# emdgroup/tnmf

Hardware: AMD Instinct MI355X
Metric: MU-iterations/sec (higher is better)
Workload: dtype f32

## Files before the change

include/tnmf_hip.h:

```cpp
#ifndef TNMF_HIP_H
#define TNMF_HIP_H

#include <stddef.h>

#ifdef __cplusplus
extern "C" {
#endif

#define TNMF_HIP_ABI_VERSION 8

enum {
    TNMF_OK = 0,
    TNMF_E_NULL = -1,
    TNMF_E_GEOM = -2,
    TNMF_E_DTYPE = -3,
    TNMF_E_WORKSPACE = -4,
    TNMF_E_UNSUPPORTED = -5,
    TNMF_E_STRIDE = -6
};

typedef struct tnmf_hip_ctx tnmf_hip_ctx;

typedef struct {
    int ndim;
    int N;
    int M;
    int C;
    int D[3];
    int A[3];
    int dtype;
    int h_row_stride;
} tnmf_hip_geom;

enum { TNMF_PATH_AUTO = 0, TNMF_PATH_GENERIC = 1, TNMF_PATH_MFMA = 2, TNMF_PATH_FFT = 3, TNMF_PATH_HYBRID = 4,
       TNMF_PATH_SPLIT = 5 };

int tnmf_hip_ctx_set_split(tnmf_hip_ctx *ctx, int enable);

int tnmf_hip_ctx_set_persistent(tnmf_hip_ctx *ctx, int mode);
int tnmf_hip_ctx_last_schedule_persistent(const tnmf_hip_ctx *ctx);

int tnmf_hip_abi_version(void);
int tnmf_hip_ctx_h_row_stride(tnmf_hip_ctx *ctx, const tnmf_hip_geom *geom, int *stride_out);
const char *tnmf_hip_strerror(int code);

int tnmf_hip_ctx_create(int device_id, tnmf_hip_ctx **out);
int tnmf_hip_ctx_destroy(tnmf_hip_ctx *ctx);
int tnmf_hip_ctx_reserve(tnmf_hip_ctx *ctx, const tnmf_hip_geom *geom);
int tnmf_hip_ctx_set_path(tnmf_hip_ctx *ctx, int path);
const char *tnmf_hip_ctx_last_path(const tnmf_hip_ctx *ctx);
int tnmf_hip_ctx_set_cache(tnmf_hip_ctx *ctx, int enable);
int tnmf_hip_ctx_invalidate(tnmf_hip_ctx *ctx);
int tnmf_hip_ctx_bind(tnmf_hip_ctx *ctx, const tnmf_hip_geom *geom, const void *H, const void *V);
int tnmf_hip_ctx_cache_counters(const tnmf_hip_ctx *ctx, unsigned long long out[4]);


int tnmf_hip_reconstruct(tnmf_hip_ctx *ctx, const tnmf_hip_geom *geom, const void *W, const void *H, void *R,
                         void *stream);

int tnmf_hip_grad_H(tnmf_hip_ctx *ctx, const tnmf_hip_geom *geom, const void *V, const void *R_or_null,
                    const void *W, const void *H, void *neg, void *pos, void *stream);

int tnmf_hip_grad_W(tnmf_hip_ctx *ctx, const tnmf_hip_geom *geom, const void *V, const void *R_or_null,
                    const void *W, const void *H, void *neg, void *pos, void *stream);

int tnmf_hip_mu_update(tnmf_hip_ctx *ctx, int dtype, void *arr, const void *neg, void *pos, double reg,
                       size_t n_elems, void *stream);

int tnmf_hip_normalize_W(tnmf_hip_ctx *ctx, const tnmf_hip_geom *geom, void *W, void *stream);

int tnmf_hip_energy(tnmf_hip_ctx *ctx, const tnmf_hip_geom *geom, const void *V, const void *W, const void *H,
                    double *out_host, void *stream);

int tnmf_hip_convolve_multi_1d(tnmf_hip_ctx *ctx, int dtype, int ndim, size_t rows, const int *shape,
                               const void *in, void *out, void *tmp, const double *kernel0, int len0,
                               const double *kernel1, int len1, void *stream);

int tnmf_hip_convolve_axis(tnmf_hip_ctx *ctx, int dtype, size_t rows, int len, size_t inner, const void *in, void *out,
                           const double *kernel, int klen, void *stream);


enum { TNMF_MODE_VALID = 0, TNMF_MODE_FULL = 1, TNMF_MODE_CIRCULAR = 2, TNMF_MODE_REFLECT = 3 };

int tnmf_hip_pad_H(tnmf_hip_ctx *ctx, const tnmf_hip_geom *geom, int mode, const void *H, void *Hpad, void *stream);
int tnmf_hip_fold_H(tnmf_hip_ctx *ctx, const tnmf_hip_geom *geom, int mode, const void *Gpad, void *G, void *stream);


int tnmf_hip_update_H(tnmf_hip_ctx *ctx, const tnmf_hip_geom *geom, const void *V, const void *W, void *H_inout,
                      void *R_scratch, int r_is_valid, double eps, double sparsity, void *stream);

int tnmf_hip_update_H_ex(tnmf_hip_ctx *ctx, const tnmf_hip_geom *geom, int mode, const void *V, const void *W,
                         void *H_inout, void *R_scratch, double eps, double sparsity, double inhibition,
                         double cross_inhibition, const double *kernel0, int len0, const double *kernel1, int len1,
                         const double *kernel2, int len2, void *stream);

int tnmf_hip_grad_W_fused(tnmf_hip_ctx *ctx, const tnmf_hip_geom *geom, const void *V, const void *W, const void *H,
                          void *R_scratch, int r_is_valid, void *negpos, void *stream);

enum { TNMF_OP_UPDATE_H = 0, TNMF_OP_GRAD_W = 1, TNMF_OP_APPLY_W = 2 };
typedef struct {
    int kind;
    int n0, n1;
    double a, b;
} tnmf_hip_op;
int tnmf_hip_run_schedule(tnmf_hip_ctx *ctx, const tnmf_hip_geom *geom, const void *V, void *W_inout, void *H_inout,
                          void *R_scratch, void *acc, const tnmf_hip_op *ops, int n_ops, double eps, double sparsity,
                          void *stream);

int tnmf_hip_axpby(tnmf_hip_ctx *ctx, int dtype, void *acc, const void *g, double a, double b, size_t n_elems,
                   void *stream);

int tnmf_hip_sum_parts(tnmf_hip_ctx *ctx, int dtype, const void *parts, int n_parts, size_t n_elems, void *out,
                       void *stream);

int tnmf_hip_apply_W(tnmf_hip_ctx *ctx, const tnmf_hip_geom *geom, void *W_inout, void *negpos, double eps,
                     void *stream);


int tnmf_hip_beta_fields(tnmf_hip_ctx *ctx, int dtype, double beta, double eps, const void *V, const void *R, void *Q,
                         void *P, size_t n_elems, void *stream);

int tnmf_hip_update_H_beta(tnmf_hip_ctx *ctx, const tnmf_hip_geom *geom, int mode, const void *V, const void *W,
                           void *H_inout, void *R_scratch, double eps, double sparsity, double inhibition,
                           double cross_inhibition, const double *kernel0, int len0, const double *kernel1, int len1,
                           const double *kernel2, int len2, double beta, void *stream);

int tnmf_hip_grad_W_beta(tnmf_hip_ctx *ctx, const tnmf_hip_geom *geom, const void *V, const void *W, const void *H,
                         void *R_scratch, int r_is_valid, void *negpos, double beta, double eps, void *stream);

int tnmf_hip_energy_beta(tnmf_hip_ctx *ctx, const tnmf_hip_geom *geom, double beta, double eps, const void *V,
                         const void *W, const void *H, double *out_host, void *stream);


int tnmf_hip_weighted_fields(tnmf_hip_ctx *ctx, int dtype, double beta, double eps, const void *V, const void *G,
                             const void *R, void *Q, void *P, size_t n_elems, void *stream);

int tnmf_hip_update_H_weighted(tnmf_hip_ctx *ctx, const tnmf_hip_geom *geom, int mode, const void *V, const void *G,
                               const void *W, void *H_inout, void *R_scratch, double eps, double sparsity,
                               double inhibition, double cross_inhibition, const double *kernel0, int len0,
                               const double *kernel1, int len1, const double *kernel2, int len2, double beta,
                               void *stream);

int tnmf_hip_grad_W_weighted(tnmf_hip_ctx *ctx, const tnmf_hip_geom *geom, const void *V, const void *G, const void *W,
                             const void *H, void *R_scratch, int r_is_valid, void *negpos, double beta, double eps,
                             void *stream);

int tnmf_hip_energy_weighted(tnmf_hip_ctx *ctx, const tnmf_hip_geom *geom, double beta, double eps, const void *V,
                             const void *G, const void *W, const void *H, double *out_host, void *stream);


int tnmf_hip_ctx_set_objective_tap(tnmf_hip_ctx *ctx, double *per_sample_dev);

int tnmf_hip_sample_objective(tnmf_hip_ctx *ctx, const tnmf_hip_geom *geom, double beta, double eps, const void *V,
                              const void *G_or_null, const void *W, const void *H, double *per_sample_dev, void *stream);

enum { TNMF_GROUP_FLIP = 0, TNMF_GROUP_MIRRORS = 1, TNMF_GROUP_ROT90 = 2, TNMF_GROUP_DIHEDRAL = 3 };

int tnmf_hip_group_expand_W(tnmf_hip_ctx *ctx, const tnmf_hip_geom *geom, int group, const void *W, void *W_eff,
                            void *stream);

int tnmf_hip_group_fold_grad_W(tnmf_hip_ctx *ctx, const tnmf_hip_geom *geom, int group, const void *negpos_eff,
                               void *negpos, void *stream);

int tnmf_hip_group_apply_W(tnmf_hip_ctx *ctx, const tnmf_hip_geom *geom, int group, void *W_inout, void *W_eff_out,
                           const void *negpos_eff, double eps, void *stream);

typedef struct tnmf_hip_atom_ops tnmf_hip_atom_ops;

int tnmf_hip_atom_ops_create(tnmf_hip_ctx *ctx, int ndim, const int *A, int T, int nnz, const int *t,
                             const int *out_px, const int *in_px, const double *w, tnmf_hip_atom_ops **out);
int tnmf_hip_atom_ops_destroy(tnmf_hip_atom_ops *ops);

int tnmf_hip_ops_expand_W(tnmf_hip_ctx *ctx, const tnmf_hip_geom *geom, const tnmf_hip_atom_ops *ops, const void *W,
                          void *W_eff, void *stream);

int tnmf_hip_ops_fold_grad_W(tnmf_hip_ctx *ctx, const tnmf_hip_geom *geom, const tnmf_hip_atom_ops *ops,
                             const void *negpos_eff, void *negpos, void *stream);

int tnmf_hip_ops_apply_W(tnmf_hip_ctx *ctx, const tnmf_hip_geom *geom, const tnmf_hip_atom_ops *ops, void *W_inout,
                         void *W_eff_out, const void *negpos_eff, double eps, void *stream);

int tnmf_hip_find_peaks(tnmf_hip_ctx *ctx, const tnmf_hip_geom *geom, const void *H, double threshold, const int *radius,
                        int group, long long *idx_out, void *val_out, size_t capacity, unsigned long long *count_out,
                        void *stream);

#define TNMF_EVENTS_CELL_1D 256
#define TNMF_EVENTS_CELL_2D 16

int tnmf_hip_events_render(tnmf_hip_ctx *ctx, const tnmf_hip_geom *geom, const void *W_eff, const int *images,
                           long long n_images, const int *cell_start, const void *strength, long long n_events, void *R,
                           void *stream);

int tnmf_hip_events_update(tnmf_hip_ctx *ctx, const tnmf_hip_geom *geom, int mode, const void *W_eff, const int *events,
                           void *strength_inout, long long n_events, const void *V, const void *R, double eps,
                           double sparsity, void *stream);

int tnmf_hip_events_gain(tnmf_hip_ctx *ctx, const tnmf_hip_geom *geom, int mode, const void *W_eff, const int *events,
                         const void *strength, long long n_events, const void *V, const void *R, double *gain,
                         double *mag , void *stream);

#ifndef TNMF_EVENTS_SEGMENT
#define TNMF_EVENTS_SEGMENT 64
#endif

int tnmf_hip_events_grad_W(tnmf_hip_ctx *ctx, const tnmf_hip_geom *geom, int mode, const int *events, const int *by_plane,
                           const int *plane_start, const void *strength, long long n_events, const void *V, const void *R,
                           void *workspace, void *negpos_eff, void *stream);

int tnmf_hip_events_norms(tnmf_hip_ctx *ctx, const tnmf_hip_geom *geom, int mode, const void *W_eff,
                          double *b , void *stream);

int tnmf_hip_pursuit_score(tnmf_hip_ctx *ctx, const tnmf_hip_geom *geom, const void *a, const double *b, void *gain_out,
// ... 12 lines not shown
```

tnmf_amd/_lib.py:

```python
import ctypes
import os
from typing import Optional, Sequence

_HERE = os.path.dirname(os.path.abspath(__file__))
LIB_PATH = os.path.join(_HERE, 'lib', 'libtnmf_hip.so')

ABI_VERSION = 8

EXPORTS = (
    'tnmf_hip_abi_version', 'tnmf_hip_strerror', 'tnmf_hip_ctx_create', 'tnmf_hip_ctx_destroy',
    'tnmf_hip_ctx_reserve', 'tnmf_hip_ctx_set_path', 'tnmf_hip_ctx_last_path', 'tnmf_hip_reconstruct',
    'tnmf_hip_grad_H', 'tnmf_hip_grad_W', 'tnmf_hip_mu_update', 'tnmf_hip_normalize_W', 'tnmf_hip_energy',
    'tnmf_hip_convolve_multi_1d', 'tnmf_hip_update_H', 'tnmf_hip_grad_W_fused', 'tnmf_hip_apply_W',
    'tnmf_hip_pad_H', 'tnmf_hip_fold_H', 'tnmf_hip_ctx_set_cache', 'tnmf_hip_ctx_invalidate',
    'tnmf_hip_ctx_set_split', 'tnmf_hip_ctx_h_row_stride', 'tnmf_hip_ctx_bind', 'tnmf_hip_ctx_set_persistent',
    'tnmf_hip_ctx_last_schedule_persistent',
    'tnmf_hip_ctx_cache_counters', 'tnmf_hip_sum_parts',
    'tnmf_hip_update_H_ex', 'tnmf_hip_run_schedule', 'tnmf_hip_axpby', 'tnmf_hip_convolve_axis',
    'tnmf_hip_beta_fields', 'tnmf_hip_update_H_beta', 'tnmf_hip_grad_W_beta', 'tnmf_hip_energy_beta',
    'tnmf_hip_weighted_fields', 'tnmf_hip_update_H_weighted', 'tnmf_hip_grad_W_weighted', 'tnmf_hip_energy_weighted',
    'tnmf_hip_group_expand_W', 'tnmf_hip_group_fold_grad_W', 'tnmf_hip_group_apply_W',
    'tnmf_hip_atom_ops_create', 'tnmf_hip_atom_ops_destroy', 'tnmf_hip_ops_expand_W', 'tnmf_hip_ops_fold_grad_W',
    'tnmf_hip_ops_apply_W',
    'tnmf_hip_ctx_set_objective_tap', 'tnmf_hip_sample_objective',
    'tnmf_hip_find_peaks',
    'tnmf_hip_events_render', 'tnmf_hip_events_update', 'tnmf_hip_events_grad_W', 'tnmf_hip_events_gain',
    'tnmf_hip_events_norms', 'tnmf_hip_pursuit_score', 'tnmf_hip_pursuit_pick',
)

MODES = {'valid': 0, 'full': 1, 'circular': 2, 'reflect': 3}

GROUPS = {'flip': 0, 'mirrors': 1, 'rot90': 2, 'dihedral': 3}

EVENT_CELLS = {1: (256,), 2: (16, 16)}
EVENT_SEGMENT = 64

PATHS = {'auto': 0, 'generic': 1, 'mfma': 2, 'fft': 3, 'hybrid': 4, 'split': 5}


class Geom(ctypes.Structure):
    _fields_ = [('ndim', ctypes.c_int), ('N', ctypes.c_int), ('M', ctypes.c_int), ('C', ctypes.c_int),
                ('D', ctypes.c_int * 3), ('A', ctypes.c_int * 3), ('dtype', ctypes.c_int),
                ('h_row_stride', ctypes.c_int)]


class Op(ctypes.Structure):
    _fields_ = [('kind', ctypes.c_int), ('n0', ctypes.c_int), ('n1', ctypes.c_int), ('a', ctypes.c_double),
                ('b', ctypes.c_double)]


OP_UPDATE_H, OP_GRAD_W, OP_APPLY_W = 0, 1, 2

E_GEOM = -2
E_UNSUPPORTED = -5
E_STRIDE = -6


class TnmfHipError(RuntimeError):
    def __init__(self, code: int, where: str, text: str):
        super().__init__(f'{where} failed with code {code}: {text}')
        self.code = code


_lib: Optional[ctypes.CDLL] = None


def load() -> ctypes.CDLL:
    global _lib
    if _lib is not None:
        return _lib
    if not os.path.exists(LIB_PATH):
        raise RuntimeError(
            f'{LIB_PATH} not found: the HIP extension is not built. The hip backend has no CPU fallback. '
            'Run `make -C tnmf_amd/csrc` (needs hipcc) first.')
    lib = ctypes.CDLL(LIB_PATH)
    missing = [name for name in EXPORTS if not hasattr(lib, name)]
    if missing:
        raise RuntimeError(f'{LIB_PATH} does not export {missing}')
    vp, ci, cd, sz = ctypes.c_void_p, ctypes.c_int, ctypes.c_double, ctypes.c_size_t
    gp = ctypes.POINTER(Geom)
    lib.tnmf_hip_abi_version.restype = ci
    lib.tnmf_hip_strerror.restype = ctypes.c_char_p
    lib.tnmf_hip_strerror.argtypes = [ci]
    lib.tnmf_hip_ctx_create.argtypes = [ci, ctypes.POINTER(vp)]
    lib.tnmf_hip_ctx_destroy.argtypes = [vp]
    lib.tnmf_hip_ctx_reserve.argtypes = [vp, gp]
    lib.tnmf_hip_ctx_set_path.argtypes = [vp, ci]
    lib.tnmf_hip_ctx_set_cache.argtypes = [vp, ci]
    lib.tnmf_hip_ctx_set_split.argtypes = [vp, ci]
    lib.tnmf_hip_ctx_set_persistent.argtypes = [vp, ci]
    lib.tnmf_hip_ctx_last_schedule_persistent.argtypes = [vp]
    lib.tnmf_hip_ctx_last_schedule_persistent.restype = ci
    lib.tnmf_hip_ctx_h_row_stride.argtypes = [vp, gp, ctypes.POINTER(ci)]
    lib.tnmf_hip_ctx_invalidate.argtypes = [vp]
    lib.tnmf_hip_ctx_bind.argtypes = [vp, gp, vp, vp]
    lib.tnmf_hip_ctx_cache_counters.argtypes = [vp, ctypes.POINTER(ctypes.c_ulonglong * 4)]
    lib.tnmf_hip_ctx_last_path.restype = ctypes.c_char_p
    lib.tnmf_hip_ctx_last_path.argtypes = [vp]
    lib.tnmf_hip_reconstruct.argtypes = [vp, gp, vp, vp, vp, vp]
    lib.tnmf_hip_grad_H.argtypes = [vp, gp, vp, vp, vp, vp, vp, vp, vp]
    lib.tnmf_hip_grad_W.argtypes = [vp, gp, vp, vp, vp, vp, vp, vp, vp]
    lib.tnmf_hip_mu_update.argtypes = [vp, ci, vp, vp, vp, cd, sz, vp]
    lib.tnmf_hip_normalize_W.argtypes = [vp, gp, vp, vp]
    lib.tnmf_hip_energy.argtypes = [vp, gp, vp, vp, vp, ctypes.POINTER(cd), vp]
    lib.tnmf_hip_convolve_multi_1d.argtypes = [vp, ci, ci, sz, ctypes.POINTER(ci), vp, vp, vp,
                                               ctypes.POINTER(cd), ci, ctypes.POINTER(cd), ci, vp]
    lib.tnmf_hip_convolve_axis.argtypes = [vp, ci, sz, ci, sz, vp, vp, ctypes.POINTER(cd), ci, vp]
    lib.tnmf_hip_update_H.argtypes = [vp, gp, vp, vp, vp, vp, ci, cd, cd, vp]
    lib.tnmf_hip_update_H_ex.argtypes = [vp, gp, ci, vp, vp, vp, vp, cd, cd, cd, cd, ctypes.POINTER(cd), ci,
                                         ctypes.POINTER(cd), ci, ctypes.POINTER(cd), ci, vp]
    lib.tnmf_hip_run_schedule.argtypes = [vp, gp, vp, vp, vp, vp, vp, ctypes.POINTER(Op), ci, cd, cd, vp]
    lib.tnmf_hip_grad_W_fused.argtypes = [vp, gp, vp, vp, vp, vp, ci, vp, vp]
    lib.tnmf_hip_apply_W.argtypes = [vp, gp, vp, vp, cd, vp]
    lib.tnmf_hip_sum_parts.argtypes = [vp, ci, vp, ci, sz, vp, vp]
    lib.tnmf_hip_axpby.argtypes = [vp, ci, vp, vp, cd, cd, sz, vp]
    lib.tnmf_hip_beta_fields.argtypes = [vp, ci, cd, cd, vp, vp, vp, vp, sz, vp]
    lib.tnmf_hip_update_H_beta.argtypes = [vp, gp, ci, vp, vp, vp, vp, cd, cd, cd, cd, ctypes.POINTER(cd), ci,
                                           ctypes.POINTER(cd), ci, ctypes.POINTER(cd), ci, cd, vp]
    lib.tnmf_hip_grad_W_beta.argtypes = [vp, gp, vp, vp, vp, vp, ci, vp, cd, cd, vp]
    lib.tnmf_hip_energy_beta.argtypes = [vp, gp, cd, cd, vp, vp, vp, ctypes.POINTER(cd), vp]
    lib.tnmf_hip_weighted_fields.argtypes = [vp, ci, cd, cd, vp, vp, vp, vp, vp, sz, vp]
    lib.tnmf_hip_update_H_weighted.argtypes = [vp, gp, ci, vp, vp, vp, vp, vp, cd, cd, cd, cd, ctypes.POINTER(cd), ci,
                                               ctypes.POINTER(cd), ci, ctypes.POINTER(cd), ci, cd, vp]
    lib.tnmf_hip_grad_W_weighted.argtypes = [vp, gp, vp, vp, vp, vp, vp, ci, vp, cd, cd, vp]
    lib.tnmf_hip_energy_weighted.argtypes = [vp, gp, cd, cd, vp, vp, vp, vp, ctypes.POINTER(cd), vp]
    lib.tnmf_hip_group_expand_W.argtypes = [vp, gp, ci, vp, vp, vp]
    lib.tnmf_hip_group_fold_grad_W.argtypes = [vp, gp, ci, vp, vp, vp]
    lib.tnmf_hip_group_apply_W.argtypes = [vp, gp, ci, vp, vp, vp, cd, vp]
    pi = ctypes.POINTER(ci)
    lib.tnmf_hip_atom_ops_create.argtypes = [vp, ci, pi, ci, ci, pi, pi, pi, ctypes.POINTER(cd), ctypes.POINTER(vp)]
    lib.tnmf_hip_atom_ops_destroy.argtypes = [vp]
    lib.tnmf_hip_ops_expand_W.argtypes = [vp, gp, vp, vp, vp, vp]
    lib.tnmf_hip_ops_fold_grad_W.argtypes = [vp, gp, vp, vp, vp, vp]
    lib.tnmf_hip_ops_apply_W.argtypes = [vp, gp, vp, vp, vp, vp, cd, vp]
    lib.tnmf_hip_ctx_set_objective_tap.argtypes = [vp, vp]
    lib.tnmf_hip_sample_objective.argtypes = [vp, gp, cd, cd, vp, vp, vp, vp, vp, vp]
    lib.tnmf_hip_find_peaks.argtypes = [vp, gp, vp, cd, pi, ci, vp, vp, sz, vp, vp]
    ll = ctypes.c_longlong
    lib.tnmf_hip_events_render.argtypes = [vp, gp, vp, vp, ll, vp, vp, ll, vp, vp]
    lib.tnmf_hip_events_update.argtypes = [vp, gp, ci, vp, vp, vp, ll, vp, vp, cd, cd, vp]
    lib.tnmf_hip_events_grad_W.argtypes = [vp, gp, ci, vp, vp, vp, vp, ll, vp, vp, vp, vp, vp]
    lib.tnmf_hip_events_gain.argtypes = [vp, gp, ci, vp, vp, vp, ll, vp, vp, vp, vp, vp]
    lib.tnmf_hip_events_norms.argtypes = [vp, gp, ci, vp, vp, vp]
    lib.tnmf_hip_pursuit_score.argtypes = [vp, gp, vp, vp, vp, vp, ll, vp]
    lib.tnmf_hip_pursuit_pick.argtypes = [vp, gp, ci, vp, vp, ll, vp, vp, vp, vp, vp, vp, vp]
    lib.tnmf_hip_pad_H.argtypes = [vp, gp, ci, vp, vp, vp]
    lib.tnmf_hip_fold_H.argtypes = [vp, gp, ci, vp, vp, vp]
    for name in EXPORTS:
        fn = getattr(lib, name)
        if fn.restype is ctypes.c_int or name not in ('tnmf_hip_strerror', 'tnmf_hip_ctx_last_path'):
            fn.restype = ci
    if lib.tnmf_hip_abi_version() != ABI_VERSION:
        raise RuntimeError(f'{LIB_PATH}: ABI version {lib.tnmf_hip_abi_version()} != expected {ABI_VERSION}')
    _lib = lib
    return lib


def check(code: int, where: str) -> None:
    if code != 0:
        text = load().tnmf_hip_strerror(code)
        raise TnmfHipError(code, where, text.decode() if text else '?')


def make_geom(n: int, m: int, c: int, sample_shape: Sequence[int], atom_shape: Sequence[int], dtype_code: int,
              h_row_stride: int = 0) -> Geom:
    k = len(atom_shape)
    if k not in (1, 2, 3) or len(sample_shape) != k:
        raise NotImplementedError('the hip backend supports 1, 2 or 3 shift dimensions')
    g = Geom()
    g.ndim, g.N, g.M, g.C, g.dtype = k, int(n), int(m), int(c), int(dtype_code)
    for i in range(k):
        g.D[i] = int(sample_shape[i])
        g.A[i] = int(atom_shape[i])
    g.h_row_stride = int(h_row_stride)
    return g
```

tnmf_amd/backends/HIP.py:

```python
from typing import Optional, Sequence, Tuple

import ctypes
import itertools
import weakref

import numpy as np
import torch

from .. import _lib, sharding, transforms as _transforms
from ._Backend import Backend, sliceNone

_DTYPES = {np.dtype('float32'): (torch.float32, 0), np.dtype('float64'): (torch.float64, 1)}


def _ptr(t: Optional[torch.Tensor]):
    return None if t is None else ctypes.c_void_p(t.data_ptr())


class _EventSpan:

    def __init__(self, backend, name):
        self.backend, self.name = backend, name

    def __enter__(self):
# ... 849 lines not shown
            _lib.check(self._lib.tnmf_hip_axpby(self._ctx, self._dtype_code, _ptr(d), _ptr(self._V_dev), -1., 1., d.numel(),
                                                self._stream()), 'tnmf_hip_axpby')
            taken = s * P + p
            for i in range(k):
                taken = taken * self._transform_shape[i] + u[:, i]
            return self.pursuit_round(W, b, d, taken.contiguous(), min_gain, buffers)

        def score(sample, plane, shift, strength, idx):
            at = torch.as_tensor(np.ascontiguousarray(idx, dtype=np.int64)).to(self._device)
            _, h, gain = self.pick_events(W, at, R)
            return h.cpu().numpy(), gain.cpu().numpy()

        def refit(sample, plane, shift, strength, n):
            return self.refit_events(V, W, sample, plane, shift, strength, n, 0., eps).cpu().numpy()
        return pursuit_loop(shape, self.atom_shape, self._sample_shape, self._reconstruction_mode, min_gain, max_events,
                            max_rounds, refit_iterations, sample.cpu().numpy(), plane.cpu().numpy(),
                            shift.cpu().numpy().reshape(-1, k), strength.cpu().numpy(), candidates, score, refit)

    def event_plane_list(self, plane: torch.Tensor, n_planes: int):
        with self._timed('event_plane_list'):
            K = plane.numel()
            sorted_plane, by_plane = torch.sort(plane, stable=True)
            plane_start = torch.searchsorted(sorted_plane, torch.arange(n_planes + 1, dtype=torch.int64,
                                                                        device=self._device)).to(torch.int32).contiguous()
            taps = self.n_channels * int(np.prod(self.atom_shape))
            workspace = torch.empty((K // _lib.EVENT_SEGMENT + n_planes) * 2 * taps, dtype=torch.float64,
                                    device=self._device)
        return by_plane.to(torch.int32).contiguous(), plane_start, workspace

    def gradient_W_event_list(self, W: torch.Tensor, events: torch.Tensor, lists, strength: torch.Tensor,
                              R: torch.Tensor) -> torch.Tensor:
        self._check_W(W)
        by_plane, plane_start, workspace = lists
        assert strength.is_contiguous() and strength.dtype == self._torch_dtype and events.shape[0] == strength.numel()
        assert by_plane.numel() == strength.numel() and plane_start.numel() == W.shape[0] + 1
        assert R.is_contiguous() and R.dtype == self._torch_dtype and tuple(R.shape) == tuple(self._V_dev.shape)
        negpos = torch.empty((2,) + tuple(W.shape), dtype=W.dtype, device=W.device)
        with self._timed('events_grad_W'):
            _lib.check(self._lib.tnmf_hip_events_grad_W(
                self._ctx, ctypes.byref(self._geom(self.n_local_samples, W.shape[0])), self._mode, _ptr(events),
                _ptr(by_plane), _ptr(plane_start), _ptr(strength), strength.numel(), _ptr(self._V_dev), _ptr(R),
                _ptr(workspace), _ptr(negpos), self._stream()), 'tnmf_hip_events_grad_W')
        return negpos

    def update_W_event_list(self, W: torch.Tensor, W_eff: Optional[torch.Tensor], transforms, negpos_eff: torch.Tensor,
                            eps: float = 1e-9) -> None:
        negpos = negpos_eff if transforms is None else self.fold_gradient_W(negpos_eff, transforms)
        self._all_reduce(negpos)
        keep = ~negpos[0].reshape(W.shape[0], -1).any(dim=1)
        kept = W.clone()
        if transforms is None:
            self.apply_W(W, negpos, eps)
        elif self._world == 1:
            self.apply_W_transformed(W, W_eff, negpos_eff, transforms, eps)
        else:
            self.apply_W(W, negpos, eps)
        W.copy_(torch.where(keep.reshape((-1,) + (1,) * (W.dim() - 1)), kept, W))
        if transforms is not None:
            self.expand_W(W, transforms, W_eff)

    def fit_events(self, V, W: torch.Tensor, W_eff: Optional[torch.Tensor], transforms, sample, plane, shift, strength,
                   n_iterations: int, update_H: bool = True, update_W: bool = True, sparsity: float = 0.,
                   eps: float = 1e-9) -> torch.Tensor:
        if self._G_dev is not None:
            raise NotImplementedError('fit_events is unweighted')
        D = W if transforms is None else W_eff
        sample, plane, shift, strength = self._check_events(D.shape[0], sample, plane, shift, strength)
        images, cell_start, events = self.event_list(sample, plane, shift)
        lists = self.event_plane_list(plane, D.shape[0]) if update_W else None
        strength = strength.clone()
        R = torch.empty_like(self._V_dev)
        for _ in range(int(n_iterations)):
            if update_H:
                self.render_event_list(D, images, cell_start, strength, R)
                self.update_event_list(D, events, strength, R, sparsity, eps)
            if update_W:
                self.render_event_list(D, images, cell_start, strength, R)
                negpos_eff = self.gradient_W_event_list(D, events, lists, strength, R)
                self.update_W_event_list(W, W_eff, transforms, negpos_eff, eps)
        return strength

    @property
    def supports_schedules(self) -> bool:
        return self._mode == 0 and self._world == 1

    def prefers_schedule(self, H: torch.Tensor) -> bool:
        return self.supports_schedules and H.shape[0] > 0 and H.numel() <= (1 << 18)

    def blend_gradient_W(self, acc: torch.Tensor, g: torch.Tensor, a: float, b: float) -> torch.Tensor:
        assert acc.is_contiguous() and g.is_contiguous() and acc.shape == g.shape and acc.dtype == g.dtype
        _lib.check(self._lib.tnmf_hip_axpby(self._ctx, self._dtype_code, _ptr(acc), _ptr(g), float(a), float(b),
                                            acc.numel(), self._stream()), 'tnmf_hip_axpby')
        return acc

    def new_gradient_accumulator(self, W: torch.Tensor) -> torch.Tensor:
        return torch.empty((2,) + tuple(W.shape), dtype=W.dtype, device=W.device)

    def run_schedule(self, V, W: torch.Tensor, H: torch.Tensor, ops, acc: torch.Tensor, sparsity: float = 0.,
                     eps: float = 1e-9) -> None:
        assert self.supports_schedules
        if self._G_dev is not None:
            raise NotImplementedError('run_schedule is unweighted; a weighted fit runs its epochs step by step')
        self._check_W(W)
        self._check_H(H, W.shape[0])
        ld = self._row_stride(H)
        assert ld is not None and H.shape[0] == self.n_local_samples
        assert acc.is_contiguous() and tuple(acc.shape) == (2,) + tuple(W.shape)
        assert acc.dtype == W.dtype and acc.device == W.device
        arr = (_lib.Op * max(1, len(ops)))()
        for i, op in enumerate(ops):
            if op[0] == 'W':
                arr[i].kind, arr[i].n0, arr[i].n1 = _lib.OP_APPLY_W, 0, 0
                continue
            sl = self._local(op[1])
            arr[i].n0, arr[i].n1 = sl.start, sl.stop
            if op[0] == 'H':
                arr[i].kind = _lib.OP_UPDATE_H
            else:
                arr[i].kind, arr[i].a, arr[i].b = _lib.OP_GRAD_W, float(op[2]), float(op[3])

        def run(Hc, ld):
            with self._timed('schedule'):
                return self._lib.tnmf_hip_run_schedule(
                    self._ctx, ctypes.byref(self._geom(Hc.shape[0], W.shape[0], ld)), _ptr(self._V_dev), _ptr(W),
                    _ptr(Hc), _ptr(self._R_scratch), _ptr(acc), arr, len(ops), float(eps), float(sparsity),
                    self._stream()), 'tnmf_hip_run_schedule'
        self._call_resident_H(H, W, True, run)

    def apply_W(self, W: torch.Tensor, negpos: torch.Tensor, eps: float = 1e-9) -> None:
        self._check_W(W)
        assert negpos.is_contiguous() and tuple(negpos.shape) == (2,) + tuple(W.shape)
        assert negpos.dtype == W.dtype and negpos.device == W.device
        g = self._geom(0, W.shape[0])
        with self._timed('apply_W'):
            _lib.check(self._lib.tnmf_hip_apply_W(self._ctx, ctypes.byref(g), _ptr(W), _ptr(negpos), float(eps),
                                                  self._stream()), 'tnmf_hip_apply_W')

    def local_gradient_W(self, V, W: torch.Tensor, H: torch.Tensor, s: slice = sliceNone, beta: float = 2.,
                         eps: float = 1e-9) -> torch.Tensor:
        self._check_beta(beta)
        ls = self._local(s)
        Hs, Vs = H[ls], self._V_dev[ls]
        self._check_W(W)
        self._check_H(Hs, W.shape[0])
        Hs = self._pad(Hs)
        negpos = torch.empty_like(self._negpos)
        Rs = self._R_scratch[ls] if Hs.shape[0] else None
        Gs = self._G(ls)

        def run(Hc, ld):
            g = self._geom(Hc.shape[0], W.shape[0], ld)
            r_valid = 0
            if self._timeline is not None and Hc.shape[0]:
                with self._timed('reconstruct'):
                    rc = self._lib.tnmf_hip_reconstruct(self._ctx, ctypes.byref(g), _ptr(W), _ptr(Hc), _ptr(Rs),
                                                        self._stream())
                if rc != 0:
                    return rc, 'tnmf_hip_reconstruct'
                r_valid = 1
            with self._timed('grad_W'):
                if Gs is not None:
                    return self._lib.tnmf_hip_grad_W_weighted(
                        self._ctx, ctypes.byref(g), _ptr(Vs), Gs, _ptr(W), _ptr(Hc), _ptr(Rs), r_valid, _ptr(negpos),
                        float(beta), float(eps), self._stream()), 'tnmf_hip_grad_W_weighted'
                rc = self._lib.tnmf_hip_grad_W_beta(self._ctx, ctypes.byref(g), _ptr(Vs), _ptr(W), _ptr(Hc), _ptr(Rs),
                                                    r_valid, _ptr(negpos), float(beta), float(eps), self._stream())
            return rc, 'tnmf_hip_grad_W_beta'
        self._call_resident_H(Hs, W, False, run)
        return negpos

    def all_reduce_gradient_W(self, negpos: torch.Tensor) -> torch.Tensor:
        self._all_reduce(negpos)
        return negpos

    def fused_update_W(self, V, W: torch.Tensor, H: torch.Tensor, s: slice = sliceNone, eps: float = 1e-9,
                       beta: float = 2.) -> None:
        negpos = self.local_gradient_W(V, W, H, s, beta=beta, eps=eps)
        self._all_reduce(negpos)
        self.apply_W(W, negpos, eps)

    def expand_W(self, W: torch.Tensor, transforms, W_eff: Optional[torch.Tensor] = None) -> torch.Tensor:
        kind, arg = self._transform_arg(transforms)
        self._check_W(W)
        shape = (W.shape[0] * _transforms.size(transforms),) + tuple(W.shape[1:])
        if W_eff is None:
            W_eff = torch.empty(shape, dtype=W.dtype, device=W.device)
        self._check_W(W_eff)
        assert tuple(W_eff.shape) == shape
        g = self._geom(0, W.shape[0])
        name = f'tnmf_hip_{kind}_expand_W'
        with self._timed(f'{kind}_expand_W'):
            _lib.check(getattr(self._lib, name)(self._ctx, ctypes.byref(g), arg, _ptr(W), _ptr(W_eff), self._stream()),
                       name)
        return W_eff

    def fold_gradient_W(self, negpos_eff: torch.Tensor, transforms) -> torch.Tensor:
        kind, arg = self._transform_arg(transforms)
        T = _transforms.size(transforms)
        assert negpos_eff.is_contiguous() and negpos_eff.dtype == self._torch_dtype and negpos_eff.shape[1] % T == 0
        assert tuple(negpos_eff.shape[2:]) == (self.n_channels,) + self.atom_shape and negpos_eff.shape[0] == 2
        M = negpos_eff.shape[1] // T
        negpos = torch.empty((2, M) + tuple(negpos_eff.shape[2:]), dtype=negpos_eff.dtype, device=negpos_eff.device)
        g = self._geom(0, M)
        name = f'tnmf_hip_{kind}_fold_grad_W'
        with self._timed(f'{kind}_fold_grad_W'):
            _lib.check(getattr(self._lib, name)(self._ctx, ctypes.byref(g), arg, _ptr(negpos_eff), _ptr(negpos),
                                                self._stream()), name)
        return negpos

    def apply_W_transformed(self, W: torch.Tensor, W_eff: torch.Tensor, negpos_eff: torch.Tensor, transforms,
                            eps: float = 1e-9) -> None:
        kind, arg = self._transform_arg(transforms)
        self._check_W(W)
        self._check_W(W_eff)
        T = _transforms.size(transforms)
        assert W_eff.shape[0] == W.shape[0] * T
        assert negpos_eff.is_contiguous() and tuple(negpos_eff.shape) == (2,) + tuple(W_eff.shape)
        assert negpos_eff.dtype == W.dtype and negpos_eff.device == W.device
        g = self._geom(0, W.shape[0])
        name = f'tnmf_hip_{kind}_apply_W'
        with self._timed(f'{kind}_apply_W'):
            _lib.check(getattr(self._lib, name)(self._ctx, ctypes.byref(g), arg, _ptr(W), _ptr(W_eff), _ptr(negpos_eff),
                                                float(eps), self._stream()), name)

    def fused_update_W_transformed(self, V, W: torch.Tensor, W_eff: torch.Tensor, H: torch.Tensor, s: slice = sliceNone,
                                   transforms=None, eps: float = 1e-9, beta: float = 2.) -> None:
        negpos_eff = self.local_gradient_W(V, W_eff, H, s, beta=beta, eps=eps)
        if self._world == 1:
            self.apply_W_transformed(W, W_eff, negpos_eff, transforms, eps)
            return
        negpos = self.fold_gradient_W(negpos_eff, transforms)
        self._all_reduce(negpos)
        self.apply_W(W, negpos, eps)
        self.expand_W(W, transforms, W_eff)
```

tnmf_amd/csrc/api.hip:

```cpp
#include <cstdlib>
#include <cstring>
#include <new>
#include <algorithm>
#include <vector>

#include "beta.h"
#include "events.h"
#include "fft.h"
#include "generic.h"
#include "mfma.h"
#include "peaks.h"
#include "split.h"
#include "volume.h"

namespace {

int to_geo(const tnmf_hip_geom *in, Geo *g) {
    if (!in) return TNMF_E_NULL;
    if (in->dtype != 0 && in->dtype != 1) return TNMF_E_DTYPE;
    if (in->ndim != 1 && in->ndim != 2) return TNMF_E_GEOM;
    g->N = in->N;
    g->M = in->M;
    g->C = in->C;
    if (in->ndim == 1) {
// ... 22 lines not shown

int to_vol(const tnmf_hip_geom *in, Vol *v) {
    if (!in) return TNMF_E_NULL;
    if (in->dtype != 0 && in->dtype != 1) return TNMF_E_DTYPE;
    v->N = in->N;
    v->M = in->M;
    v->C = in->C;
    if (v->N < 0 || v->M <= 0 || v->C <= 0) return TNMF_E_GEOM;
    for (int i = 0; i < 3; ++i) {
        v->D[i] = in->D[i];
        v->A[i] = in->A[i];
        if (v->D[i] <= 0 || v->A[i] <= 0) return TNMF_E_GEOM;
        v->H[i] = v->D[i] + v->A[i] - 1;
    }
    if (in->h_row_stride > 0 && in->h_row_stride != v->H[2]) return TNMF_E_STRIDE;
    return TNMF_OK;
}
inline size_t vol_vox(const Vol &v) { return (size_t)v.D[0] * v.D[1] * v.D[2]; }
inline size_t vol_hvox(const Vol &v) { return (size_t)v.H[0] * v.H[1] * v.H[2]; }
inline size_t vol_avox(const Vol &v) { return (size_t)v.A[0] * v.A[1] * v.A[2]; }
inline Geo vol_dict_geo(const Vol &v) {
    Geo g = {};
    g.N = v.N;
    g.M = v.M;
    g.C = v.C;
    g.Ay = v.A[0] * v.A[1];
    g.Ax = v.A[2];
    return g;
}

struct Scratch {
    size_t r_off, r_bytes;
    size_t part_off, part_bytes;
    size_t red_off, red_bytes;
    size_t total;
    int P;
};

Scratch plan_scratch(const tnmf_hip_ctx *ctx, const Geo &g, int dtype) {
    Scratch s;
    s.r_off = 0;
    s.r_bytes = align_up((size_t)g.N * g.C * g.Dy * g.Dx * esize(dtype), 256);
    int P = generic_corr_H_chunks(ctx, g);
    const int Pm = mfma_corr_H_chunks(ctx, g);
    if (Pm > P) P = Pm;
    s.P = P;
    s.part_off = s.r_off + s.r_bytes;
    s.part_bytes = align_up((size_t)P * g.M * g.C * g.Ay * g.Ax * 2 * sizeof(double), 256);
    s.red_off = s.part_off + s.part_bytes;
    s.red_bytes = align_up((size_t)(kEnergyPartials + 8) * sizeof(double), 256);
    s.total = s.red_off + s.red_bytes;
    return s;
}

int ensure_buffer(void **buf, size_t *have, size_t bytes, bool slack);

int ensure_scratch(tnmf_hip_ctx *ctx, size_t bytes) { return ensure_buffer(&ctx->ws, &ctx->ws_bytes, bytes, true); }
int ensure_hwork(tnmf_hip_ctx *ctx, size_t bytes) { return ensure_buffer(&ctx->hw, &ctx->hw_bytes, bytes, false); }

int ensure_buffer(void **buf, size_t *have, size_t bytes, bool slack) {
    if (bytes <= *have) return TNMF_OK;
    const size_t want = align_up(bytes + (slack ? bytes / 8 : 0), 1 << 20);
    void *bigger = nullptr;
    if (hipMalloc(&bigger, want) != hipSuccess) {
        (void)hipGetLastError();
        bigger = nullptr;
        if (!*buf) return TNMF_E_WORKSPACE;
    }
    if (*buf) {
        TNMF_HIP_TRY(hipDeviceSynchronize());
        TNMF_HIP_TRY(hipFree(*buf));
        *buf = nullptr;
        *have = 0;
    }
    if (!bigger && hipMalloc(&bigger, want) != hipSuccess) {
        (void)hipGetLastError();
        return TNMF_E_WORKSPACE;
    }
    *buf = bigger;
    *have = want;
    return TNMF_OK;
}

inline char *ws_at(tnmf_hip_ctx *ctx, size_t off) { return static_cast<char *>(ctx->ws) + off; }

enum Prim { kReconstruct, kCorrW, kCorrH };

bool use_fft_hybrid(const tnmf_hip_ctx *ctx, const Geo &g, int dtype) {
    if (ctx->path == TNMF_PATH_HYBRID) return fft_has(g, dtype);
    if (ctx->path != TNMF_PATH_AUTO || dtype != 0 || !fft_has(g, dtype)) return false;
    return (size_t)g.N * g.M * g.Hy * g.Hx >= ((size_t)1 << 19);
}

bool use_split(const tnmf_hip_ctx *ctx, const Geo &g, int dtype) {
    if (ctx->path == TNMF_PATH_SPLIT) return split_has_corr_W(g, dtype);
    if (ctx->path != TNMF_PATH_AUTO && ctx->path != TNMF_PATH_HYBRID) return false;
    if (ctx->path == TNMF_PATH_AUTO && (size_t)g.N * g.M * g.Hy * g.Hx < ((size_t)1 << 16)) return false;
    return ctx->split && split_has_corr_W(g, dtype, true);
}

bool use_mfma(const tnmf_hip_ctx *ctx, const Geo &g, int dtype, Prim prim) {
    if (ctx->path == TNMF_PATH_GENERIC || ctx->path == TNMF_PATH_FFT) return false;
    switch (prim) {
        case kReconstruct: return mfma_has_reconstruct(g, dtype);
        case kCorrW: return mfma_has_corr_W(g, dtype);
        default: return mfma_has_corr_H(g, dtype);
    }
}

#define ENTER(ctx, geom)                                   \
    if (!(ctx)) return TNMF_E_NULL;                        \
    Geo g;                                                 \
    {                                                      \
        const int _rc = to_geo((geom), &g);                \
        if (_rc != TNMF_OK) return _rc;                    \
    }                                                      \
    const int dtype = (geom)->dtype;                       \
    hipStream_t s = static_cast<hipStream_t>(stream);      \
    TNMF_HIP_TRY(hipSetDevice((ctx)->device));

#define CHECK(rc_expr)                  \
    do {                                \
        const int _rc = (rc_expr);      \
        if (_rc != TNMF_OK) return _rc; \
    } while (0)

#define VOL_ENTER(ctx, geom)                               \
    if (!(ctx)) return TNMF_E_NULL;                        \
    Vol v;                                                 \
    {                                                      \
        const int _rc = to_vol((geom), &v);                \
        if (_rc != TNMF_OK) return _rc;                    \
    }                                                      \
    const int dtype = (geom)->dtype;                       \
    hipStream_t s = static_cast<hipStream_t>(stream);      \
    TNMF_HIP_TRY(hipSetDevice((ctx)->device));             \
    (ctx)->last_path = "volume";

int vol_scratch(tnmf_hip_ctx *ctx, const Vol &v, int dtype, void **R, double **red, double **part = nullptr,
                int *P = nullptr, size_t extra = 0) {
    const size_t r_bytes = align_up((size_t)v.N * v.C * vol_vox(v) * esize(dtype), 256);
    const size_t e_bytes = align_up((size_t)(kEnergyPartials + 8) * sizeof(double), 256);
    const int chunks = vol_corr_H_chunks(ctx, v);
    const size_t p_bytes = align_up((size_t)chunks * v.M * v.C * vol_avox(v) * 2 * sizeof(double), 256);
    const int rc = ensure_scratch(ctx, r_bytes + e_bytes + p_bytes + extra);
    if (rc != TNMF_OK) return rc;
    if (R) *R = ws_at(ctx, 0);
    if (red) *red = reinterpret_cast<double *>(ws_at(ctx, r_bytes));
    if (part) *part = reinterpret_cast<double *>(ws_at(ctx, r_bytes + e_bytes));
    if (P) *P = chunks;
    return TNMF_OK;
}

int do_reconstruct(tnmf_hip_ctx *ctx, const Geo &g, int dtype, const void *W, const void *H, void *R, hipStream_t s) {
    if (g.N == 0) return TNMF_OK;
    if (ctx->path == TNMF_PATH_FFT || use_fft_hybrid(ctx, g, dtype)) {
        const int rc = fft_reconstruct(ctx, g, dtype, W, H, R, true, s);
        if (!(rc == TNMF_E_WORKSPACE && ctx->path == TNMF_PATH_AUTO)) return rc;
    }
    if (g.Hs == g.Hx && use_mfma(ctx, g, dtype, kReconstruct)) {
        ctx->last_path = "mfma";
        return mfma_reconstruct(ctx, g, (const float *)W, (const float *)H, (float *)R, s);
    }
    if (ctx->path == TNMF_PATH_MFMA) return g.Hs != g.Hx ? TNMF_E_STRIDE : TNMF_E_UNSUPPORTED;
    ctx->last_path = "generic";
    return generic_reconstruct(ctx, g, dtype, W, H, R, s);
}

int do_corr_W(tnmf_hip_ctx *ctx, const Geo &g, int dtype, const void *V, const void *R, const void *W, void *Hio,
              void *neg, void *pos, bool fused, double reg, hipStream_t s, const void *extra = nullptr) {
    if (g.N == 0) return TNMF_OK;
    if (extra && (!fused || ctx->path == TNMF_PATH_FFT)) return TNMF_E_UNSUPPORTED;
    if (ctx->path == TNMF_PATH_FFT)
        return fused ? fft_update_H(ctx, g, dtype, V, R, W, Hio, reg, s) : fft_grad_H(ctx, g, dtype, V, R, W, neg, pos, s);
    if (fused) fft_invalidate_H(ctx, g, dtype, Hio);
    if (use_split(ctx, g, dtype)) {
        const int rc = split_corr_W(ctx, g, (const float *)V, (const float *)R, (const float *)W, (float *)Hio,
                                    (float *)neg, (float *)pos, fused, (float)reg, s, (const float *)extra);
        if (rc == TNMF_OK) ctx->last_path = "split";
        if (rc != TNMF_E_UNSUPPORTED) return rc;
    }
    if ((!fused || g.Hs == g.Hx) && use_mfma(ctx, g, dtype, kCorrW)) {
        if (extra) return TNMF_E_UNSUPPORTED;
        ctx->last_path = "mfma";
        return mfma_corr_W(ctx, g, (const float *)V, (const float *)R, (const float *)W, (float *)Hio, (float *)neg,
                           (float *)pos, fused, (float)reg, s);
    }
    if (ctx->path == TNMF_PATH_MFMA || ctx->path == TNMF_PATH_SPLIT)
        return fused && g.Hs != g.Hx ? TNMF_E_STRIDE : TNMF_E_UNSUPPORTED;
    ctx->last_path = "generic";
    return generic_corr_W(ctx, g, dtype, V, R, W, Hio, neg, pos, fused, reg, s, extra);
}

int do_corr_H_partials(tnmf_hip_ctx *ctx, const Geo &g, int dtype, const void *V, const void *R, const void *H,
                       double *partials, int *P_out, hipStream_t s) {
    if (g.Hs == g.Hx && use_mfma(ctx, g, dtype, kCorrH)) {
        ctx->last_path = "mfma";
        *P_out = mfma_corr_H_chunks(ctx, g);
        return mfma_corr_H(ctx, g, (const float *)V, (const float *)R, (const float *)H, partials, *P_out, s);
    }
    if (ctx->path == TNMF_PATH_MFMA) return g.Hs != g.Hx ? TNMF_E_STRIDE : TNMF_E_UNSUPPORTED;
    ctx->last_path = "generic";
    *P_out = generic_corr_H_chunks(ctx, g);
    return generic_corr_H(ctx, g, dtype, V, R, H, partials, *P_out, s);
}

bool corr_H_on_fft(const tnmf_hip_ctx *ctx, const Geo &g, int dtype) {
    return ctx->path == TNMF_PATH_FFT || use_fft_hybrid(ctx, g, dtype);
}

int do_corr_H(tnmf_hip_ctx *ctx, const Geo &g, int dtype, const Scratch &sc, const void *V, const void *R,
              const void *H, void *neg, void *pos, hipStream_t s) {
    double *partials = reinterpret_cast<double *>(ws_at(ctx, sc.part_off));
    int P;
    if (g.N == 0) {
        TNMF_HIP_TRY(hipMemsetAsync(neg, 0, (size_t)g.M * g.C * g.Ay * g.Ax * esize(dtype), s));
        TNMF_HIP_TRY(hipMemsetAsync(pos, 0, (size_t)g.M * g.C * g.Ay * g.Ax * esize(dtype), s));
        return TNMF_OK;
    }
    if (corr_H_on_fft(ctx, g, dtype)) {
        const int rc = fft_grad_W(ctx, g, dtype, V, R, H, neg, pos, true, s);
        if (!(rc == TNMF_E_WORKSPACE && ctx->path == TNMF_PATH_AUTO)) return rc;
    }
    CHECK(do_corr_H_partials(ctx, g, dtype, V, R, H, partials, &P, s));
    return finalize_corr_H(g, dtype, partials, P, neg, pos, s);
}


int beta_fields_of(tnmf_hip_ctx *ctx, const Geo &g, int dtype, const double *beta, double eps, const void *V,
                   const void *G, void *R, const void **Q_out, hipStream_t s) {
    const size_t n = (size_t)g.N * g.C * g.Dy * g.Dx;
    CHECK(ensure_buffer(&ctx->qb, &ctx->qb_bytes, align_up(n * esize(dtype), 256), false));
    ctx->fft.V_volatile = ctx->qb;
    CHECK(launch_beta_fields(ctx, dtype, beta ? *beta : 2.0, eps, V, G, R, ctx->qb, R, n, s));
    *Q_out = ctx->qb;
    return TNMF_OK;
}

int sample_objective_of(tnmf_hip_ctx *ctx, int dtype, const double *beta, double eps, const void *V, const void *G,
                        const void *R, size_t N, size_t L, double *out, hipStream_t s) {
    const size_t B = objective_blocks(L);
    if (B > 1) CHECK(ensure_buffer(&ctx->ob, &ctx->ob_bytes, align_up(N * B * sizeof(double), 256), false));
    return launch_sample_objective(dtype, beta ? *beta : 2.0, eps, V, G, R, N, L, static_cast<double *>(ctx->ob), out, s);
}

inline int tap_objective(tnmf_hip_ctx *ctx, int dtype, const double *beta, double eps, const void *V, const void *G,
                         const void *R, size_t N, size_t L, hipStream_t s) {
    if (!ctx->obj_tap) return TNMF_OK;
    return sample_objective_of(ctx, dtype, beta, eps, V, G, R, N, L, ctx->obj_tap, s);
}

static_assert(kBetaPartials <= kEnergyPartials, "the energy words of the scratch hold the beta partials");

inline bool beta_ok(double beta) { return beta == beta && beta - beta == 0.0; }

int vol_api_reconstruct(tnmf_hip_ctx *ctx, const tnmf_hip_geom *geom, const void *W, const void *H, void *R, void *stream) {
    VOL_ENTER(ctx, geom);
    if (!W || (v.N > 0 && (!H || !R))) return TNMF_E_NULL;
    return vol_reconstruct(v, dtype, W, H, R, s);
}

int vol_api_grad_H(tnmf_hip_ctx *ctx, const tnmf_hip_geom *geom, const void *V, const void *R_or_null, const void *W,
                   const void *H, void *neg, void *pos, void *stream) {
    VOL_ENTER(ctx, geom);
    if (!W || (v.N > 0 && (!V || !neg || !pos))) return TNMF_E_NULL;
    const void *R = R_or_null;
    if (!R && v.N > 0) {
        if (!H) return TNMF_E_NULL;
        void *Rs;
        CHECK(vol_scratch(ctx, v, dtype, &Rs, nullptr));
        CHECK(vol_reconstruct(v, dtype, W, H, Rs, s));
        R = Rs;
    }
    return vol_corr_W(v, dtype, V, R, W, nullptr, neg, pos, false, 0.0, s);
}

int vol_api_grad_W(tnmf_hip_ctx *ctx, const tnmf_hip_geom *geom, const void *V, const void *R_scratch, int r_is_valid,
                   const void *W, const void *H, void *neg, void *pos, void *stream) {
    VOL_ENTER(ctx, geom);
    if (!neg || !pos || (v.N > 0 && (!V || !H))) return TNMF_E_NULL;
    const void *R = R_scratch;
    void *Rws;
    double *part;
    int P;
    CHECK(vol_scratch(ctx, v, dtype, &Rws, nullptr, &part, &P));
    if (v.N > 0 && !r_is_valid) {
        if (!W) return TNMF_E_NULL;
        void *Rs = R_scratch ? const_cast<void *>(R_scratch) : Rws;
        CHECK(vol_reconstruct(v, dtype, W, H, Rs, s));
        R = Rs;
    }
    return vol_corr_H(v, dtype, V, R, H, neg, pos, part, P, s);
}

int vol_api_energy(tnmf_hip_ctx *ctx, const tnmf_hip_geom *geom, const void *V, const void *W, const void *H,
                   double *out_host, void *stream) {
    VOL_ENTER(ctx, geom);
    if (!out_host) return TNMF_E_NULL;
    *out_host = 0.0;
    if (v.N == 0) return TNMF_OK;
    if (!V || !W || !H) return TNMF_E_NULL;
    void *Rs;
    double *red;
    CHECK(vol_scratch(ctx, v, dtype, &Rs, &red));
    CHECK(vol_reconstruct(v, dtype, W, H, Rs, s));
    CHECK(launch_half_sqdiff(ctx, dtype, V, Rs, (size_t)v.N * v.C * vol_vox(v), red, red + kEnergyPartials, s));
    TNMF_HIP_TRY(hipMemcpyAsync(out_host, red + kEnergyPartials, sizeof(double), hipMemcpyDeviceToHost, s));
    TNMF_HIP_TRY(hipStreamSynchronize(s));
    return TNMF_OK;
}
// ... 179 lines not shown

int tnmf_hip_ctx_create(int device_id, tnmf_hip_ctx **out) {
    if (!out) return TNMF_E_NULL;
    *out = nullptr;
    TNMF_HIP_TRY(hipSetDevice(device_id));
    hipDeviceProp_t prop;
    TNMF_HIP_TRY(hipGetDeviceProperties(&prop, device_id));
    {
        int rc = mfma_prepare_device();
        if (rc == TNMF_OK) rc = split_prepare_device();
        if (rc != TNMF_OK) return rc;
    }
    tnmf_hip_ctx *ctx = new (std::nothrow) tnmf_hip_ctx();
    if (!ctx) return TNMF_E_WORKSPACE;
    ctx->device = device_id;
    ctx->num_cu = prop.multiProcessorCount > 0 ? prop.multiProcessorCount : 256;
    ctx->path = TNMF_PATH_AUTO;
    ctx->last_path = "none";
    {
        const char *ab = tnmf_diag_env("TNMF_HIP_ABLATE");
        ctx->ablate = ab ? atoi(ab) : 0;
    }
    ctx->ws = nullptr;
    ctx->ws_bytes = 0;
    ctx->split = 1;
    ctx->wimg = nullptr;
    ctx->wimg_bytes = 0;
    ctx->fft = FftState();
    *out = ctx;
    return TNMF_OK;
}

int tnmf_hip_ctx_destroy(tnmf_hip_ctx *ctx) {
    if (!ctx) return TNMF_OK;
    int rc = TNMF_OK;
    if (ctx->ws || ctx->fft.ws || ctx->wimg || ctx->hw || ctx->qb || ctx->ob) {
        (void)hipSetDevice(ctx->device);
        (void)hipDeviceSynchronize();
    }
    fft_release(ctx);
    split_release(ctx);
    if (ctx->hw) (void)hipFree(ctx->hw);
    if (ctx->qb) (void)hipFree(ctx->qb);
    if (ctx->ob) (void)hipFree(ctx->ob);
    for (int i = 0; i < tnmf_hip_ctx::kOpSlots; ++i) {
        if (ctx->ops_done[i]) (void)hipEventDestroy(ctx->ops_done[i]);
        if (ctx->ops_pinned[i]) (void)hipHostFree(ctx->ops_pinned[i]);
    }
    if (ctx->ws) {
        const hipError_t e = hipFree(ctx->ws);
        if (e != hipSuccess) rc = (int)e;
    }
    delete ctx;
    return rc;
}

int tnmf_hip_ctx_reserve(tnmf_hip_ctx *ctx, const tnmf_hip_geom *geom) {
    void *stream = nullptr;
    if (is_vol(geom)) {
        VOL_ENTER(ctx, geom);
        (void)s;
        return vol_scratch(ctx, v, dtype, nullptr, nullptr);
    }
    ENTER(ctx, geom);
    (void)s;
    if (g.N > 0 && ctx->path == TNMF_PATH_FFT) CHECK(fft_reserve(ctx, g, dtype, true));
    if (g.N > 0 && use_fft_hybrid(ctx, g, dtype)) {
        const int rc = fft_reserve(ctx, g, dtype, false);
        if (rc != TNMF_OK && !(rc == TNMF_E_WORKSPACE && ctx->path == TNMF_PATH_AUTO)) return rc;
    }
    return ensure_scratch(ctx, plan_scratch(ctx, g, dtype).total);
}

int tnmf_hip_ctx_set_path(tnmf_hip_ctx *ctx, int path) {
    if (!ctx) return TNMF_E_NULL;
    if (path < TNMF_PATH_AUTO || path > TNMF_PATH_SPLIT) return TNMF_E_UNSUPPORTED;
    if (path != ctx->path) fft_invalidate(ctx);
    ctx->path = path;
    return TNMF_OK;
}

int tnmf_hip_ctx_set_split(tnmf_hip_ctx *ctx, int enable) {
    if (!ctx) return TNMF_E_NULL;
    ctx->split = enable != 0;
    return TNMF_OK;
}

int tnmf_hip_ctx_set_persistent(tnmf_hip_ctx *ctx, int mode) {
    if (!ctx) return TNMF_E_NULL;
    if (mode < 0 || mode > 2) return TNMF_E_UNSUPPORTED;
    ctx->persistent = mode;
    return TNMF_OK;
}

int tnmf_hip_ctx_last_schedule_persistent(const tnmf_hip_ctx *ctx) { return ctx && ctx->last_schedule_persistent ? 1 : 0; }

int tnmf_hip_ctx_set_cache(tnmf_hip_ctx *ctx, int enable) {
    if (!ctx) return TNMF_E_NULL;
    ctx->fft.cache_enabled = enable != 0;
    fft_invalidate(ctx);
    return TNMF_OK;
}

int tnmf_hip_ctx_bind(tnmf_hip_ctx *ctx, const tnmf_hip_geom *geom, const void *H, const void *V) {
    if (!ctx) return TNMF_E_NULL;
    if (!geom || !H) {
        fft_unbind(ctx);
        return TNMF_OK;
    }
    if (is_vol(geom)) {
        fft_unbind(ctx);
        return TNMF_OK;
    }
    Geo g;
    const int rc = to_geo(geom, &g);
    if (rc != TNMF_OK) return rc;
    fft_bind(ctx, g, geom->dtype, H, V);
    return TNMF_OK;
}

int tnmf_hip_ctx_cache_counters(const tnmf_hip_ctx *ctx, unsigned long long out[4]) {
    if (!ctx || !out) return TNMF_E_NULL;
    out[0] = ctx->fft.h_runs;
    out[1] = ctx->fft.h_hits;
    out[2] = ctx->fft.v_runs;
    out[3] = ctx->fft.v_hits;
    return TNMF_OK;
}

int tnmf_hip_ctx_invalidate(tnmf_hip_ctx *ctx) {
    if (!ctx) return TNMF_E_NULL;
    fft_invalidate(ctx);
    return TNMF_OK;
}

const char *tnmf_hip_ctx_last_path(const tnmf_hip_ctx *ctx) { return ctx ? ctx->last_path : "none"; }

#ifdef TNMF_DIAG
int tnmf_hip_diag_set_ablate(tnmf_hip_ctx *ctx, int mask) {
    if (!ctx) return TNMF_E_NULL;
    ctx->ablate = mask;
    return TNMF_OK;
}
#endif

int tnmf_hip_reconstruct(tnmf_hip_ctx *ctx, const tnmf_hip_geom *geom, const void *W, const void *H, void *R,
                         void *stream) {
    if (is_vol(geom)) return vol_api_reconstruct(ctx, geom, W, H, R, stream);
    ENTER(ctx, geom);
    if (!W || (g.N > 0 && (!H || !R))) return TNMF_E_NULL;
    return do_reconstruct(ctx, g, dtype, W, H, R, s);
}

int tnmf_hip_grad_H(tnmf_hip_ctx *ctx, const tnmf_hip_geom *geom, const void *V, const void *R_or_null,
                    const void *W, const void *H, void *neg, void *pos, void *stream) {
    if (is_vol(geom)) return vol_api_grad_H(ctx, geom, V, R_or_null, W, H, neg, pos, stream);
    ENTER(ctx, geom);
    if (!W || (g.N > 0 && (!V || !neg || !pos))) return TNMF_E_NULL;
    const void *R = R_or_null;
    if (!R && g.N > 0) {
        if (!H) return TNMF_E_NULL;
        const Scratch sc = plan_scratch(ctx, g, dtype);
        CHECK(ensure_scratch(ctx, sc.total));
        void *Rs = ws_at(ctx, sc.r_off);
        CHECK(do_reconstruct(ctx, g, dtype, W, H, Rs, s));
        R = Rs;
    }
    return do_corr_W(ctx, g, dtype, V, R, W, nullptr, neg, pos, false, 0.0, s);
}

int tnmf_hip_grad_W(tnmf_hip_ctx *ctx, const tnmf_hip_geom *geom, const void *V, const void *R_or_null,
                    const void *W, const void *H, void *neg, void *pos, void *stream) {
    if (is_vol(geom)) return vol_api_grad_W(ctx, geom, V, R_or_null, R_or_null != nullptr, W, H, neg, pos, stream);
    ENTER(ctx, geom);
    if (!neg || !pos || (g.N > 0 && (!V || !H))) return TNMF_E_NULL;
    const Scratch sc = plan_scratch(ctx, g, dtype);
    CHECK(ensure_scratch(ctx, sc.total));
    const void *R = R_or_null;
    if (!R && g.N > 0) {
        if (!W) return TNMF_E_NULL;
        void *Rs = ws_at(ctx, sc.r_off);
        CHECK(do_reconstruct(ctx, g, dtype, W, H, Rs, s));
        R = Rs;
    }
    return do_corr_H(ctx, g, dtype, sc, V, R, H, neg, pos, s);
}

int tnmf_hip_mu_update(tnmf_hip_ctx *ctx, int dtype, void *arr, const void *neg, void *pos, double reg,
                       size_t n_elems, void *stream) {
    if (!ctx) return TNMF_E_NULL;
    if (dtype != 0 && dtype != 1) return TNMF_E_DTYPE;
    if (n_elems > 0 && (!arr || !neg || !pos)) return TNMF_E_NULL;
    TNMF_HIP_TRY(hipSetDevice(ctx->device));
    fft_invalidate(ctx);
    return launch_mu_update(ctx, dtype, arr, neg, pos, reg, n_elems, static_cast<hipStream_t>(stream));
}

int tnmf_hip_normalize_W(tnmf_hip_ctx *ctx, const tnmf_hip_geom *geom, void *W, void *stream) {
    if (is_vol(geom)) {
        VOL_ENTER(ctx, geom);
        if (!W) return TNMF_E_NULL;
        return launch_apply_normalize_W(vol_dict_geo(v), dtype, W, nullptr, nullptr, 0.0, false, s);
    }
    ENTER(ctx, geom);
    if (!W) return TNMF_E_NULL;
    fft_invalidate_W(ctx);
    return launch_apply_normalize_W(g, dtype, W, nullptr, nullptr, 0.0, false, s);
}

static int energy_2d(tnmf_hip_ctx *ctx, const tnmf_hip_geom *geom, const void *V, const void *G, const void *W,
                     const void *H, double *out_host, const double *beta, double eps, void *stream) {
    ENTER(ctx, geom);
    if (!out_host) return TNMF_E_NULL;
    if (g.N == 0) {
        *out_host = 0.0;
        return TNMF_OK;
    }
    if (!V || !W || !H) return TNMF_E_NULL;
    const Scratch sc = plan_scratch(ctx, g, dtype);
    CHECK(ensure_scratch(ctx, sc.total));
    void *Rs = ws_at(ctx, sc.r_off);
    CHECK(do_reconstruct(ctx, g, dtype, W, H, Rs, s));
    double *red = reinterpret_cast<double *>(ws_at(ctx, sc.red_off));
    const size_t n = (size_t)g.N * g.C * g.Dy * g.Dx;
    CHECK(beta || G ? launch_beta_energy(ctx, dtype, beta ? *beta : 2.0, eps, V, G, Rs, n, red, red + kEnergyPartials, s)
                    : launch_half_sqdiff(ctx, dtype, V, Rs, n, red, red + kEnergyPartials, s));
    TNMF_HIP_TRY(hipMemcpyAsync(out_host, red + kEnergyPartials, sizeof(double), hipMemcpyDeviceToHost, s));
    TNMF_HIP_TRY(hipStreamSynchronize(s));
    return TNMF_OK;
}

int tnmf_hip_energy(tnmf_hip_ctx *ctx, const tnmf_hip_geom *geom, const void *V, const void *W, const void *H,
                    double *out_host, void *stream) {
    if (is_vol(geom)) return vol_api_energy(ctx, geom, V, W, H, out_host, stream);
    return energy_2d(ctx, geom, V, nullptr, W, H, out_host, nullptr, 0.0, stream);
}

int tnmf_hip_energy_beta(tnmf_hip_ctx *ctx, const tnmf_hip_geom *geom, double beta, double eps, const void *V,
                         const void *W, const void *H, double *out_host, void *stream) {
    if (beta == 2.0) return tnmf_hip_energy(ctx, geom, V, W, H, out_host, stream);
    if (!ctx || !geom) return TNMF_E_NULL;
    if (is_vol(geom) || !beta_ok(beta)) return TNMF_E_UNSUPPORTED;
    return energy_2d(ctx, geom, V, nullptr, W, H, out_host, &beta, eps, stream);
}

int tnmf_hip_energy_weighted(tnmf_hip_ctx *ctx, const tnmf_hip_geom *geom, double beta, double eps, const void *V,
                             const void *G, const void *W, const void *H, double *out_host, void *stream) {
    if (!G) return tnmf_hip_energy_beta(ctx, geom, beta, eps, V, W, H, out_host, stream);
    if (!ctx || !geom) return TNMF_E_NULL;
    if (is_vol(geom) || !beta_ok(beta)) return TNMF_E_UNSUPPORTED;
    return energy_2d(ctx, geom, V, G, W, H, out_host, beta == 2.0 ? nullptr : &beta, eps, stream);
}

int tnmf_hip_ctx_set_objective_tap(tnmf_hip_ctx *ctx, double *per_sample_dev) {
    if (!ctx) return TNMF_E_NULL;
    ctx->obj_tap = per_sample_dev;
    return TNMF_OK;
}

int tnmf_hip_sample_objective(tnmf_hip_ctx *ctx, const tnmf_hip_geom *geom, double beta, double eps, const void *V,
                              const void *G_or_null, const void *W, const void *H, double *per_sample_dev, void *stream) {
    if (!ctx || !geom) return TNMF_E_NULL;
    if (!beta_ok(beta)) return TNMF_E_UNSUPPORTED;
    const double *bp = beta == 2.0 ? nullptr : &beta;
    if (is_vol(geom)) {
        if (bp || G_or_null) return TNMF_E_UNSUPPORTED;
        VOL_ENTER(ctx, geom);
        if (v.N == 0) return TNMF_OK;
        if (!V || !W || !H || !per_sample_dev) return TNMF_E_NULL;
        void *Rs;
        CHECK(vol_scratch(ctx, v, dtype, &Rs, nullptr));
        CHECK(vol_reconstruct(v, dtype, W, H, Rs, s));
        return sample_objective_of(ctx, dtype, nullptr, eps, V, nullptr, Rs, (size_t)v.N, (size_t)v.C * vol_vox(v),
                                   per_sample_dev, s);
    }
    ENTER(ctx, geom);
    if (g.N == 0) return TNMF_OK;
    if (!V || !W || !H || !per_sample_dev) return TNMF_E_NULL;
    const Scratch sc = plan_scratch(ctx, g, dtype);
    CHECK(ensure_scratch(ctx, sc.total));
    void *Rs = ws_at(ctx, sc.r_off);
    CHECK(do_reconstruct(ctx, g, dtype, W, H, Rs, s));
    return sample_objective_of(ctx, dtype, bp, eps, V, G_or_null, Rs, (size_t)g.N, (size_t)g.C * g.Dy * g.Dx,
                               per_sample_dev, s);
}

int tnmf_hip_beta_fields(tnmf_hip_ctx *ctx, int dtype, double beta, double eps, const void *V, const void *R, void *Q,
                         void *P, size_t n_elems, void *stream) {
    if (!ctx) return TNMF_E_NULL;
    if (dtype != 0 && dtype != 1) return TNMF_E_DTYPE;
    if (!beta_ok(beta)) return TNMF_E_UNSUPPORTED;
    if (n_elems > 0 && (!V || !R || !Q || !P)) return TNMF_E_NULL;
    if (n_elems > 0 && (Q == V || Q == R || P == V)) return TNMF_E_NULL;
    TNMF_HIP_TRY(hipSetDevice(ctx->device));
    return launch_beta_fields(ctx, dtype, beta, eps, V, nullptr, R, Q, P, n_elems, static_cast<hipStream_t>(stream));
}

int tnmf_hip_weighted_fields(tnmf_hip_ctx *ctx, int dtype, double beta, double eps, const void *V, const void *G,
                             const void *R, void *Q, void *P, size_t n_elems, void *stream) {
    if (!ctx || !G) return TNMF_E_NULL;
    if (dtype != 0 && dtype != 1) return TNMF_E_DTYPE;
    if (!beta_ok(beta)) return TNMF_E_UNSUPPORTED;
    if (n_elems > 0 && (!V || !R || !Q || !P)) return TNMF_E_NULL;
    if (n_elems > 0 && (Q == V || Q == G || Q == R || P == V || P == G)) return TNMF_E_NULL;
    TNMF_HIP_TRY(hipSetDevice(ctx->device));
    return launch_beta_fields(ctx, dtype, beta, eps, V, G, R, Q, P, n_elems, static_cast<hipStream_t>(stream));
// ... 21 lines not shown
    if (dtype != 0 && dtype != 1) return TNMF_E_DTYPE;
    if (len < 0 || inner > 0x7fffffffu) return TNMF_E_GEOM;
    TNMF_HIP_TRY(hipSetDevice(ctx->device));
    if (rows == 0 || len == 0 || inner == 0) return TNMF_OK;
    if (!in || !out || in == out) return TNMF_E_NULL;
    return launch_convolve_axis(ctx, dtype, in, out, rows, len, (int)inner, kernel, klen, static_cast<hipStream_t>(stream));
}

int tnmf_hip_pad_H(tnmf_hip_ctx *ctx, const tnmf_hip_geom *geom, int mode, const void *H, void *Hpad, void *stream) {
    if (is_vol(geom)) return vol_api_pad_fold(ctx, geom, mode, false, H, Hpad, stream);
    ENTER(ctx, geom);
    if (mode < TNMF_MODE_VALID || mode > TNMF_MODE_REFLECT) return TNMF_E_UNSUPPORTED;
    if (g.N > 0 && (!H || !Hpad)) return TNMF_E_NULL;
    if (g.Hs != g.Hx) return TNMF_E_STRIDE;
    return launch_pad_fold(ctx, g, dtype, mode, false, H, Hpad, s);
}

int tnmf_hip_fold_H(tnmf_hip_ctx *ctx, const tnmf_hip_geom *geom, int mode, const void *Gpad, void *G, void *stream) {
    if (is_vol(geom)) return vol_api_pad_fold(ctx, geom, mode, true, Gpad, G, stream);
    ENTER(ctx, geom);
    if (mode < TNMF_MODE_VALID || mode > TNMF_MODE_REFLECT) return TNMF_E_UNSUPPORTED;
    if (g.N > 0 && (!Gpad || !G)) return TNMF_E_NULL;
    return launch_pad_fold(ctx, g, dtype, mode, true, Gpad, G, s);
}

static int update_H_2d(tnmf_hip_ctx *ctx, const tnmf_hip_geom *geom, int mode, const void *V, const void *G,
                       const void *W, void *H_inout, void *R_scratch, int r_is_valid, double eps, double sparsity,
                       double inhibition, double cross_inhibition, const double *kernel0, int len0,
                       const double *kernel1, int len1, const double *beta, void *stream) {
    ENTER(ctx, geom);
    if (mode < TNMF_MODE_VALID || mode > TNMF_MODE_REFLECT) return TNMF_E_UNSUPPORTED;
    if (g.N == 0) return TNMF_OK;
    if (!V || !W || !H_inout) return TNMF_E_NULL;
    const bool lateral = inhibition > 0 || cross_inhibition > 0;
    if (lateral && (!kernel0 || (geom->ndim == 2 && !kernel1))) return TNMF_E_NULL;
    if (inhibition < 0 || cross_inhibition < 0) return TNMF_E_GEOM;
    double reg = eps;
    if (sparsity > 0) reg += sparsity;
    const size_t es = esize(dtype);
    void *Rs = R_scratch;
    if (!Rs) {
        if (r_is_valid) return TNMF_E_NULL;
        const Scratch sc = plan_scratch(ctx, g, dtype);
        CHECK(ensure_scratch(ctx, sc.total));
        Rs = ws_at(ctx, sc.r_off);
    }
    const double one = 1.0;
    const double *ky = geom->ndim == 2 ? kernel0 : &one, *kx = geom->ndim == 2 ? kernel1 : kernel0;
    const int ly = geom->ndim == 2 ? len0 : 1, lx = geom->ndim == 2 ? len1 : len0;
    const double xc = cross_inhibition > 0 && g.M > 1 ? cross_inhibition / (g.M - 1) : 0.0;

    if (mode == TNMF_MODE_VALID) {
        const size_t nE = align_up((size_t)g.N * g.M * g.Hy * g.Hs * es, 256);
        const size_t nG = align_up((size_t)g.N * g.M * g.Hy * g.Hx * es, 256);
        void *E = nullptr;
        if (lateral) {
            CHECK(ensure_hwork(ctx, nE));
            E = ctx->hw;
            CHECK(launch_inhibition(ctx, dtype, g.N, g.M, g.Hy, g.Hs, H_inout, E, ky, ly, kx, lx, inhibition, xc, s));
        }
        if (!r_is_valid) CHECK(do_reconstruct(ctx, g, dtype, W, H_inout, Rs, s));
        CHECK(tap_objective(ctx, dtype, beta, eps, V, G, Rs, (size_t)g.N, (size_t)g.C * g.Dy * g.Dx, s));
        if (beta || G) CHECK(beta_fields_of(ctx, g, dtype, beta, eps, V, G, Rs, &V, s));
        int rc = do_corr_W(ctx, g, dtype, V, Rs, W, H_inout, nullptr, nullptr, true, reg, s, E);
        if (!E || (rc != TNMF_E_UNSUPPORTED && rc != TNMF_E_STRIDE)) return rc;
        if (ctx->hw_bytes < nE + 2 * nG) {
            CHECK(ensure_hwork(ctx, nE + 2 * nG));
            E = ctx->hw;
            CHECK(launch_inhibition(ctx, dtype, g.N, g.M, g.Hy, g.Hs, H_inout, E, ky, ly, kx, lx, inhibition, xc, s));
        }
        char *neg = static_cast<char *>(ctx->hw) + nE, *pos = neg + nG;
        CHECK(do_corr_W(ctx, g, dtype, V, Rs, W, nullptr, neg, pos, false, 0.0, s));
        fft_invalidate_H(ctx, g, dtype, H_inout);
        return launch_mu_update_extra(ctx, dtype, H_inout, neg, pos, E, (size_t)g.N * g.M * g.Hy, g.Hx, g.Hs, reg, s);
    }

    if (g.Hs != g.Hx) return TNMF_E_STRIDE;
    const int Sy = geom->ndim == 1 ? 1 : (mode == TNMF_MODE_FULL ? g.Dy - g.Ay + 1 : g.Dy);
    const int Sx = mode == TNMF_MODE_FULL ? g.Dx - g.Ax + 1 : g.Dx;
    if (Sy < 1 || Sx < 1) return TNMF_E_GEOM;
    const size_t nP = align_up((size_t)g.N * g.M * g.Hy * g.Hx * es, 256);
    const size_t nE = lateral ? align_up((size_t)g.N * g.M * Sy * Sx * es, 256) : 0;
    CHECK(ensure_hwork(ctx, 3 * nP + nE));
    char *Hp = static_cast<char *>(ctx->hw), *negp = Hp + nP, *posp = negp + nP;
    void *E = lateral ? posp + nP : nullptr;
    fft_invalidate(ctx);
    CHECK(launch_pad_fold(ctx, g, dtype, mode, false, H_inout, Hp, s));
    CHECK(do_reconstruct(ctx, g, dtype, W, Hp, Rs, s));
    CHECK(tap_objective(ctx, dtype, beta, eps, V, G, Rs, (size_t)g.N, (size_t)g.C * g.Dy * g.Dx, s));
    if (beta || G) CHECK(beta_fields_of(ctx, g, dtype, beta, eps, V, G, Rs, &V, s));
    CHECK(do_corr_W(ctx, g, dtype, V, Rs, W, nullptr, negp, posp, false, 0.0, s));
    if (lateral) CHECK(launch_inhibition(ctx, dtype, g.N, g.M, Sy, Sx, H_inout, E, ky, ly, kx, lx, inhibition, xc, s));
    fft_invalidate(ctx);
    return launch_fold_update(ctx, g, dtype, mode, Sy, Sx, H_inout, negp, posp, E, reg, s);
}

int tnmf_hip_update_H(tnmf_hip_ctx *ctx, const tnmf_hip_geom *geom, const void *V, const void *W, void *H_inout,
                      void *R_scratch, int r_is_valid, double eps, double sparsity, void *stream) {
    if (is_vol(geom)) return vol_api_update_H(ctx, geom, V, W, H_inout, R_scratch, r_is_valid, eps, sparsity, stream);
    return update_H_2d(ctx, geom, TNMF_MODE_VALID, V, nullptr, W, H_inout, R_scratch, r_is_valid, eps, sparsity, 0.0, 0.0,
                       nullptr, 0, nullptr, 0, nullptr, stream);
}

int tnmf_hip_update_H_ex(tnmf_hip_ctx *ctx, const tnmf_hip_geom *geom, int mode, const void *V, const void *W,
                         void *H_inout, void *R_scratch, double eps, double sparsity, double inhibition,
                         double cross_inhibition, const double *kernel0, int len0, const double *kernel1, int len1,
                         const double *kernel2, int len2, void *stream) {
    if (is_vol(geom)) {
        const double *const kern[3] = {kernel0, kernel1, kernel2};
        const int klen[3] = {len0, len1, len2};
        return vol_api_update_H_ex(ctx, geom, mode, V, W, H_inout, R_scratch, eps, sparsity, inhibition, cross_inhibition,
                                   kern, klen, stream);
    }
    return update_H_2d(ctx, geom, mode, V, nullptr, W, H_inout, R_scratch, 0, eps, sparsity, inhibition,
                       cross_inhibition, kernel0, len0, kernel1, len1, nullptr, stream);
}

int tnmf_hip_update_H_beta(tnmf_hip_ctx *ctx, const tnmf_hip_geom *geom, int mode, const void *V, const void *W,
                           void *H_inout, void *R_scratch, double eps, double sparsity, double inhibition,
                           double cross_inhibition, const double *kernel0, int len0, const double *kernel1, int len1,
                           const double *kernel2, int len2, double beta, void *stream) {
    if (beta == 2.0)
        return tnmf_hip_update_H_ex(ctx, geom, mode, V, W, H_inout, R_scratch, eps, sparsity, inhibition,
                                    cross_inhibition, kernel0, len0, kernel1, len1, kernel2, len2, stream);
    if (!ctx || !geom) return TNMF_E_NULL;
    if (is_vol(geom) || !beta_ok(beta)) return TNMF_E_UNSUPPORTED;
    return update_H_2d(ctx, geom, mode, V, nullptr, W, H_inout, R_scratch, 0, eps, sparsity, inhibition,
                       cross_inhibition, kernel0, len0, kernel1, len1, &beta, stream);
}

int tnmf_hip_update_H_weighted(tnmf_hip_ctx *ctx, const tnmf_hip_geom *geom, int mode, const void *V, const void *G,
                               const void *W, void *H_inout, void *R_scratch, double eps, double sparsity,
                               double inhibition, double cross_inhibition, const double *kernel0, int len0,
                               const double *kernel1, int len1, const double *kernel2, int len2, double beta,
                               void *stream) {
    if (!G)
        return tnmf_hip_update_H_beta(ctx, geom, mode, V, W, H_inout, R_scratch, eps, sparsity, inhibition,
                                      cross_inhibition, kernel0, len0, kernel1, len1, kernel2, len2, beta, stream);
    if (!ctx || !geom) return TNMF_E_NULL;
    if (is_vol(geom) || !beta_ok(beta)) return TNMF_E_UNSUPPORTED;
    return update_H_2d(ctx, geom, mode, V, G, W, H_inout, R_scratch, 0, eps, sparsity, inhibition, cross_inhibition,
                       kernel0, len0, kernel1, len1, beta == 2.0 ? nullptr : &beta, stream);
}

static int grad_W_2d(tnmf_hip_ctx *ctx, const tnmf_hip_geom *geom, const void *V, const void *G, const void *W,
                     const void *H, void *R_scratch, int r_is_valid, void *negpos, const double *beta, double eps,
                     void *stream) {
    ENTER(ctx, geom);
    if (!negpos || !W || (g.N > 0 && (!V || !H))) return TNMF_E_NULL;
    const Scratch sc = plan_scratch(ctx, g, dtype);
    CHECK(ensure_scratch(ctx, sc.total));
    if (r_is_valid && !R_scratch) return TNMF_E_NULL;
    void *Rs = R_scratch ? R_scratch : ws_at(ctx, sc.r_off);
    if (!r_is_valid) CHECK(do_reconstruct(ctx, g, dtype, W, H, Rs, s));
    if ((beta || G) && g.N > 0) CHECK(beta_fields_of(ctx, g, dtype, beta, eps, V, G, Rs, &V, s));
    char *np = static_cast<char *>(negpos);
    const size_t wbytes = (size_t)g.M * g.C * g.Ay * g.Ax * esize(dtype);
    return do_corr_H(ctx, g, dtype, sc, V, Rs, H, np, np + wbytes, s);
}

int tnmf_hip_grad_W_fused(tnmf_hip_ctx *ctx, const tnmf_hip_geom *geom, const void *V, const void *W, const void *H,
                          void *R_scratch, int r_is_valid, void *negpos, void *stream) {
    if (is_vol(geom)) {
        if (!negpos || (r_is_valid && !R_scratch)) return TNMF_E_NULL;
        Vol vv;
        CHECK(to_vol(geom, &vv));
        char *np3 = static_cast<char *>(negpos);
        return vol_api_grad_W(ctx, geom, V, R_scratch, r_is_valid, W, H, np3,
                              np3 + (size_t)vv.M * vv.C * vol_avox(vv) * esize(geom->dtype), stream);
    }
    return grad_W_2d(ctx, geom, V, nullptr, W, H, R_scratch, r_is_valid, negpos, nullptr, 0.0, stream);
}

int tnmf_hip_grad_W_beta(tnmf_hip_ctx *ctx, const tnmf_hip_geom *geom, const void *V, const void *W, const void *H,
                         void *R_scratch, int r_is_valid, void *negpos, double beta, double eps, void *stream) {
    if (beta == 2.0) return tnmf_hip_grad_W_fused(ctx, geom, V, W, H, R_scratch, r_is_valid, negpos, stream);
    if (!ctx || !geom) return TNMF_E_NULL;
    if (is_vol(geom) || !beta_ok(beta)) return TNMF_E_UNSUPPORTED;
    return grad_W_2d(ctx, geom, V, nullptr, W, H, R_scratch, r_is_valid, negpos, &beta, eps, stream);
}

int tnmf_hip_grad_W_weighted(tnmf_hip_ctx *ctx, const tnmf_hip_geom *geom, const void *V, const void *G, const void *W,
                             const void *H, void *R_scratch, int r_is_valid, void *negpos, double beta, double eps,
                             void *stream) {
    if (!G) return tnmf_hip_grad_W_beta(ctx, geom, V, W, H, R_scratch, r_is_valid, negpos, beta, eps, stream);
    if (!ctx || !geom) return TNMF_E_NULL;
    if (is_vol(geom) || !beta_ok(beta)) return TNMF_E_UNSUPPORTED;
    return grad_W_2d(ctx, geom, V, G, W, H, R_scratch, r_is_valid, negpos, beta == 2.0 ? nullptr : &beta, eps, stream);
}

int tnmf_hip_run_schedule(tnmf_hip_ctx *ctx, const tnmf_hip_geom *geom, const void *V, void *W_inout, void *H_inout,
                          void *R_scratch, void *acc, const tnmf_hip_op *ops, int n_ops, double eps, double sparsity,
                          void *stream) {
    if (is_vol(geom))
        return vol_api_run_schedule(ctx, geom, V, W_inout, H_inout, R_scratch, acc, ops, n_ops, eps, sparsity, stream);
    ENTER(ctx, geom);
    if (n_ops < 0 || (n_ops > 0 && !ops)) return TNMF_E_NULL;
    if (!V || !W_inout || !H_inout || !acc) return TNMF_E_NULL;
    const size_t es = esize(dtype);
    const size_t vs = (size_t)g.C * g.Dy * g.Dx * es, hs = (size_t)g.M * g.Hy * g.Hs * es;
    const size_t wn = (size_t)g.M * g.C * g.Ay * g.Ax;
    for (int i = 0; i < n_ops; ++i) {
        if (ops[i].kind != TNMF_OP_UPDATE_H && ops[i].kind != TNMF_OP_GRAD_W && ops[i].kind != TNMF_OP_APPLY_W)
            return TNMF_E_UNSUPPORTED;
        if (ops[i].kind == TNMF_OP_APPLY_W) continue;
        if (ops[i].n0 < 0 || ops[i].n1 < ops[i].n0 || ops[i].n1 > g.N) return TNMF_E_GEOM;
    }
    std::vector<tnmf_hip_op> joined;
    joined.reserve(n_ops);
    for (int i = 0; i < n_ops;) {
        if (ops[i].kind != TNMF_OP_UPDATE_H) {
            joined.push_back(ops[i++]);
            continue;
        }
        int j = i;
        while (j < n_ops && ops[j].kind == TNMF_OP_UPDATE_H) ++j;
        std::vector<tnmf_hip_op> run(ops + i, ops + j);
        run.erase(std::remove_if(run.begin(), run.end(), [](const tnmf_hip_op &o) { return o.n1 <= o.n0; }), run.end());
        std::vector<tnmf_hip_op> sorted_run = run;
        std::sort(sorted_run.begin(), sorted_run.end(), [](const tnmf_hip_op &a, const tnmf_hip_op &b) { return a.n0 < b.n0; });
        bool disjoint = true;
        for (size_t k = 1; k < sorted_run.size(); ++k) disjoint = disjoint && sorted_run[k].n0 >= sorted_run[k - 1].n1;
        if (!disjoint) {
            joined.insert(joined.end(), run.begin(), run.end());
        } else {
            for (size_t k = 0; k < sorted_run.size(); ++k) {
                if (!joined.empty() && joined.back().kind == TNMF_OP_UPDATE_H && k > 0 && joined.back().n1 == sorted_run[k].n0)
                    joined.back().n1 = sorted_run[k].n1;
                else
                    joined.push_back(sorted_run[k]);
            }
        }
        i = j;
    }
    ops = joined.data();
    n_ops = (int)joined.size();
    int nmax = 1;
    for (int i = 0; i < n_ops; ++i)
        if (ops[i].kind != TNMF_OP_APPLY_W && ops[i].n1 - ops[i].n0 > nmax) nmax = ops[i].n1 - ops[i].n0;
    double reg = eps;
    if (sparsity > 0) reg += sparsity;
    (void)nmax;
    const bool tiny = (size_t)g.N * g.M * g.Hy * g.Hx <= ((size_t)1 << 18);
    if (n_ops > 0 && tiny && ctx->persistent != 0 && (ctx->path == TNMF_PATH_AUTO || ctx->path == TNMF_PATH_GENERIC) &&
        generic_schedule_fits(ctx, g, dtype)) {
        const int P = generic_schedule_chunks(ctx, g);
        const size_t r_bytes = R_scratch ? 0 : align_up((size_t)g.N * vs, 256);
        const size_t p_bytes = align_up((size_t)P * wn * 2 * sizeof(double), 256);
        const size_t o_bytes = align_up((size_t)n_ops * sizeof(tnmf_hip_op), 256);
        CHECK(ensure_scratch(ctx, r_bytes + p_bytes + o_bytes + 1024));
        void *Rs = R_scratch ? R_scratch : static_cast<void *>(ws_at(ctx, 0));
        double *partials = reinterpret_cast<double *>(ws_at(ctx, r_bytes));
        tnmf_hip_op *ops_dev = reinterpret_cast<tnmf_hip_op *>(ws_at(ctx, r_bytes + p_bytes));
        unsigned *counter = reinterpret_cast<unsigned *>(ws_at(ctx, r_bytes + p_bytes + o_bytes));
        {
            const int slot = ctx->ops_next;
            ctx->ops_next = (slot + 1) % tnmf_hip_ctx::kOpSlots;
            const size_t need = (size_t)n_ops * sizeof(tnmf_hip_op);
            if (ctx->ops_done[slot]) TNMF_HIP_TRY(hipEventSynchronize(ctx->ops_done[slot]));
            else TNMF_HIP_TRY(hipEventCreateWithFlags(&ctx->ops_done[slot], hipEventDisableTiming));
            if (ctx->ops_cap[slot] < need) {
                if (ctx->ops_pinned[slot]) TNMF_HIP_TRY(hipHostFree(ctx->ops_pinned[slot]));
                ctx->ops_pinned[slot] = nullptr;
                ctx->ops_cap[slot] = 0;
                if (hipHostMalloc(&ctx->ops_pinned[slot], align_up(need, 4096), hipHostMallocDefault) != hipSuccess) {
                    (void)hipGetLastError();
                    return TNMF_E_WORKSPACE;
                }
                ctx->ops_cap[slot] = align_up(need, 4096);
            }
            memcpy(ctx->ops_pinned[slot], ops, need);
            TNMF_HIP_TRY(hipMemcpyAsync(ops_dev, ctx->ops_pinned[slot], need, hipMemcpyHostToDevice, s));
            TNMF_HIP_TRY(hipEventRecord(ctx->ops_done[slot], s));
        }
        fft_invalidate(ctx);
        ctx->last_path = "generic";
        const int rc = generic_run_schedule(ctx, g, dtype, V, W_inout, H_inout, Rs, acc, partials, P, ops_dev, n_ops, reg,
                                            eps, counter, s);
        if (rc != TNMF_E_UNSUPPORTED) {
            ctx->last_schedule_persistent = rc == TNMF_OK;
            return rc;
        }
    }
    ctx->last_schedule_persistent = false;
    Geo gmax = g;
    gmax.N = nmax;
    const Scratch scm = plan_scratch(ctx, gmax, dtype);
    const size_t grad_off = scm.total;
    CHECK(ensure_scratch(ctx, scm.total + align_up(2 * wn * es, 256)));
    char *grad = ws_at(ctx, grad_off);
    for (int i = 0; i < n_ops; ++i) {
        const tnmf_hip_op &op = ops[i];
        Geo gs = g;
        gs.N = op.n1 - op.n0;
        const char *Vb = static_cast<const char *>(V) + (size_t)op.n0 * vs;
        char *Hb = static_cast<char *>(H_inout) + (size_t)op.n0 * hs;
        void *Rb = R_scratch ? static_cast<void *>(static_cast<char *>(R_scratch) + (size_t)op.n0 * vs)
                             : static_cast<void *>(ws_at(ctx, scm.r_off));
        switch (op.kind) {
            case TNMF_OP_UPDATE_H:
                if (gs.N == 0) break;
                CHECK(do_reconstruct(ctx, gs, dtype, W_inout, Hb, Rb, s));
                CHECK(do_corr_W(ctx, gs, dtype, Vb, Rb, W_inout, Hb, nullptr, nullptr, true, reg, s));
                break;
            case TNMF_OP_GRAD_W: {
                Scratch sc = plan_scratch(ctx, gs, dtype);
                sc.part_off = scm.part_off;
// ... 246 lines not shown
```

tnmf_amd/csrc/common.h:

```cpp
#pragma once

#include <hip/hip_runtime.h>
#include <stddef.h>
#include <stdint.h>

#include "tnmf_hip.h"

struct Geo {
    int N, M, C;
    int Dy, Dx;
    int Ay, Ax;
    int Hy, Hx;
    int Hs;
};

#include <vector>
struct FftState {
    void *ws = nullptr;
    size_t ws_bytes = 0;
    size_t failed_bytes = 0;
    bool cache_enabled = false;
    bool bound = false;
    bool explicit_bind = false;
    const void *H_base = nullptr;
    const void *V_base = nullptr;
    const void *V_volatile = nullptr;
    Geo geo = {};
    int dtype = 0;
    std::vector<unsigned char> T_ok;
    std::vector<unsigned char> SH_ok;
    std::vector<unsigned char> V_ok;
    std::vector<unsigned char> SV_ok;
    const void *W_owner = nullptr;
    bool W_ok = false;
    Geo W_geo = {};
    int W_dtype = 0;
    unsigned long long h_runs = 0, h_hits = 0, v_runs = 0, v_hits = 0;
};

struct tnmf_hip_ctx {
    int device;
    int num_cu;
    int path;
    const char *last_path;
    int ablate;
    void *ws;
    size_t ws_bytes;
    int split;
    void *wimg;
    size_t wimg_bytes;
    void *hw = nullptr;
    size_t hw_bytes = 0;
    void *qb = nullptr;
    size_t qb_bytes = 0;
    double *obj_tap = nullptr;
    void *ob = nullptr;
    size_t ob_bytes = 0;
    static constexpr int kOpSlots = 4;
    void *ops_pinned[kOpSlots] = {nullptr, nullptr, nullptr, nullptr};
    size_t ops_cap[kOpSlots] = {0, 0, 0, 0};
    hipEvent_t ops_done[kOpSlots] = {nullptr, nullptr, nullptr, nullptr};
    int ops_next = 0;
    int persistent = 1;
    bool last_schedule_persistent = false;
    FftState fft;
};

#ifdef TNMF_DIAG
#include <stdlib.h>
#define TNMF_ABL(x) (x)
static inline const char *tnmf_diag_env(const char *name) { return getenv(name); }
#else
#define TNMF_ABL(x) 0
static inline const char *tnmf_diag_env(const char *) { return nullptr; }
#endif

#define TNMF_HIP_TRY(expr)                          \
    do {                                            \
        hipError_t _e = (expr);                     \
        if (_e != hipSuccess) return (int)_e;       \
    } while (0)

#define TNMF_LAUNCH_CHECK()                         \
    do {                                            \
        hipError_t _e = hipGetLastError();          \
        if (_e != hipSuccess) return (int)_e;       \
    } while (0)

static inline size_t align_up(size_t x, size_t a) { return (x + a - 1) / a * a; }
static inline int cdiv(int a, int b) { return (a + b - 1) / b; }
```

tnmf_amd/csrc/fft.h:

```cpp
#pragma once
#include "common.h"

struct FftArgs {
    const void *src0, *src1, *src2;
    void *dst0, *dst1;
    long ps_src, ps_dst;
    int planes, rows, cols;
    int ld_src, ld_dst;
    int KX, KXP;
    int yoff, xoff;
    int N, M, C, Hy;
    int n0, ngroups, nper;
    int mgroups, mper;
    int clamp0;
    double reg;
};

enum FftOp {
    kFftRowsFwd = 0,
    kFftRowsInv,
    kFftRowsInv2,
    kFftRowsMu,
    kFftColsFwd,
    kFftColsInv,
    kFftContractR,
    kFftGradH,
    kFftGradW,
};

typedef int (*fft_run_fn)(int op, int dtype, const FftArgs *a, hipStream_t s);
#define TNMF_FFT_DECL(L) int fft_run_##L(int op, int dtype, const FftArgs *a, hipStream_t s)
TNMF_FFT_DECL(32);
TNMF_FFT_DECL(48);
TNMF_FFT_DECL(64);
TNMF_FFT_DECL(96);
TNMF_FFT_DECL(144);
TNMF_FFT_DECL(192);
TNMF_FFT_DECL(270);
TNMF_FFT_DECL(288);
TNMF_FFT_DECL(384);
TNMF_FFT_DECL(540);
TNMF_FFT_DECL(576);
#undef TNMF_FFT_DECL

bool mixed_has_reconstruct(const Geo &g, int dtype);
bool mixed_has_grad_W(const Geo &g, int dtype);
int mixed_reconstruct(const Geo &g, const void *Tsp, const void *WT, void *OT, int KX, int KXP, hipStream_t s);
int mixed_grad_W(const Geo &g, const void *Tsp, const void *VT, const void *RT, void *Gn, void *Gp, int KX, int KXP,
                 int ngroups, int nper, hipStream_t s);

#ifndef TNMF_MIX_W3_WAVES
#define TNMF_MIX_W3_WAVES 3
#endif
constexpr int kMixW3Atoms = 16, kMixW3Waves = TNMF_MIX_W3_WAVES, kMixW3MaxAy = 12;
constexpr long kMixW3MinBytes = 24L << 20;
constexpr int mix_w3_waves(int Ay) {
    const int w = Ay >= 8 ? 3 : (Ay >= 4 ? 4 : (Ay >= 2 ? 5 : 7));
    return kMixW3Waves < 3 ? kMixW3Waves : w;
}
bool mixed_grad_W3_takes(const Geo &g, int KXP);

int spectral_contract_R(const Geo &g, int dtype, const void *SH, const void *SW, void *SR, int Ly, int KX, int KXP,
                        hipStream_t s);
int spectral_grad_W(const Geo &g, int dtype, const void *SH, const void *SV, const void *SR, void *Gn, void *Gp, int Ly,
                    int KX, int KXP, int ngroups, int nper, hipStream_t s);

bool fft_has(const Geo &g, int dtype);
void fft_invalidate(tnmf_hip_ctx *ctx);
void fft_invalidate_H(tnmf_hip_ctx *ctx, const Geo &g, int dtype, const void *H);
void fft_bind(tnmf_hip_ctx *ctx, const Geo &g, int dtype, const void *H, const void *V);
void fft_unbind(tnmf_hip_ctx *ctx);
void fft_invalidate_W(tnmf_hip_ctx *ctx);
void fft_release(tnmf_hip_ctx *ctx);
int fft_reserve(tnmf_hip_ctx *ctx, const Geo &g, int dtype, bool with_window);

int fft_reconstruct(tnmf_hip_ctx *ctx, const Geo &g, int dtype, const void *W, const void *H, void *R, bool nonneg,
                    hipStream_t s);
int fft_grad_H(tnmf_hip_ctx *ctx, const Geo &g, int dtype, const void *V, const void *R, const void *W, void *neg,
               void *pos, hipStream_t s);
int fft_update_H(tnmf_hip_ctx *ctx, const Geo &g, int dtype, const void *V, const void *R, const void *W, void *H,
                 double reg, hipStream_t s);
int fft_grad_W(tnmf_hip_ctx *ctx, const Geo &g, int dtype, const void *V, const void *R, const void *H, void *neg,
               void *pos, bool nonneg, hipStream_t s);
```

tnmf_amd/csrc/fft.hip:

```cpp
#include <algorithm>
#include <cstdlib>

#include "fft.h"
#include "fft_engine.h"

namespace {

const int kLensY[] = {32, 48, 64, 96, 144, 192, 270, 288, 384, 576};
const int kLensX[] = {32, 48, 64, 96, 144, 192, 270, 288, 384, 540, 576};
constexpr int kMixMaxGroups = 128;

int pick_len(int h, int dtype, bool along_x, bool tall = false) {
    if (along_x || tall) {
        for (int L : kLensX)
            if (L >= h && (dtype == 0 || L <= 288)) return L;
        return 0;
    }
    for (int L : kLensY)
        if (L >= h && (dtype == 0 || L <= 288)) return L;
    return 0;
}

bool tall_columns(const tnmf_hip_ctx *ctx) { return ctx->path != TNMF_PATH_FFT; }

fft_run_fn lookup(int L) {
    switch (L) {
        case 32: return fft_run_32;
        case 48: return fft_run_48;
        case 64: return fft_run_64;
        case 96: return fft_run_96;
        case 144: return fft_run_144;
        case 192: return fft_run_192;
        case 270: return fft_run_270;
        case 288: return fft_run_288;
        case 384: return fft_run_384;
        case 540: return fft_run_540;
        case 576: return fft_run_576;
        default: return nullptr;
    }
}

bool use_mixed(const Geo &g, int dtype, bool grad_W);

struct Lay {
    int Ly, Lx, KX, KXP, ngroups, nper, chunk, mgroups, mper;
    fft_run_fn rowf, colf;
    size_t csz;
    size_t T, SH, Tn, Tp, SV, SR, Ts, VT, RT, SW, SWf, TW, TWr, Wt, Gn, Gp, Gs, Wo, total, total_no_window;
    size_t sT, sSH, sS, sD;
    bool resident;
};

void sample_groups(const Geo &g, int tiles, int *ngroups, int *nper) {
    int ng = cdiv(2048, g.M * tiles);
    if (ng > 16) ng = 16;
    if (ng > g.N) ng = g.N;
    if (ng < 1) ng = 1;
    *nper = cdiv(g.N > 0 ? g.N : 1, ng);
    *ngroups = cdiv(g.N > 0 ? g.N : 1, *nper);
}

bool make_layout(const tnmf_hip_ctx *ctx, const Geo &gfull, const Geo &g, int dtype, Lay *l) {
    l->Ly = pick_len(g.Hy, dtype, false, tall_columns(ctx));
    l->Lx = pick_len(g.Hx, dtype, true);
    if (!l->Ly || !l->Lx) return false;
    l->rowf = lookup(l->Lx);
    l->colf = lookup(l->Ly);
    l->KX = l->Lx / 2 + 1;
    l->KXP = (int)align_up((size_t)l->KX, 16);
    l->csz = dtype == 0 ? 8 : 16;
    const int tiles = cdiv(l->KX, l->Ly > 384 ? 8 : 16);
    int ngroups_full, nper_full;
    sample_groups(gfull, tiles, &ngroups_full, &nper_full);
    sample_groups(g, tiles, &l->ngroups, &l->nper);
    const size_t c = l->csz, kxp = (size_t)l->KXP;
    const size_t Nf = gfull.N > 0 ? gfull.N : 1;
    l->sT = (size_t)g.M * g.Hy * kxp * c;
    l->sSH = (size_t)g.M * l->Ly * kxp * c;
    l->sS = (size_t)g.C * l->Ly * kxp * c;
    l->sD = (size_t)g.C * g.Dy * kxp * c;
    size_t budget = (size_t)8 << 30;
    if (const char *e = tnmf_diag_env("TNMF_FFT_WINDOW_MB")) budget = (size_t)atol(e) << 20;
    long chunk_full = (long)(budget / (2 * l->sT));
    if (chunk_full < 1) chunk_full = 1;
    if (chunk_full > (long)Nf) chunk_full = (long)Nf;
    l->chunk = (int)(chunk_full > g.N && g.N > 0 ? g.N : chunk_full);
    int mg = cdiv(1024, l->chunk * cdiv(l->KX, 16) * 2);
    if (mg > g.M) mg = g.M;
    if (mg < 1) mg = 1;
    l->mper = cdiv(g.M, mg);
    l->mgroups = cdiv(g.M, l->mper);
    const size_t nSW = (size_t)g.M * g.C * l->Ly * kxp * c;
    size_t o = 0;
    auto take = [&o](size_t bytes) {
        const size_t at = o;
        o += align_up(bytes, 256);
        return at;
    };
    l->T = take(Nf * l->sT + (size_t)64 * kxp * c);
    l->resident = !(use_mixed(g, dtype, false) && use_mixed(g, dtype, true));
    l->SH = take(l->resident ? Nf * l->sSH : 0);
    l->SV = take(Nf * l->sS);
    l->SR = take(Nf * l->sS);
    l->Ts = take(Nf * l->sD);
    l->VT = take(Nf * l->sD);
    l->RT = take(Nf * l->sD);
    l->SW = take(nSW);
    l->SWf = take(nSW);
    l->TW = take((size_t)2 * g.M * g.C * g.Ay * kxp * c);
    l->TWr = take((size_t)g.M * g.C * g.Ay * kxp * c);
    l->Wt = take((size_t)2 * g.M * g.C * g.Ay * g.Ax * (c / 2));
    const size_t nG = std::max(nSW * ngroups_full, (size_t)kMixMaxGroups * g.M * g.C * g.Ay * kxp * c);
    l->Gn = take(nG);
    l->Gp = take(nG);
    l->Gs = take(nSW * 2);
    l->Wo = take((size_t)2 * g.M * g.C * g.Ay * g.Ax * (c / 2));
    l->total_no_window = o;
    const size_t nTc = (size_t)chunk_full * l->sT;
    l->Tn = take(nTc);
    l->Tp = take(nTc);
    l->total = o;
    return true;
}

void clear_flags(FftState &f) {
    f.W_ok = false;
    std::fill(f.T_ok.begin(), f.T_ok.end(), 0);
    std::fill(f.SH_ok.begin(), f.SH_ok.end(), 0);
    std::fill(f.V_ok.begin(), f.V_ok.end(), 0);
    std::fill(f.SV_ok.begin(), f.SV_ok.end(), 0);
}

int ensure_ws(tnmf_hip_ctx *ctx, size_t bytes) {
    FftState &f = ctx->fft;
    if (bytes <= f.ws_bytes) return TNMF_OK;
    if (f.failed_bytes && bytes >= f.failed_bytes) return TNMF_E_WORKSPACE;
    const size_t want = align_up(bytes, 1 << 20);
    void *bigger = nullptr;
    if (hipMalloc(&bigger, want) != hipSuccess) {
        (void)hipGetLastError();
        bigger = nullptr;
        if (!f.ws) {
            f.failed_bytes = bytes;
            return TNMF_E_WORKSPACE;
        }
    }
    if (f.ws) {
        TNMF_HIP_TRY(hipDeviceSynchronize());
        TNMF_HIP_TRY(hipFree(f.ws));
        f.ws = nullptr;
        f.ws_bytes = 0;
        clear_flags(f);
    }
    if (!bigger && hipMalloc(&bigger, want) != hipSuccess) {
        (void)hipGetLastError();
        f.failed_bytes = bytes;
        return TNMF_E_WORKSPACE;
    }
    f.ws = bigger;
    f.ws_bytes = want;
    clear_flags(f);
    return TNMF_OK;
}

inline char *at(tnmf_hip_ctx *ctx, size_t off) { return static_cast<char *>(ctx->fft.ws) + off; }

#define CHECK(rc_expr)                  \
    do {                                \
        const int _rc = (rc_expr);      \
        if (_rc != TNMF_OK) return _rc; \
    } while (0)

template <typename T>
__global__ void k_fft_prep_W(const T *W, T *out0, T *out1, int planes, int Ay, int Ax, double scale) {
    const int i = blockIdx.x * blockDim.x + threadIdx.x, per = Ay * Ax;
    if (i >= planes * per) return;
    const int p = i / per, r = i - p * per, ay = r / Ax, ax = r - ay * Ax;
    const T v = (T)(scale * (double)W[i]);
    out0[i] = v;
    out1[(long)p * per + (Ay - 1 - ay) * Ax + (Ax - 1 - ax)] = v;
}

template <typename T>
__global__ __launch_bounds__(64) void k_fft_sum_groups(const cplx<T> *parts0, const cplx<T> *parts1, cplx<T> *out0,
                                                      cplx<T> *out1, long count, int ngroups, double scale) {
    const long i = (long)blockIdx.x * blockDim.x + threadIdx.x;
    if (i >= count) return;
    const cplx<T> *parts = blockIdx.y ? parts1 : parts0;
    double re = 0, im = 0;
    int gidx = 0;
    for (; gidx + 4 <= ngroups; gidx += 4) {
        cplx<T> v[4];
#pragma unroll
        for (int k = 0; k < 4; ++k) v[k] = parts[(gidx + k) * count + i];
#pragma unroll
        for (int k = 0; k < 4; ++k) {
            re += (double)v[k].x;
            im += (double)v[k].y;
        }
    }
    for (; gidx < ngroups; ++gidx) {
        const cplx<T> v = parts[gidx * count + i];
        re += (double)v.x;
        im += (double)v.y;
    }
    (blockIdx.y ? out1 : out0)[i] = {(T)(re * scale), (T)(im * scale)};
}

template <typename T>
__global__ void k_fft_flip_out(const T *in, T *out, int planes, int Ay, int Ax, int clamp0) {
    const int i = blockIdx.x * blockDim.x + threadIdx.x, per = Ay * Ax;
    if (i >= planes * per) return;
    const int p = i / per, r = i - p * per, ay = r / Ax, ax = r - ay * Ax;
    T v = in[(long)p * per + (Ay - 1 - ay) * Ax + (Ax - 1 - ax)];
    if (clamp0) v = v < (T)0 ? (T)0 : v;
    out[i] = v;
}

FftArgs base_args(const Geo &g, const Lay &l) {
    FftArgs a = {};
    a.KX = l.KX;
    a.KXP = l.KXP;
    a.N = g.N;
    a.M = g.M;
    a.C = g.C;
    a.Hy = g.Hy;
    return a;
}

int forward_planes(const Geo &g, const Lay &l, int dtype, const void *src, int planes, int rows, int cols, void *Ttmp,
                   void *S, hipStream_t s) {
    FftArgs a = base_args(g, l);
    a.src0 = src;
    a.dst0 = Ttmp;
    a.planes = planes;
    a.rows = rows;
    a.cols = cols;
    a.ld_src = cols;
    a.ps_src = (long)rows * cols;
    a.ps_dst = (long)rows * l.KXP;
    CHECK(l.rowf(kFftRowsFwd, dtype, &a, s));
    FftArgs b = base_args(g, l);
    b.src0 = Ttmp;
    b.dst0 = S;
    b.planes = planes;
    b.rows = rows;
    return l.colf(kFftColsFwd, dtype, &b, s);
}

bool use_mixed(const Geo &g, int dtype, bool grad_W) {
    static const bool off = tnmf_diag_env("TNMF_FFT_NO_MIXED") != nullptr;
    return !off && (grad_W ? mixed_has_grad_W(g, dtype) : mixed_has_reconstruct(g, dtype));
}

bool use_resident(const Lay &l) {
    static const bool off = tnmf_diag_env("TNMF_FFT_NO_RESIDENT") != nullptr;
    return l.resident && !off;
}

int scaled_W(tnmf_hip_ctx *ctx, const Geo &g, const Lay &l, int dtype, const void *W, double scale, hipStream_t s) {
    const int planes = g.M * g.C, n = planes * g.Ay * g.Ax;
    char *wt = at(ctx, l.Wt);
    const size_t half = (size_t)n * (l.csz / 2);
    if (dtype == 0)
        hipLaunchKernelGGL(k_fft_prep_W<float>, dim3(cdiv(n, 256)), dim3(256), 0, s, (const float *)W, (float *)wt,
                           (float *)(wt + half), planes, g.Ay, g.Ax, scale);
    else
        hipLaunchKernelGGL(k_fft_prep_W<double>, dim3(cdiv(n, 256)), dim3(256), 0, s, (const double *)W, (double *)wt,
                           (double *)(wt + half), planes, g.Ay, g.Ax, scale);
    TNMF_LAUNCH_CHECK();
    return TNMF_OK;
}

int spectra_W(tnmf_hip_ctx *ctx, const Geo &g, const Lay &l, int dtype, const void *W, bool plain, bool flipped,
              hipStream_t s) {
    const int planes = g.M * g.C, per = g.Ay * g.Ax, n = planes * per;
    const double scale = 1.0 / ((double)l.Ly * l.Lx);
    char *wt = at(ctx, l.Wt);
    const size_t half = (size_t)n * (l.csz / 2);
    if (dtype == 0)
        hipLaunchKernelGGL(k_fft_prep_W<float>, dim3(cdiv(n, 256)), dim3(256), 0, s, (const float *)W, (float *)wt,
                           (float *)(wt + half), planes, g.Ay, g.Ax, scale);
    else
        hipLaunchKernelGGL(k_fft_prep_W<double>, dim3(cdiv(n, 256)), dim3(256), 0, s, (const double *)W, (double *)wt,
                           (double *)(wt + half), planes, g.Ay, g.Ax, scale);
    TNMF_LAUNCH_CHECK();
    if (plain) CHECK(forward_planes(g, l, dtype, wt, planes, g.Ay, g.Ax, at(ctx, l.TW), at(ctx, l.SW), s));
    if (flipped) CHECK(forward_planes(g, l, dtype, wt + half, planes, g.Ay, g.Ax, at(ctx, l.TW), at(ctx, l.SWf), s));
    return TNMF_OK;
}


inline size_t esz_of(int dtype) { return dtype == 0 ? 4 : 8; }

bool same_shape(const Geo &a, const Geo &b) {
    return a.M == b.M && a.C == b.C && a.Dy == b.Dy && a.Dx == b.Dx && a.Ay == b.Ay && a.Ax == b.Ax && a.Hs == b.Hs;
}

void bind(FftState &f, const Geo &g, int dtype, const void *H, const void *V, bool explicit_bind) {
    f.bound = true;
    f.explicit_bind = explicit_bind;
    f.H_base = H;
    f.V_base = V;
    f.geo = g;
    f.dtype = dtype;
    const size_t n = g.N > 0 ? (size_t)g.N : 0;
    f.T_ok.assign(n, 0);
    f.SH_ok.assign(n, 0);
    f.V_ok.assign(n, 0);
    f.SV_ok.assign(n, 0);
}

struct Slot {
    int n0;
    bool cached;
    bool v_cached;
};

Slot locate(FftState &f, const Geo &g, int dtype, const void *H, const void *V) {
    Slot sl = {0, false, false};
    if (!f.cache_enabled || !f.bound || dtype != f.dtype || !same_shape(f.geo, g) || g.N <= 0) return sl;
    const size_t es = esz_of(dtype);
    const size_t hb = (size_t)g.M * g.Hy * g.Hs * es, vb = (size_t)g.C * g.Dy * g.Dx * es;
    long n0 = -1;
    if (H) {
        const ptrdiff_t d = static_cast<const char *>(H) - static_cast<const char *>(f.H_base);
        if (!f.H_base || d < 0 || (size_t)d % hb) return sl;
        n0 = (long)((size_t)d / hb);
    } else if (V && f.V_base) {
        const ptrdiff_t d = static_cast<const char *>(V) - static_cast<const char *>(f.V_base);
        if (d < 0 || (size_t)d % vb) return sl;
        n0 = (long)((size_t)d / vb);
    }
    if (n0 < 0 || n0 + g.N > f.geo.N) return sl;
    sl.n0 = (int)n0;
    sl.cached = true;
    if (V) {
        if (!f.V_base) {
            f.V_base = static_cast<const char *>(V) - (size_t)n0 * vb;
            std::fill(f.V_ok.begin(), f.V_ok.end(), 0);
            std::fill(f.SV_ok.begin(), f.SV_ok.end(), 0);
        }
        sl.v_cached = static_cast<const char *>(V) == static_cast<const char *>(f.V_base) + (size_t)n0 * vb;
    }
    return sl;
}

bool all_ok(const std::vector<unsigned char> &v, int n0, int n) {
    for (int i = n0; i < n0 + n; ++i)
        if (!v[i]) return false;
    return true;
}
void set_ok(std::vector<unsigned char> &v, int n0, int n, unsigned char val) {
    for (int i = n0; i < n0 + n && i < (int)v.size(); ++i) v[i] = val;
}

struct Call {
    Lay l;
    Slot sl;
    char *T, *SH, *SV, *SR, *Ts, *VT, *RT;
};

int prepare(tnmf_hip_ctx *ctx, const Geo &g, int dtype, const void *H, const void *V, Call *c, bool window = false) {
    if (!fft_has(g, dtype)) return TNMF_E_UNSUPPORTED;
    FftState &f = ctx->fft;
    if (V && V == f.V_volatile) V = nullptr;
    c->sl = locate(f, g, dtype, H, V);
    if (!c->sl.cached) {
        if (f.cache_enabled && !f.explicit_bind && (H || V)) {
            bind(f, g, dtype, H, V, false);
            c->sl = {0, H != nullptr, V != nullptr};
        } else {
            clear_flags(f);
        }
    }
    const bool in_binding = c->sl.cached || c->sl.v_cached;
    if (!make_layout(ctx, in_binding ? f.geo : g, g, dtype, &c->l)) return TNMF_E_UNSUPPORTED;
    CHECK(ensure_ws(ctx, window ? c->l.total : c->l.total_no_window));
    const Lay &l = c->l;
    const size_t n0 = (size_t)c->sl.n0;
    c->T = at(ctx, l.T) + n0 * l.sT;
    c->SH = at(ctx, l.SH) + n0 * l.sSH;
    c->SV = at(ctx, l.SV) + n0 * l.sS;
    c->SR = at(ctx, l.SR) + n0 * l.sS;
    c->Ts = at(ctx, l.Ts) + n0 * l.sD;
    c->VT = at(ctx, l.VT) + n0 * l.sD;
    c->RT = at(ctx, l.RT) + n0 * l.sD;
    ctx->last_path = "fft";
    return TNMF_OK;
}

int forward_rows(const Geo &g, const Lay &l, int dtype, const void *src, int planes, int rows, int cols, void *Tdst,
                 hipStream_t s) {
    FftArgs a = base_args(g, l);
    a.src0 = src;
    a.dst0 = Tdst;
    a.planes = planes;
    a.rows = rows;
    a.cols = cols;
    a.ld_src = cols;
    a.ps_src = (long)rows * cols;
    a.ps_dst = (long)rows * l.KXP;
    return l.rowf(kFftRowsFwd, dtype, &a, s);
}

int columns_of(const Geo &g, const Lay &l, int dtype, const void *Tsrc, int planes, int rows, void *S, hipStream_t s) {
    FftArgs b = base_args(g, l);
    b.src0 = Tsrc;
    b.dst0 = S;
    b.planes = planes;
    b.rows = rows;
    return l.colf(kFftColsFwd, dtype, &b, s);
}

int spectra_V(tnmf_hip_ctx *ctx, const Geo &g, const Call &c, int dtype, const void *V, bool full, hipStream_t s) {
    FftState &f = ctx->fft;
    const Lay &l = c.l;
    const bool track = c.sl.v_cached && f.cache_enabled;
    const bool hit = track && all_ok(f.V_ok, c.sl.n0, g.N);
    ++(hit ? f.v_hits : f.v_runs);
    if (!track && c.sl.cached) {
        set_ok(f.V_ok, c.sl.n0, g.N, 0);
        set_ok(f.SV_ok, c.sl.n0, g.N, 0);
    }
    if (!hit) {
        if (track) {
            set_ok(f.V_ok, c.sl.n0, g.N, 0);
            set_ok(f.SV_ok, c.sl.n0, g.N, 0);
        }
        CHECK(forward_rows(g, l, dtype, V, g.N * g.C, g.Dy, g.Dx, c.VT, s));
        if (track) set_ok(f.V_ok, c.sl.n0, g.N, 1);
    }
    if (full && !(hit && all_ok(f.SV_ok, c.sl.n0, g.N))) {
        CHECK(columns_of(g, l, dtype, c.VT, g.N * g.C, g.Dy, c.SV, s));
        if (track) set_ok(f.SV_ok, c.sl.n0, g.N, 1);
    }
    return TNMF_OK;
}

int rows_of_H(tnmf_hip_ctx *ctx, const Geo &g, const Call &c, int dtype, const void *H, hipStream_t s) {
    FftState &f = ctx->fft;
    const bool track = c.sl.cached && f.cache_enabled;
    if (track && all_ok(f.T_ok, c.sl.n0, g.N)) {
        ++f.h_hits;
        return TNMF_OK;
    }
    ++f.h_runs;
    if (track) {
        set_ok(f.T_ok, c.sl.n0, g.N, 0);
        set_ok(f.SH_ok, c.sl.n0, g.N, 0);
    }
    FftArgs a = base_args(g, c.l);
    a.src0 = H;
    a.dst0 = c.T;
    a.planes = g.N * g.M;
    a.rows = g.Hy;
    a.cols = g.Hx;
    a.ld_src = g.Hs;
    a.ps_src = (long)g.Hy * g.Hs;
    a.ps_dst = (long)g.Hy * c.l.KXP;
    CHECK(c.l.rowf(kFftRowsFwd, dtype, &a, s));
    if (track) set_ok(f.T_ok, c.sl.n0, g.N, 1);
    return TNMF_OK;
}

int spectra_of_H(tnmf_hip_ctx *ctx, const Geo &g, const Call &c, int dtype, const void *H, hipStream_t s) {
    FftState &f = ctx->fft;
    CHECK(rows_of_H(ctx, g, c, dtype, H, s));
    const bool track = c.sl.cached && f.cache_enabled;
    if (track && all_ok(f.SH_ok, c.sl.n0, g.N)) return TNMF_OK;
    CHECK(columns_of(g, c.l, dtype, c.T, g.N * g.M, g.Hy, c.SH, s));
    if (track) set_ok(f.SH_ok, c.sl.n0, g.N, 1);
    return TNMF_OK;
}

}

bool fft_has(const Geo &g, int dtype) {
    if (g.Dy == 1 && g.Ay == 1) {
        return pick_len(g.Hx, dtype, true) != 0 && mixed_has_reconstruct(g, dtype) && mixed_has_grad_W(g, dtype);
    }
    return pick_len(g.Hy, dtype, false) != 0 && pick_len(g.Hx, dtype, true) != 0;
}

void fft_bind(tnmf_hip_ctx *ctx, const Geo &g, int dtype, const void *H, const void *V) {
    bind(ctx->fft, g, dtype, H, V, true);
}

void fft_unbind(tnmf_hip_ctx *ctx) {
    FftState &f = ctx->fft;
    f.bound = f.explicit_bind = false;
    f.H_base = f.V_base = nullptr;
    f.T_ok.clear();
    f.SH_ok.clear();
    f.V_ok.clear();
    f.SV_ok.clear();
}

void fft_invalidate_H(tnmf_hip_ctx *ctx, const Geo &g, int dtype, const void *H) {
    FftState &f = ctx->fft;
    const Slot sl = locate(f, g, dtype, H, nullptr);
    if (sl.cached) {
        set_ok(f.T_ok, sl.n0, g.N, 0);
        set_ok(f.SH_ok, sl.n0, g.N, 0);
    } else {
        std::fill(f.T_ok.begin(), f.T_ok.end(), 0);
        std::fill(f.SH_ok.begin(), f.SH_ok.end(), 0);
    }
}

void fft_invalidate(tnmf_hip_ctx *ctx) { clear_flags(ctx->fft); }

void fft_invalidate_W(tnmf_hip_ctx *ctx) { ctx->fft.W_ok = false; }

int fft_reserve(tnmf_hip_ctx *ctx, const Geo &g, int dtype, bool with_window) {
    Lay l;
    ctx->fft.failed_bytes = 0;
    const FftState &f = ctx->fft;
    const bool in_binding = f.bound && f.dtype == dtype && same_shape(f.geo, g) && f.geo.N >= g.N;
    if (!fft_has(g, dtype) || !make_layout(ctx, in_binding ? f.geo : g, g, dtype, &l)) return TNMF_E_UNSUPPORTED;
    return ensure_ws(ctx, with_window ? l.total : l.total_no_window);
}

void fft_release(tnmf_hip_ctx *ctx) {
    if (ctx->fft.ws) (void)hipFree(ctx->fft.ws);
    ctx->fft.ws = nullptr;
    ctx->fft.ws_bytes = 0;
    ctx->fft.failed_bytes = 0;
    clear_flags(ctx->fft);
}

int fft_reconstruct(tnmf_hip_ctx *ctx, const Geo &g, int dtype, const void *W, const void *H, void *R, bool nonneg,
                    hipStream_t s) {
    Call c;
    CHECK(prepare(ctx, g, dtype, H, nullptr, &c));
    const Lay &l = c.l;
    CHECK(rows_of_H(ctx, g, c, dtype, H, s));
    FftState &f = ctx->fft;
    const bool w_hit = f.cache_enabled && f.W_ok && f.W_owner == W && f.W_dtype == dtype && same_shape(f.W_geo, g) &&
                       (c.sl.cached || f.W_geo.N == g.N);
    auto w_mark = [&]() {
        f.W_ok = f.cache_enabled;
        f.W_owner = W;
        f.W_geo = g;
        f.W_dtype = dtype;
    };
    if (use_mixed(g, dtype, false)) {
        if (!w_hit) {
            f.W_ok = false;
            CHECK(scaled_W(ctx, g, l, dtype, W, 1.0 / l.Lx, s));
            CHECK(forward_rows(g, l, dtype, at(ctx, l.Wt), g.M * g.C, g.Ay, g.Ax, at(ctx, l.TWr), s));
            w_mark();
        }
        CHECK(mixed_reconstruct(g, c.T, at(ctx, l.TWr), c.Ts, l.KX, l.KXP, s));
    } else {
        if (!w_hit) {
            f.W_ok = false;
            CHECK(spectra_W(ctx, g, l, dtype, W, true, false, s));
            w_mark();
        }
        if (use_resident(l)) {
            CHECK(spectra_of_H(ctx, g, c, dtype, H, s));
            CHECK(spectral_contract_R(g, dtype, c.SH, at(ctx, l.SW), c.SR, l.Ly, l.KX, l.KXP, s));
        } else {
            FftArgs a = base_args(g, l);
            a.src0 = c.T;
            a.src1 = at(ctx, l.SW);
            a.dst0 = c.SR;
            CHECK(l.colf(kFftContractR, dtype, &a, s));
        }
        FftArgs b = base_args(g, l);
        b.src0 = c.SR;
        b.dst0 = c.Ts;
        b.planes = g.N * g.C;
        b.rows = g.Dy;
        b.yoff = g.Ay - 1;
        CHECK(l.colf(kFftColsInv, dtype, &b, s));
    }
    FftArgs d = base_args(g, l);
    d.src0 = c.Ts;
    d.dst0 = R;
    d.planes = g.N * g.C;
    d.rows = g.Dy;
    d.cols = g.Dx;
    d.xoff = g.Ax - 1;
    d.ld_dst = g.Dx;
    d.ps_dst = (long)g.Dy * g.Dx;
    d.clamp0 = nonneg ? 1 : 0;
    return l.rowf(kFftRowsInv, dtype, &d, s);
}

namespace {

int grad_H_spectra(tnmf_hip_ctx *ctx, const Geo &g, const Call &c, int dtype, const void *V, const void *R,
                   const void *W, hipStream_t s) {
    CHECK(spectra_W(ctx, g, c.l, dtype, W, false, true, s));
    CHECK(spectra_V(ctx, g, c, dtype, V, true, s));
    return forward_planes(g, c.l, dtype, R, g.N * g.C, g.Dy, g.Dx, c.Ts, c.SR, s);
}

int grad_H_window(tnmf_hip_ctx *ctx, const Geo &g, const Call &c, int dtype, int n0, int cnt, hipStream_t s) {
    const Lay &l = c.l;
    FftArgs a = base_args(g, l);
    a.src0 = c.SV;
    a.src1 = c.SR;
    a.src2 = at(ctx, l.SWf);
    a.dst0 = at(ctx, l.Tn);
    a.dst1 = at(ctx, l.Tp);
    a.n0 = n0;
    a.planes = cnt;
    a.mgroups = l.mgroups;
    a.mper = l.mper;
    return l.colf(kFftGradH, dtype, &a, s);
}

}

int fft_grad_H(tnmf_hip_ctx *ctx, const Geo &g, int dtype, const void *V, const void *R, const void *W, void *neg,
               void *pos, hipStream_t s) {
    if (g.Dy == 1 && g.Ay == 1) return TNMF_E_UNSUPPORTED;
    Call c;
    CHECK(prepare(ctx, g, dtype, nullptr, V, &c, true));
    const Lay &l = c.l;
    CHECK(grad_H_spectra(ctx, g, c, dtype, V, R, W, s));
    const size_t esz = l.csz / 2, hplane = (size_t)g.M * g.Hy * g.Hx;
    for (int n0 = 0; n0 < g.N; n0 += l.chunk) {
        const int cnt = g.N - n0 < l.chunk ? g.N - n0 : l.chunk;
        CHECK(grad_H_window(ctx, g, c, dtype, n0, cnt, s));
        FftArgs a = base_args(g, l);
        a.src0 = at(ctx, l.Tn);
        a.src1 = at(ctx, l.Tp);
        a.dst0 = static_cast<char *>(neg) + (size_t)n0 * hplane * esz;
        a.dst1 = static_cast<char *>(pos) + (size_t)n0 * hplane * esz;
        a.planes = cnt * g.M;
        a.rows = g.Hy;
        a.cols = g.Hx;
        a.xoff = 0;
        a.ld_dst = g.Hx;
        a.ps_dst = (long)g.Hy * g.Hx;
        CHECK(l.rowf(kFftRowsInv2, dtype, &a, s));
    }
    return TNMF_OK;
}

int fft_update_H(tnmf_hip_ctx *ctx, const Geo &g, int dtype, const void *V, const void *R, const void *W, void *H,
                 double reg, hipStream_t s) {
    if (g.Dy == 1 && g.Ay == 1) return TNMF_E_UNSUPPORTED;
    Call c;
    CHECK(prepare(ctx, g, dtype, H, V, &c, true));
    const Lay &l = c.l;
    FftState &f = ctx->fft;
    const bool track = c.sl.cached && f.cache_enabled;
    CHECK(grad_H_spectra(ctx, g, c, dtype, V, R, W, s));
    if (track) {
        set_ok(f.T_ok, c.sl.n0, g.N, 0);
        set_ok(f.SH_ok, c.sl.n0, g.N, 0);
    }
    const size_t esz = l.csz / 2, hplane = (size_t)g.M * g.Hy * g.Hs;
    for (int n0 = 0; n0 < g.N; n0 += l.chunk) {
        const int cnt = g.N - n0 < l.chunk ? g.N - n0 : l.chunk;
        CHECK(grad_H_window(ctx, g, c, dtype, n0, cnt, s));
        FftArgs a = base_args(g, l);
        a.src0 = at(ctx, l.Tn);
        a.src1 = at(ctx, l.Tp);
        a.dst0 = static_cast<char *>(H) + (size_t)n0 * hplane * esz;
        a.dst1 = c.T + (size_t)n0 * l.sT;
        a.planes = cnt * g.M;
        a.rows = g.Hy;
        a.cols = g.Hx;
        a.ld_dst = g.Hs;
        a.ps_src = (long)g.Hy * g.Hs;
        a.ps_dst = (long)g.Hy * l.KXP;
        a.reg = reg;
        CHECK(l.rowf(kFftRowsMu, dtype, &a, s));
    }
    if (track) set_ok(f.T_ok, c.sl.n0, g.N, 1);
    return TNMF_OK;
}

int mix_groups(const tnmf_hip_ctx *ctx, const Geo &g, const Lay &l) {
    const long slots = 2L * 4 * (ctx->num_cu > 0 ? ctx->num_cu : 256);
    const long per_group_block = (long)(g.C == 1 && g.Ay <= 12 ? cdiv(g.M, 2) : g.M) * cdiv(l.KX, 16);
    int best = 32;
    double best_cost = 1e30;
    for (int cand = 32; cand <= kMixMaxGroups; cand *= 2) {
        int ng = g.N < cand ? g.N : cand;
        const int nper = cdiv(g.N, ng);
        ng = cdiv(g.N, nper);
        const double rounds = (double)(per_group_block * cdiv(ng, 4)) / (double)slots;
        const double whole = rounds <= 1.0 ? 1.0 : (double)(long)(rounds + 0.999999);
        const double cost = whole / rounds + 0.03 * (cand / 32);
        if (cost < best_cost - 1e-9) {
            best_cost = cost;
            best = cand;
        }
    }
    return best;
}

int mix_groups_w3(const tnmf_hip_ctx *ctx, const Geo &g, const Lay &l) {
    const long slots3 = (long)mix_w3_waves(g.Ay) * (ctx->num_cu > 0 ? ctx->num_cu : 256);
    const long per_group = (long)cdiv(g.M, kMixW3Atoms) * cdiv(l.KX, 16);
    int best = 1;
    double best_cost = 1e30;
    for (int cand = g.N < kMixMaxGroups ? g.N : kMixMaxGroups; cand >= 1; --cand) {
        const int ng = cdiv(g.N, cdiv(g.N, cand));
        const double rounds = (double)(per_group * ng) / (double)slots3;
        const double whole = rounds <= 1.0 ? 1.0 : (double)(long)(rounds + 0.999999);
        const double cost3 = whole / rounds + 0.03 * ng / 32.0;
        if (cost3 < best_cost - 1e-9) {
            best_cost = cost3;
            best = ng;
        }
    }
    return best;
}

int fft_grad_W(tnmf_hip_ctx *ctx, const Geo &g, int dtype, const void *V, const void *R, const void *H, void *neg,
               void *pos, bool nonneg, hipStream_t s) {
    Call c;
    CHECK(prepare(ctx, g, dtype, H, V, &c));
    const Lay &l = c.l;
    CHECK(rows_of_H(ctx, g, c, dtype, H, s));
    const bool mixed = use_mixed(g, dtype, true);
    CHECK(spectra_V(ctx, g, c, dtype, V, !mixed, s));
    const int planes = 2 * g.M * g.C;
    if (mixed) {
        CHECK(forward_rows(g, l, dtype, R, g.N * g.C, g.Dy, g.Dx, c.RT, s));
        int ng_want = mix_groups(ctx, g, l);
        if (const char *e = tnmf_diag_env("TNMF_MIX_GROUPS")) ng_want = atoi(e);
        ng_want = ng_want < 1 ? 1 : (ng_want > kMixMaxGroups ? kMixMaxGroups : ng_want);
        int ng = g.N < ng_want ? g.N : ng_want;
        const int nper = cdiv(g.N, ng);
        ng = cdiv(g.N, nper);
        const int ngpad = (int)align_up((size_t)ng, 4);
        int nparts = ngpad, nper_call = nper;
        if (mixed_grad_W3_takes(g, l.KXP)) {
            nper_call = cdiv(g.N, mix_groups_w3(ctx, g, l));
            nparts = cdiv(g.N, nper_call);
        }
        CHECK(mixed_grad_W(g, c.T, c.VT, c.RT, at(ctx, l.Gn), at(ctx, l.Gp), l.KX, l.KXP, nparts, nper_call, s));
        const long count = (long)g.M * g.C * g.Ay * l.KXP;
        char *out = at(ctx, l.TW);
        hipLaunchKernelGGL(k_fft_sum_groups<float>, dim3((unsigned)((count + 63) / 64), 2), dim3(64), 0, s,
                           (const cplx<float> *)at(ctx, l.Gn), (const cplx<float> *)at(ctx, l.Gp), (cplx<float> *)out,
                           (cplx<float> *)(out + (size_t)count * l.csz), count, nparts, 1.0 / l.Lx);
        TNMF_LAUNCH_CHECK();
    } else {
        CHECK(forward_planes(g, l, dtype, R, g.N * g.C, g.Dy, g.Dx, c.Ts, c.SR, s));
        int ngroups = l.ngroups;
        if (use_resident(l)) {
            CHECK(spectra_of_H(ctx, g, c, dtype, H, s));
            const long blocks = (long)cdiv(g.M, 4) * (((long)l.Ly * l.KXP + 255) / 256) * cdiv(g.C, 4);
            int ng = (int)((8L * ctx->num_cu + blocks - 1) / blocks);
            ng = ng < 1 ? 1 : (ng > l.ngroups ? l.ngroups : ng);
            const int nper = cdiv(g.N, ng);
            ngroups = cdiv(g.N, nper);
            CHECK(spectral_grad_W(g, dtype, c.SH, c.SV, c.SR, at(ctx, l.Gn), at(ctx, l.Gp), l.Ly, l.KX, l.KXP, ngroups,
                                  nper, s));
        } else {
            FftArgs a = base_args(g, l);
            a.src0 = c.T;
            a.src1 = c.SV;
            a.src2 = c.SR;
            a.dst0 = at(ctx, l.Gn);
            a.dst1 = at(ctx, l.Gp);
            a.ngroups = l.ngroups;
            a.nper = l.nper;
            CHECK(l.colf(kFftGradW, dtype, &a, s));
        }
        const long count = (long)g.M * g.C * l.Ly * l.KXP;
        const size_t sbytes = (size_t)count * l.csz;
        const double scale = 1.0 / ((double)l.Ly * l.Lx);
        {
            char *out = at(ctx, l.Gs);
            const dim3 grid((unsigned)((count + 63) / 64), 2);
            if (dtype == 0)
                hipLaunchKernelGGL(k_fft_sum_groups<float>, grid, dim3(64), 0, s, (const cplx<float> *)at(ctx, l.Gn),
                                   (const cplx<float> *)at(ctx, l.Gp), (cplx<float> *)out, (cplx<float> *)(out + sbytes),
                                   count, ngroups, scale);
            else
                hipLaunchKernelGGL(k_fft_sum_groups<double>, grid, dim3(64), 0, s, (const cplx<double> *)at(ctx, l.Gn),
                                   (const cplx<double> *)at(ctx, l.Gp), (cplx<double> *)out,
                                   (cplx<double> *)(out + sbytes), count, ngroups, scale);
            TNMF_LAUNCH_CHECK();
        }
        FftArgs b = base_args(g, l);
        b.src0 = at(ctx, l.Gs);
        b.dst0 = at(ctx, l.TW);
        b.planes = planes;
        b.rows = g.Ay;
        b.yoff = 0;
        CHECK(l.colf(kFftColsInv, dtype, &b, s));
    }
    FftArgs d = base_args(g, l);
    d.src0 = at(ctx, l.TW);
    d.dst0 = at(ctx, l.Wo);
    d.planes = planes;
    d.rows = g.Ay;
    d.cols = g.Ax;
    d.xoff = 0;
    d.ld_dst = g.Ax;
    d.ps_dst = (long)g.Ay * g.Ax;
    CHECK(l.rowf(kFftRowsInv, dtype, &d, s));
    const int per = g.M * g.C * g.Ay * g.Ax;
    const char *wo = at(ctx, l.Wo);
    if (dtype == 0) {
        hipLaunchKernelGGL(k_fft_flip_out<float>, dim3(cdiv(per, 256)), dim3(256), 0, s, (const float *)wo,
                           (float *)neg, g.M * g.C, g.Ay, g.Ax, nonneg ? 1 : 0);
        hipLaunchKernelGGL(k_fft_flip_out<float>, dim3(cdiv(per, 256)), dim3(256), 0, s, (const float *)wo + per,
                           (float *)pos, g.M * g.C, g.Ay, g.Ax, nonneg ? 1 : 0);
    } else {
        hipLaunchKernelGGL(k_fft_flip_out<double>, dim3(cdiv(per, 256)), dim3(256), 0, s, (const double *)wo,
                           (double *)neg, g.M * g.C, g.Ay, g.Ax, nonneg ? 1 : 0);
        hipLaunchKernelGGL(k_fft_flip_out<double>, dim3(cdiv(per, 256)), dim3(256), 0, s, (const double *)wo + per,
                           (double *)pos, g.M * g.C, g.Ay, g.Ax, nonneg ? 1 : 0);
    }
    TNMF_LAUNCH_CHECK();
    return TNMF_OK;
}
```

tnmf_amd/csrc/fft_kernels.h:

```cpp
#pragma once
#include <atomic>
#include "fft.h"
#include "fft_engine.h"
#include "fft_len_twiddles.h"

namespace {


template <int L>
struct LenCfg {
    static constexpr int col_tile = L > 384 ? 8 : 16;
    static constexpr int col_threads = (L == 270 || L == 540) ? 480 : (L > 192 ? 512 : 256);
    static_assert((L * col_tile) % col_threads == 0 && (L * 16) % col_threads == 0, "whole tile elements per thread");
    static constexpr int col_elems = L * col_tile / col_threads;
    static constexpr int row_pairs = L > 288 ? 8 : 16;
    static constexpr int row_threads = 256;
    static constexpr int mu_pairs = L > 288 ? 4 : 8;
    static constexpr int mu_threads = L / 2 + 1 > 256 ? 512 : 256;
};

template <int L, bool WIDE>
struct ColTile {
    static constexpr int v = WIDE ? 16 : LenCfg<L>::col_tile;
};

template <typename T, int L>
__device__ __forceinline__ void make_twiddles(cplx<T> *tw, int tid, int nt) {
    static_assert(sizeof(tnmf_len_twiddles) == sizeof(double) * 2 * L, "the table of this translation unit's length");
    for (int t = tid; t < L; t += nt) tw[t] = {(T)tnmf_len_twiddles[t][0], (T)tnmf_len_twiddles[t][1]};
}

template <typename T, typename P, int NB, int BS, int NT>
__device__ __forceinline__ void tile_fwd(cplx<T> *x, const cplx<T> *tw, int tid) {
#pragma unroll 1
    for (int t = tid; t < NB * P::tasks1; t += NT) P::template fwd1<BS>(x + (t % NB), tw, t / NB);
    __syncthreads();
#pragma unroll 1
    for (int t = tid; t < NB * P::tasks2; t += NT) P::template fwd2<BS>(x + (t % NB), tw, t / NB);
    __syncthreads();
#pragma unroll 1
    for (int t = tid; t < NB * P::tasks3; t += NT) P::template fwd3<BS>(x + (t % NB), t / NB);
    __syncthreads();
}

template <typename T, typename P, int NB, int BS, int NT>
__device__ __forceinline__ void tile_inv(cplx<T> *x, const cplx<T> *tw, int tid) {
#pragma unroll 1
    for (int t = tid; t < NB * P::tasks3; t += NT) P::template inv3<BS>(x + (t % NB), t / NB);
    __syncthreads();
#pragma unroll 1
    for (int t = tid; t < NB * P::tasks2; t += NT) P::template inv2<BS>(x + (t % NB), tw, t / NB);
    __syncthreads();
#pragma unroll 1
    for (int t = tid; t < NB * P::tasks1; t += NT) P::template inv1<BS>(x + (t % NB), tw, t / NB);
    __syncthreads();
}


template <typename T, typename P, int NB, int BS, int NT>
__device__ __forceinline__ void store_rows_split(const cplx<T> *x, cplx<T> *dst, int y0, int rows, int KXP, int tid) {
    constexpr int L = P::L, KX = L / 2 + 1;
    for (int idx = tid; idx < 2 * NB * KX; idx += NT) {
        const int r = idx / KX, k = idx - r * KX, y = y0 + r;
        if (y >= rows) continue;
        const int pr = r >> 1;
        const cplx<T> z1 = x[P::pos_of_k(k) * BS + pr];
        const cplx<T> z2 = x[P::pos_of_k(k == 0 ? 0 : L - k) * BS + pr];
        cplx<T> A, B;
        split_pair(z1, z2, A, B);
        dst[(long)y * KXP + k] = (r & 1) ? B : A;
    }
}

template <typename T, typename P, int NB, int BS, int NT>
__device__ __forceinline__ void load_rows_merge(cplx<T> *x, const cplx<T> *src, int y0, int rows, int KXP, int tid) {
    constexpr int L = P::L, KX = L / 2 + 1;
    for (int idx = tid; idx < NB * KX; idx += NT) {
        const int pr = idx / KX, k = idx - pr * KX, ya = y0 + 2 * pr;
        cplx<T> A = {0, 0}, B = {0, 0};
        if (ya < rows) A = src[(long)ya * KXP + k];
        if (ya + 1 < rows) B = src[(long)(ya + 1) * KXP + k];
        if (k == 0 || 2 * k == L) {
            x[P::pos_of_k(k) * BS + pr] = {A.x, B.x};
        } else {
            cplx<T> zk, zlk;
            merge_pair(A, B, zk, zlk);
            x[P::pos_of_k(k) * BS + pr] = zk;
            x[P::pos_of_k(L - k) * BS + pr] = zlk;
        }
    }
}

template <typename T, int L, int NB, int NT>
__global__ __launch_bounds__(NT) void k_fft_rows_fwd(FftArgs a) {
    using P = FftPlanFor<T, L>;
    constexpr int BS = NB + 1, KX = L / 2 + 1, R2 = 2 * NB;
    constexpr int XS = (L + NT - 1) / NT, KS = (KX + NT - 1) / NT;
    extern __shared__ __align__(16) unsigned char smem[];
    cplx<T> *x = reinterpret_cast<cplx<T> *>(smem);
    cplx<T> *tw = x + L * BS;
    const int tid = threadIdx.x, y0 = blockIdx.x * R2;
    const long plane = blockIdx.y;
    make_twiddles<T, L>(tw, tid, NT);
    const T *src = static_cast<const T *>(a.src0) + plane * a.ps_src;
    T *xr = reinterpret_cast<T *>(x);
    if (tid < L) {
        const int xc = min(tid, a.cols - 1);
        T v[R2];
#pragma unroll
        for (int r = 0; r < R2; ++r) v[r] = src[(long)min(y0 + r, a.rows - 1) * a.ld_src + xc];
#pragma unroll
        for (int r = 0; r < R2; ++r) xr[tid * (2 * BS) + r] = (y0 + r < a.rows && tid < a.cols) ? v[r] : (T)0;
    }
    if constexpr (XS > 2) {
#pragma unroll
        for (int sl = 1; sl < XS; ++sl) {
            const int xx = tid + sl * NT;
            if (xx < L) {
                const int xc = min(xx, a.cols - 1);
                T v[R2];
#pragma unroll
                for (int r = 0; r < R2; ++r) v[r] = src[(long)min(y0 + r, a.rows - 1) * a.ld_src + xc];
#pragma unroll
                for (int r = 0; r < R2; ++r) xr[xx * (2 * BS) + r] = (y0 + r < a.rows && xx < a.cols) ? v[r] : (T)0;
            }
        }
    } else if constexpr (XS == 2) {
        const int rem = a.cols > NT ? a.cols - NT : 0, c0 = NT + rem;
        for (int idx = tid; idx < rem * R2; idx += NT) {
            const int r = idx / rem, c = idx - r * rem;
            xr[(NT + c) * (2 * BS) + r] = y0 + r < a.rows ? src[(long)(y0 + r) * a.ld_src + NT + c] : (T)0;
        }
        for (int idx = tid; idx < (L - c0) * R2; idx += NT) {
            const int c = idx / R2, r = idx - c * R2;
            xr[(c0 + c) * (2 * BS) + r] = (T)0;
        }
    }
    __syncthreads();
    tile_fwd<T, P, NB, BS, NT>(x, tw, tid);
    cplx<T> *dst = static_cast<cplx<T> *>(a.dst0) + plane * a.ps_dst;
#pragma unroll
    for (int ks = 0; ks < KS; ++ks) {
        const int k = tid + ks * NT;
        if (k < KX) {
            const int pk = P::pos_of_k(k) * BS, plk = P::pos_of_k(k == 0 ? 0 : L - k) * BS;
#pragma unroll
            for (int p = 0; p < NB; ++p) {
                const int ya = y0 + 2 * p;
                cplx<T> A, B;
                split_pair(x[pk + p], x[plk + p], A, B);
                if (ya < a.rows) dst[(long)ya * a.KXP + k] = A;
                if (ya + 1 < a.rows) dst[(long)(ya + 1) * a.KXP + k] = B;
            }
        }
    }
}

template <typename T, int L, int NB, int NT, int MODE>
__global__ __launch_bounds__(NT) void k_fft_rows_inv(FftArgs a) {
    using P = FftPlanFor<T, L>;
    constexpr int BS = NB + 1;
    extern __shared__ __align__(16) unsigned char smem[];
    cplx<T> *x = reinterpret_cast<cplx<T> *>(smem);
    cplx<T> *xb = x + L * BS;
    cplx<T> *tw = MODE == 0 ? xb : xb + L * BS;
    const int tid = threadIdx.x, y0 = blockIdx.x * 2 * NB;
    const long plane = blockIdx.y;
    make_twiddles<T, L>(tw, tid, NT);
    const long tin = plane * ((long)a.rows * a.KXP);
    load_rows_merge<T, P, NB, BS, NT>(x, static_cast<const cplx<T> *>(a.src0) + tin, y0, a.rows, a.KXP, tid);
    if (MODE != 0)
        load_rows_merge<T, P, NB, BS, NT>(xb, static_cast<const cplx<T> *>(a.src1) + tin, y0, a.rows, a.KXP, tid);
    __syncthreads();
    tile_inv<T, P, NB, BS, NT>(x, tw, tid);
    if (MODE != 0) tile_inv<T, P, NB, BS, NT>(xb, tw, tid);
    const T *xr = reinterpret_cast<const T *>(x);
    const T *xbr = reinterpret_cast<const T *>(xb);
    T *d0 = static_cast<T *>(a.dst0) + plane * a.ps_dst;
    T *d1 = MODE == 1 ? static_cast<T *>(a.dst1) + plane * a.ps_dst : nullptr;
    for (int idx = tid; idx < 2 * NB * a.cols; idx += NT) {
        const int r = idx / a.cols, xc = idx - r * a.cols, y = y0 + r;
        if (y >= a.rows) continue;
        const int off = ((xc + a.xoff) * BS + (r >> 1)) * 2 + (r & 1);
        T v = xr[off];
        if (MODE == 0 && a.clamp0) v = v < (T)0 ? (T)0 : v;
        d0[(long)y * a.ld_dst + xc] = v;
        if (MODE == 1) d1[(long)y * a.ld_dst + xc] = xbr[off];
    }
}

template <typename T, int L, int NB, int NT>
__global__ __launch_bounds__(NT) void k_fft_rows_mu(FftArgs a) {
    using P = FftPlanFor<T, L>;
    constexpr int BS = NB + 1, KX = L / 2 + 1, R2 = 2 * NB;
    constexpr int XS = (L + NT - 1) / NT;
    constexpr int KS = (KX + NT - 1) / NT;
    static_assert(KS == 1, "block size must cover Lx/2+1 frequencies");
    extern __shared__ __align__(16) unsigned char smem[];
    cplx<T> *x = reinterpret_cast<cplx<T> *>(smem);
    cplx<T> *tw = x + L * BS;
    T *stash = reinterpret_cast<T *>(tw + L);
    T *xr = reinterpret_cast<T *>(x);
    const int tid = threadIdx.x, y0 = blockIdx.x * R2;
    const long plane = blockIdx.y;
    make_twiddles<T, L>(tw, tid, NT);
    const long tin = plane * ((long)a.rows * a.KXP);
    const cplx<T> *sn = static_cast<const cplx<T> *>(a.src0) + tin;
    const cplx<T> *sp = static_cast<const cplx<T> *>(a.src1) + tin;
    T *Hp = static_cast<T *>(a.dst0) + plane * a.ps_src;
    const int k = tid < KX ? tid : KX - 1;
    const bool kact = tid < KX;
    const int pk = P::pos_of_k(k) * BS, plk = P::pos_of_k(k == 0 ? 0 : L - k) * BS;
    const bool kself = (k == 0 || 2 * k == L);
    cplx<T> na[NB], nb[NB], pa[NB], pb[NB];
#pragma unroll
    for (int p = 0; p < NB; ++p) {
        na[p] = sn[(long)min(y0 + 2 * p, a.rows - 1) * a.KXP + k];
        nb[p] = sn[(long)min(y0 + 2 * p + 1, a.rows - 1) * a.KXP + k];
    }
#pragma unroll
    for (int p = 0; p < NB; ++p) {
        pa[p] = sp[(long)min(y0 + 2 * p, a.rows - 1) * a.KXP + k];
        pb[p] = sp[(long)min(y0 + 2 * p + 1, a.rows - 1) * a.KXP + k];
    }
    const int xc = min(tid, a.cols - 1);
    T hv[R2];
#pragma unroll
    for (int r = 0; r < R2; ++r) hv[r] = Hp[(long)min(y0 + r, a.rows - 1) * a.ld_dst + xc];
    if (kact) {
#pragma unroll
        for (int p = 0; p < NB; ++p) {
            const int ya = y0 + 2 * p;
            cplx<T> A = na[p], B = nb[p];
            if (ya >= a.rows) A = {0, 0};
            if (ya + 1 >= a.rows) B = {0, 0};
            if (kself) {
                x[pk + p] = {A.x, B.x};
            } else {
                cplx<T> zk, zlk;
                merge_pair(A, B, zk, zlk);
                x[pk + p] = zk;
                x[plk + p] = zlk;
            }
        }
    }
    __syncthreads();
    tile_inv<T, P, NB, BS, NT>(x, tw, tid);
    T ng[R2];
    if (tid < L) {
#pragma unroll
        for (int r = 0; r < R2; ++r) ng[r] = xr[tid * (2 * BS) + r];
    }
#pragma unroll
    for (int sl = 1; sl < XS; ++sl) {
        const int xx = tid + sl * NT;
        if (xx < L) {
#pragma unroll
            for (int r = 0; r < R2; ++r) stash[(xx - NT) * R2 + r] = xr[xx * (2 * BS) + r];
        }
    }
    __syncthreads();
    if (kact) {
#pragma unroll
        for (int p = 0; p < NB; ++p) {
            const int ya = y0 + 2 * p;
            cplx<T> A = pa[p], B = pb[p];
            if (ya >= a.rows) A = {0, 0};
            if (ya + 1 >= a.rows) B = {0, 0};
            if (kself) {
                x[pk + p] = {A.x, B.x};
            } else {
                cplx<T> zk, zlk;
                merge_pair(A, B, zk, zlk);
                x[pk + p] = zk;
                x[plk + p] = zlk;
            }
        }
    }
    __syncthreads();
    tile_inv<T, P, NB, BS, NT>(x, tw, tid);
    const T reg = (T)a.reg;
    if (tid < L) {
#pragma unroll
        for (int r = 0; r < R2; ++r) {
            const int y = y0 + r, off = tid * (2 * BS) + r;
            T hn = 0;
            if (y < a.rows && tid < a.cols) {
                hn = (hv[r] * fmax(ng[r], (T)0)) / (fmax(xr[off], (T)0) + reg);
                Hp[(long)y * a.ld_dst + tid] = hn;
            }
            xr[off] = hn;
        }
    }
#pragma unroll
    for (int sl = 1; sl < XS; ++sl) {
        const int xx = tid + sl * NT;
        if (xx < L) {
#pragma unroll
            for (int r = 0; r < R2; ++r) {
                const int y = y0 + r, off = xx * (2 * BS) + r;
                T hn = 0;
                if (y < a.rows && xx < a.cols) {
                    hn = (Hp[(long)y * a.ld_dst + xx] * fmax(stash[(xx - NT) * R2 + r], (T)0)) / (fmax(xr[off], (T)0) + reg);
                    Hp[(long)y * a.ld_dst + xx] = hn;
                }
                xr[off] = hn;
            }
        }
    }
    __syncthreads();
    tile_fwd<T, P, NB, BS, NT>(x, tw, tid);
    if (kact) {
        cplx<T> *dst = static_cast<cplx<T> *>(a.dst1) + plane * a.ps_dst;
#pragma unroll
        for (int p = 0; p < NB; ++p) {
            const int ya = y0 + 2 * p;
            cplx<T> A, B;
            split_pair(x[pk + p], x[plk + p], A, B);
            if (ya < a.rows) dst[(long)ya * a.KXP + k] = A;
            if (ya + 1 < a.rows) dst[(long)(ya + 1) * a.KXP + k] = B;
        }
    }
}


template <typename T, int L, int NT, bool WIDE>
__device__ __forceinline__ void load_col_tile(cplx<T> *x, const cplx<T> *src, int rows, int KXP, int KX, int kx0,
                                              int tid) {
    for (int idx = tid; idx < L * ColTile<L, WIDE>::v; idx += NT) {
        const int y = idx / ColTile<L, WIDE>::v, col = idx % ColTile<L, WIDE>::v, kx = kx0 + col;
        cplx<T> v = {0, 0};
        if (y < rows && kx < KX) v = src[(long)y * KXP + kx];
        x[y * (ColTile<L, WIDE>::v + 1) + col] = v;
    }
}

template <typename T, int L, int NT, bool WIDE>
__device__ __forceinline__ void store_col_tile_rows(const cplx<T> *x, cplx<T> *dst, int rows, int yoff, int KXP, int KX,
                                                    int kx0, int tid) {
    for (int idx = tid; idx < rows * ColTile<L, WIDE>::v; idx += NT) {
// ... 171 lines not shown
        for (int c = 0; c < CR; ++c) fetch_col<T, L, NT, WIDE>(sv[c], S + ((long)n * a.C + c) * splane, ln, L, a.KXP);
        fetch_col<T, L, NT, WIDE>(wb[0], SWf + (long)mbeg * a.C * splane, ln, L, a.KXP);
    }
    __syncthreads();
    for (int m = mbeg; m < mend; ++m) {
        if (CH > 0) {
            cplx<T> g[E];
#pragma unroll
            for (int e = 0; e < E; ++e) g[e] = {0, 0};
#pragma unroll
            for (int c = 0; c < CR; ++c) {
                if (c + 1 < CR)
                    fetch_col<T, L, NT, WIDE>(wb[(c + 1) & 1], SWf + ((long)m * a.C + c + 1) * splane, ln, L, a.KXP);
#pragma unroll
                for (int e = 0; e < E; ++e) cfma(g[e], sv[c][e], wb[c & 1][e]);
            }
#pragma unroll
            for (int e = 0; e < E; ++e) {
                const int idx = tid + e * NT;
                x[(idx / ColTile<L, WIDE>::v) * (ColTile<L, WIDE>::v + 1) + (idx % ColTile<L, WIDE>::v)] = g[e];
            }
        } else {
#pragma unroll
            for (int e = 0; e < E; ++e) {
                const int idx = tid + e * NT, pos = idx / ColTile<L, WIDE>::v, col = idx % ColTile<L, WIDE>::v;
                cplx<T> g = {0, 0};
                for (int c = 0; c < a.C; ++c)
                    cfma(g, (S + ((long)n * a.C + c) * splane)[(unsigned)(pos * a.KXP + ln.kxc)],
                         (SWf + ((long)m * a.C + c) * splane)[(unsigned)(pos * a.KXP + ln.kxc)]);
                x[pos * (ColTile<L, WIDE>::v + 1) + col] = g;
            }
        }
        __syncthreads();
        if (CH > 0) fetch_col<T, L, NT, WIDE>(wb[0], SWf + (long)min(m + 1, mend - 1) * a.C * splane, ln, L, a.KXP);
        tile_inv<T, P, ColTile<L, WIDE>::v, (ColTile<L, WIDE>::v + 1), NT>(x, tw, tid);
        store_col_tile_rows<T, L, NT, WIDE>(x, Tout + ((long)nl * a.M + m) * tplane, a.Hy, 0, a.KXP, a.KX, kx0, tid);
        __syncthreads();
    }
}

template <typename T, int L, int NT, int CG>
__global__ __launch_bounds__(NT) void k_fft_grad_W(FftArgs a) {
    using P = FftPlanFor<T, L>;
    constexpr bool WIDE = false;
    constexpr int E = L * ColTile<L, WIDE>::v / NT;
    extern __shared__ __align__(16) unsigned char smem[];
    cplx<T> *x = reinterpret_cast<cplx<T> *>(smem);
    cplx<T> *tw = x + L * (ColTile<L, WIDE>::v + 1);
    const int tid = threadIdx.x, m = blockIdx.x, kx0 = blockIdx.y * ColTile<L, WIDE>::v;
    const int grp = blockIdx.z % a.ngroups, c0 = (blockIdx.z / a.ngroups) * CG;
    make_twiddles<T, L>(tw, tid, NT);
    const cplx<T> *Tsrc = static_cast<const cplx<T> *>(a.src0);
    const cplx<T> *SV = static_cast<const cplx<T> *>(a.src1);
    const cplx<T> *SR = static_cast<const cplx<T> *>(a.src2);
    const long tplane = (long)a.Hy * a.KXP, splane = (long)L * a.KXP;
    cplx<T> an[CG][E], ap[CG][E], pre[E];
#pragma unroll
    for (int cc = 0; cc < CG; ++cc)
#pragma unroll
        for (int e = 0; e < E; ++e) {
            an[cc][e] = {0, 0};
            ap[cc][e] = {0, 0};
        }
    const int nbeg = grp * a.nper, nend = min(a.N, nbeg + a.nper);
    const ColLane ln = col_lane<L, NT, WIDE>(a.KX, kx0, tid);
    if (nbeg < nend) fetch_col<T, L, NT, WIDE>(pre, Tsrc + ((long)nbeg * a.M + m) * tplane, ln, a.Hy, a.KXP);
    for (int n = nbeg; n < nend; ++n) {
        commit_col_tile<T, L, NT, WIDE>(x, pre, a.Hy, a.KX, kx0, tid);
        __syncthreads();
        constexpr bool PRE = CG == 1 && E <= 12;
        cplx<T> v[PRE ? E : 1], r[PRE ? E : 1];
        if (PRE) {
            fetch_col<T, L, NT, WIDE>(v, SV + ((long)n * a.C + c0) * splane, ln, L, a.KXP);
            fetch_col<T, L, NT, WIDE>(r, SR + ((long)n * a.C + c0) * splane, ln, L, a.KXP);
        }
        fetch_col<T, L, NT, WIDE>(pre, Tsrc + ((long)min(n + 1, nend - 1) * a.M + m) * tplane, ln, a.Hy, a.KXP);
        tile_fwd<T, P, ColTile<L, WIDE>::v, (ColTile<L, WIDE>::v + 1), NT>(x, tw, tid);
#pragma unroll
        for (int e = 0; e < E; ++e) {
            const int idx = tid + e * NT, pos = idx / ColTile<L, WIDE>::v, col = idx % ColTile<L, WIDE>::v;
            const cplx<T> h = x[pos * (ColTile<L, WIDE>::v + 1) + col];
            if (PRE) {
                cfmac(an[0][e], h, v[PRE ? e : 0]);
                cfmac(ap[0][e], h, r[PRE ? e : 0]);
            } else {
#pragma unroll
                for (int cc = 0; cc < CG; ++cc) {
                    const long pl = ((long)n * a.C + min(c0 + cc, a.C - 1)) * splane;
                    const unsigned o = (unsigned)(pos * a.KXP + ln.kxc);
                    cfmac(an[cc][e], h, (SV + pl)[o]);
                    cfmac(ap[cc][e], h, (SR + pl)[o]);
                }
            }
        }
        __syncthreads();
    }
    cplx<T> *Gn = static_cast<cplx<T> *>(a.dst0) + (long)grp * a.M * a.C * splane;
    cplx<T> *Gp = static_cast<cplx<T> *>(a.dst1) + (long)grp * a.M * a.C * splane;
#pragma unroll
    for (int cc = 0; cc < CG; ++cc) {
        if (c0 + cc >= a.C) continue;
#pragma unroll
        for (int e = 0; e < E; ++e) {
            const int idx = tid + e * NT, pos = idx / ColTile<L, WIDE>::v, col = idx % ColTile<L, WIDE>::v, kx = kx0 + col;
            if (kx < a.KX) {
                const long o = ((long)m * a.C + c0 + cc) * splane + (long)pos * a.KXP + kx;
                Gn[o] = an[cc][e];
                Gp[o] = ap[cc][e];
            }
        }
    }
}


template <typename K>
int set_lds_limit(K kernel, size_t bytes) {
    if (bytes > 64 * 1024) TNMF_HIP_TRY(hipFuncSetAttribute((const void *)kernel,
                                                           hipFuncAttributeMaxDynamicSharedMemorySize, 160 * 1024));
    return TNMF_OK;
}

#define TNMF_FFT_LAUNCH(kernel, grid, threads, lds)                         \
    do {                                                                    \
        static std::atomic<unsigned long long> attr_done{0};                \
        int dev_ = 0;                                                       \
        TNMF_HIP_TRY(hipGetDevice(&dev_));                                  \
        const unsigned long long bit_ = 1ull << (dev_ & 63);                \
        if (!(attr_done.load(std::memory_order_acquire) & bit_)) {          \
             \
                                             \
            const int _rc = set_lds_limit(kernel, (lds));                   \
            if (_rc != TNMF_OK) return _rc;                                 \
            attr_done.fetch_or(bit_, std::memory_order_release);            \
        }                                                                   \
        hipLaunchKernelGGL(kernel, grid, dim3(threads), (lds), s, *a);      \
        TNMF_LAUNCH_CHECK();                                                \
        return TNMF_OK;                                                     \
    } while (0)

template <typename T, int L>
int fft_run_typed(int op, const FftArgs *a, hipStream_t s) {
    using Cfg = LenCfg<L>;
    constexpr int NB = (sizeof(T) == 8 && L > 144) ? Cfg::row_pairs / 2 : Cfg::row_pairs;
    constexpr int NTR = Cfg::row_threads, NTC = Cfg::col_threads;
    constexpr size_t row_tile = (size_t)L * (NB + 1) * sizeof(cplx<T>), tw_bytes = (size_t)L * sizeof(cplx<T>);
    constexpr size_t col_lds = (size_t)L * (LenCfg<L>::col_tile + 1) * sizeof(cplx<T>) + tw_bytes;
    constexpr size_t wide_lds = (size_t)L * 17 * sizeof(cplx<T>) + tw_bytes;
    if (row_tile * 2 + tw_bytes > 160 * 1024 || col_lds > 160 * 1024 || wide_lds > 160 * 1024) return TNMF_E_UNSUPPORTED;
    FftArgs flat;
    if ((op == kFftRowsFwd || op == kFftRowsInv) && a->rows == 1 && a->planes > 1) {
        flat = *a;
        flat.rows = a->planes;
        flat.planes = 1;
        a = &flat;
    }
    const dim3 rgrid((unsigned)cdiv(a->rows, 2 * NB), (unsigned)a->planes);
    const unsigned tiles = (unsigned)cdiv(a->KX, LenCfg<L>::col_tile), wide_tiles = (unsigned)cdiv(a->KX, 16);
    switch (op) {
        case kFftRowsFwd: TNMF_FFT_LAUNCH((k_fft_rows_fwd<T, L, NB, NTR>), rgrid, NTR, row_tile + tw_bytes);
        case kFftRowsInv: TNMF_FFT_LAUNCH((k_fft_rows_inv<T, L, NB, NTR, 0>), rgrid, NTR, row_tile + tw_bytes);
        case kFftRowsInv2: TNMF_FFT_LAUNCH((k_fft_rows_inv<T, L, NB, NTR, 1>), rgrid, NTR, 2 * row_tile + tw_bytes);
        case kFftRowsMu: {
            constexpr int NBM = (sizeof(T) == 8 && L > 144) ? Cfg::mu_pairs / 2 : Cfg::mu_pairs;
            const dim3 mgrid((unsigned)cdiv(a->rows, 2 * NBM), (unsigned)a->planes);
            constexpr int NTM = Cfg::mu_threads;
            constexpr size_t stash = L > NTM ? (size_t)(L - NTM) * 2 * NBM * sizeof(T) : 0;
            TNMF_FFT_LAUNCH((k_fft_rows_mu<T, L, NBM, NTM>), mgrid, NTM,
                            (size_t)L * (NBM + 1) * sizeof(cplx<T>) + tw_bytes + stash);
        }
        case kFftColsFwd:
            TNMF_FFT_LAUNCH((k_fft_cols_fwd<T, L, NTC>), dim3(tiles, (unsigned)a->planes), NTC, col_lds);
        case kFftColsInv:
            TNMF_FFT_LAUNCH((k_fft_cols_inv<T, L, NTC>), dim3(tiles, (unsigned)a->planes), NTC, col_lds);
        case kFftContractR: {
            const int cg = a->C <= 3 ? a->C : 4;
            const dim3 grid((unsigned)a->N, tiles, (unsigned)cdiv(a->C, cg));
            if (cg == 1) TNMF_FFT_LAUNCH((k_fft_contract_R<T, L, NTC, 1>), grid, NTC, col_lds);
            if (cg == 2) TNMF_FFT_LAUNCH((k_fft_contract_R<T, L, NTC, 2>), grid, NTC, col_lds);
            if (cg == 3) TNMF_FFT_LAUNCH((k_fft_contract_R<T, L, NTC, 3>), grid, NTC, col_lds);
            TNMF_FFT_LAUNCH((k_fft_contract_R<T, L, NTC, 4>), grid, NTC, col_lds);
        }
        case kFftGradH: {
            const dim3 grid((unsigned)a->planes, wide_tiles, 2u * (unsigned)a->mgroups);
            if (a->C == 1) TNMF_FFT_LAUNCH((k_fft_grad_H<T, L, NTC, 1>), grid, NTC, wide_lds);
            if (a->C == 2) TNMF_FFT_LAUNCH((k_fft_grad_H<T, L, NTC, 2>), grid, NTC, wide_lds);
            if (a->C == 3) TNMF_FFT_LAUNCH((k_fft_grad_H<T, L, NTC, 3>), grid, NTC, wide_lds);
            if (a->C == 4) TNMF_FFT_LAUNCH((k_fft_grad_H<T, L, NTC, 4>), grid, NTC, wide_lds);
            TNMF_FFT_LAUNCH((k_fft_grad_H<T, L, NTC, 0>), grid, NTC, wide_lds);
        }
        case kFftGradW: {
            const int cg = a->C <= 2 ? a->C : (Cfg::col_elems <= 9 ? 3 : 2);
            const dim3 grid((unsigned)a->M, tiles, (unsigned)(a->ngroups * cdiv(a->C, cg)));
            if (cg == 1) TNMF_FFT_LAUNCH((k_fft_grad_W<T, L, NTC, 1>), grid, NTC, col_lds);
            if (cg == 2) TNMF_FFT_LAUNCH((k_fft_grad_W<T, L, NTC, 2>), grid, NTC, col_lds);
            TNMF_FFT_LAUNCH((k_fft_grad_W<T, L, NTC, 3>), grid, NTC, col_lds);
        }
        default: break;
    }
    return TNMF_E_UNSUPPORTED;
}

}
```

Measured before the change: 213.4.

## Chain inverse and forward row FFTs for reconstruct-to-grad_W and fuse W scaling/flip

Adds a reconstruct variant for grad_W that, after the inverse row FFT, re-runs the forward row FFT on the clamped result in the same kernel and stashes the row spectra. A tag on the FFT state lets grad_W skip its own forward row pass over R when the stashed spectra match. It also folds the 1/Lx scaling of W into the forward row load, and folds the flip/split of the grad_W output into the inverse row store, removing separate scaling and flip kernels. The cost is extra cache-validity bookkeeping with many invalidation points and a more complex store path.

```diff
diff --git a/include/tnmf_hip.h b/include/tnmf_hip.h
--- a/include/tnmf_hip.h
+++ b/include/tnmf_hip.h
@@ -58,6 +58,9 @@
 int tnmf_hip_reconstruct(tnmf_hip_ctx *ctx, const tnmf_hip_geom *geom, const void *W, const void *H, void *R,
                          void *stream);
 
+int tnmf_hip_reconstruct_for_grad_W(tnmf_hip_ctx *ctx, const tnmf_hip_geom *geom, const void *W, const void *H, void *R,
+                                    void *stream);
+
 int tnmf_hip_grad_H(tnmf_hip_ctx *ctx, const tnmf_hip_geom *geom, const void *V, const void *R_or_null,
                     const void *W, const void *H, void *neg, void *pos, void *stream);
 
diff --git a/tnmf_amd/_lib.py b/tnmf_amd/_lib.py
--- a/tnmf_amd/_lib.py
+++ b/tnmf_amd/_lib.py
@@ -26,6 +26,7 @@
     'tnmf_hip_find_peaks',
     'tnmf_hip_events_render', 'tnmf_hip_events_update', 'tnmf_hip_events_grad_W', 'tnmf_hip_events_gain',
     'tnmf_hip_events_norms', 'tnmf_hip_pursuit_score', 'tnmf_hip_pursuit_pick',
+    'tnmf_hip_reconstruct_for_grad_W',
 )
 
 MODES = {'valid': 0, 'full': 1, 'circular': 2, 'reflect': 3}
@@ -98,6 +99,8 @@
     lib.tnmf_hip_ctx_last_path.restype = ctypes.c_char_p
     lib.tnmf_hip_ctx_last_path.argtypes = [vp]
     lib.tnmf_hip_reconstruct.argtypes = [vp, gp, vp, vp, vp, vp]
+    lib.tnmf_hip_reconstruct_for_grad_W.restype = ci
+    lib.tnmf_hip_reconstruct_for_grad_W.argtypes = [vp, gp, vp, vp, vp, vp]
     lib.tnmf_hip_grad_H.argtypes = [vp, gp, vp, vp, vp, vp, vp, vp, vp]
     lib.tnmf_hip_grad_W.argtypes = [vp, gp, vp, vp, vp, vp, vp, vp, vp]
     lib.tnmf_hip_mu_update.argtypes = [vp, ci, vp, vp, vp, cd, sz, vp]
diff --git a/tnmf_amd/backends/HIP.py b/tnmf_amd/backends/HIP.py
--- a/tnmf_amd/backends/HIP.py
+++ b/tnmf_amd/backends/HIP.py
@@ -1025,9 +1025,10 @@
             g = self._geom(Hc.shape[0], W.shape[0], ld)
             r_valid = 0
             if self._timeline is not None and Hc.shape[0]:
+                chained = Gs is None and beta == 2
+                recon = self._lib.tnmf_hip_reconstruct_for_grad_W if chained else self._lib.tnmf_hip_reconstruct
                 with self._timed('reconstruct'):
-                    rc = self._lib.tnmf_hip_reconstruct(self._ctx, ctypes.byref(g), _ptr(W), _ptr(Hc), _ptr(Rs),
-                                                        self._stream())
+                    rc = recon(self._ctx, ctypes.byref(g), _ptr(W), _ptr(Hc), _ptr(Rs), self._stream())
                 if rc != 0:
                     return rc, 'tnmf_hip_reconstruct'
                 r_valid = 1
diff --git a/tnmf_amd/csrc/api.hip b/tnmf_amd/csrc/api.hip
--- a/tnmf_amd/csrc/api.hip
+++ b/tnmf_amd/csrc/api.hip
@@ -198,10 +198,11 @@
     return TNMF_OK;
 }
 
-int do_reconstruct(tnmf_hip_ctx *ctx, const Geo &g, int dtype, const void *W, const void *H, void *R, hipStream_t s) {
+int do_reconstruct(tnmf_hip_ctx *ctx, const Geo &g, int dtype, const void *W, const void *H, void *R, hipStream_t s,
+                   bool for_grad_W = false) {
     if (g.N == 0) return TNMF_OK;
     if (ctx->path == TNMF_PATH_FFT || use_fft_hybrid(ctx, g, dtype)) {
-        const int rc = fft_reconstruct(ctx, g, dtype, W, H, R, true, s);
+        const int rc = fft_reconstruct(ctx, g, dtype, W, H, R, true, s, for_grad_W);
         if (!(rc == TNMF_E_WORKSPACE && ctx->path == TNMF_PATH_AUTO)) return rc;
     }
     if (g.Hs == g.Hx && use_mfma(ctx, g, dtype, kReconstruct)) {
@@ -687,6 +688,14 @@
     return do_reconstruct(ctx, g, dtype, W, H, R, s);
 }
 
+int tnmf_hip_reconstruct_for_grad_W(tnmf_hip_ctx *ctx, const tnmf_hip_geom *geom, const void *W, const void *H, void *R,
+                                    void *stream) {
+    if (is_vol(geom)) return vol_api_reconstruct(ctx, geom, W, H, R, stream);
+    ENTER(ctx, geom);
+    if (!W || (g.N > 0 && (!H || !R))) return TNMF_E_NULL;
+    return do_reconstruct(ctx, g, dtype, W, H, R, s, true);
+}
+
 int tnmf_hip_grad_H(tnmf_hip_ctx *ctx, const tnmf_hip_geom *geom, const void *V, const void *R_or_null,
                     const void *W, const void *H, void *neg, void *pos, void *stream) {
     if (is_vol(geom)) return vol_api_grad_H(ctx, geom, V, R_or_null, W, H, neg, pos, stream);
@@ -1014,7 +1023,7 @@
     CHECK(ensure_scratch(ctx, sc.total));
     if (r_is_valid && !R_scratch) return TNMF_E_NULL;
     void *Rs = R_scratch ? R_scratch : ws_at(ctx, sc.r_off);
-    if (!r_is_valid) CHECK(do_reconstruct(ctx, g, dtype, W, H, Rs, s));
+    if (!r_is_valid) CHECK(do_reconstruct(ctx, g, dtype, W, H, Rs, s, !beta && !G));
     if ((beta || G) && g.N > 0) CHECK(beta_fields_of(ctx, g, dtype, beta, eps, V, G, Rs, &V, s));
     char *np = static_cast<char *>(negpos);
     const size_t wbytes = (size_t)g.M * g.C * g.Ay * g.Ax * esize(dtype);
diff --git a/tnmf_amd/csrc/common.h b/tnmf_amd/csrc/common.h
--- a/tnmf_amd/csrc/common.h
+++ b/tnmf_amd/csrc/common.h
@@ -36,6 +36,15 @@
     Geo W_geo = {};
     int W_dtype = 0;
     unsigned long long h_runs = 0, h_hits = 0, v_runs = 0, v_hits = 0;
+    struct RTag {
+        bool ok = false;
+        const void *R = nullptr;
+        const void *spec = nullptr;
+        int n0 = 0, dtype = 0;
+        Geo geo = {};
+        unsigned long long epoch = 0;
+    } r_tag;
+    unsigned long long ws_epoch = 0;
 };
 
 struct tnmf_hip_ctx {
diff --git a/tnmf_amd/csrc/fft.h b/tnmf_amd/csrc/fft.h
--- a/tnmf_amd/csrc/fft.h
+++ b/tnmf_amd/csrc/fft.h
@@ -13,6 +13,8 @@
     int n0, ngroups, nper;
     int mgroups, mper;
     int clamp0;
+    int flip;
+    double scale;
     double reg;
 };
 
@@ -26,6 +28,7 @@
     kFftContractR,
     kFftGradH,
     kFftGradW,
+    kFftRowsInvFwd,
 };
 
 typedef int (*fft_run_fn)(int op, int dtype, const FftArgs *a, hipStream_t s);
@@ -75,7 +78,7 @@
 int fft_reserve(tnmf_hip_ctx *ctx, const Geo &g, int dtype, bool with_window);
 
 int fft_reconstruct(tnmf_hip_ctx *ctx, const Geo &g, int dtype, const void *W, const void *H, void *R, bool nonneg,
-                    hipStream_t s);
+                    hipStream_t s, bool for_grad_W = false);
 int fft_grad_H(tnmf_hip_ctx *ctx, const Geo &g, int dtype, const void *V, const void *R, const void *W, void *neg,
                void *pos, hipStream_t s);
 int fft_update_H(tnmf_hip_ctx *ctx, const Geo &g, int dtype, const void *V, const void *R, const void *W, void *H,
diff --git a/tnmf_amd/csrc/fft.hip b/tnmf_amd/csrc/fft.hip
--- a/tnmf_amd/csrc/fft.hip
+++ b/tnmf_amd/csrc/fft.hip
@@ -123,7 +123,10 @@
     return true;
 }
 
+void drop_r_tag(FftState &f) { f.r_tag.ok = false; }
+
 void clear_flags(FftState &f) {
+    drop_r_tag(f);
     f.W_ok = false;
     std::fill(f.T_ok.begin(), f.T_ok.end(), 0);
     std::fill(f.SH_ok.begin(), f.SH_ok.end(), 0);
@@ -150,6 +153,7 @@
         TNMF_HIP_TRY(hipFree(f.ws));
         f.ws = nullptr;
         f.ws_bytes = 0;
+        ++f.ws_epoch;
         clear_flags(f);
     }
     if (!bigger && hipMalloc(&bigger, want) != hipSuccess) {
@@ -159,6 +163,7 @@
     }
     f.ws = bigger;
     f.ws_bytes = want;
+    ++f.ws_epoch;
     clear_flags(f);
     return TNMF_OK;
 }
@@ -298,6 +303,7 @@
 }
 
 void bind(FftState &f, const Geo &g, int dtype, const void *H, const void *V, bool explicit_bind) {
+    drop_r_tag(f);
     f.bound = true;
     f.explicit_bind = explicit_bind;
     f.H_base = H;
@@ -391,8 +397,9 @@
 }
 
 int forward_rows(const Geo &g, const Lay &l, int dtype, const void *src, int planes, int rows, int cols, void *Tdst,
-                 hipStream_t s) {
+                 hipStream_t s, double scale = 0.0) {
     FftArgs a = base_args(g, l);
+    a.scale = scale;
     a.src0 = src;
     a.dst0 = Tdst;
     a.planes = planes;
@@ -489,6 +496,7 @@
 
 void fft_unbind(tnmf_hip_ctx *ctx) {
     FftState &f = ctx->fft;
+    drop_r_tag(f);
     f.bound = f.explicit_bind = false;
     f.H_base = f.V_base = nullptr;
     f.T_ok.clear();
@@ -499,6 +507,7 @@
 
 void fft_invalidate_H(tnmf_hip_ctx *ctx, const Geo &g, int dtype, const void *H) {
     FftState &f = ctx->fft;
+    drop_r_tag(f);
     const Slot sl = locate(f, g, dtype, H, nullptr);
     if (sl.cached) {
         set_ok(f.T_ok, sl.n0, g.N, 0);
@@ -511,10 +520,14 @@
 
 void fft_invalidate(tnmf_hip_ctx *ctx) { clear_flags(ctx->fft); }
 
-void fft_invalidate_W(tnmf_hip_ctx *ctx) { ctx->fft.W_ok = false; }
+void fft_invalidate_W(tnmf_hip_ctx *ctx) {
+    drop_r_tag(ctx->fft);
+    ctx->fft.W_ok = false;
+}
 
 int fft_reserve(tnmf_hip_ctx *ctx, const Geo &g, int dtype, bool with_window) {
     Lay l;
+    drop_r_tag(ctx->fft);
     ctx->fft.failed_bytes = 0;
     const FftState &f = ctx->fft;
     const bool in_binding = f.bound && f.dtype == dtype && same_shape(f.geo, g) && f.geo.N >= g.N;
@@ -527,11 +540,13 @@
     ctx->fft.ws = nullptr;
     ctx->fft.ws_bytes = 0;
     ctx->fft.failed_bytes = 0;
+    ++ctx->fft.ws_epoch;
     clear_flags(ctx->fft);
 }
 
 int fft_reconstruct(tnmf_hip_ctx *ctx, const Geo &g, int dtype, const void *W, const void *H, void *R, bool nonneg,
-                    hipStream_t s) {
+                    hipStream_t s, bool for_grad_W) {
+    drop_r_tag(ctx->fft);
     Call c;
     CHECK(prepare(ctx, g, dtype, H, nullptr, &c));
     const Lay &l = c.l;
@@ -548,8 +563,12 @@
     if (use_mixed(g, dtype, false)) {
         if (!w_hit) {
             f.W_ok = false;
+#ifdef TNMF_FFT_NO_ROWS_CHAIN
             CHECK(scaled_W(ctx, g, l, dtype, W, 1.0 / l.Lx, s));
             CHECK(forward_rows(g, l, dtype, at(ctx, l.Wt), g.M * g.C, g.Ay, g.Ax, at(ctx, l.TWr), s));
+#else
+            CHECK(forward_rows(g, l, dtype, W, g.M * g.C, g.Ay, g.Ax, at(ctx, l.TWr), s, 1.0 / l.Lx));
+#endif
             w_mark();
         }
         CHECK(mixed_reconstruct(g, c.T, at(ctx, l.TWr), c.Ts, l.KX, l.KXP, s));
@@ -587,6 +606,20 @@
     d.ld_dst = g.Dx;
     d.ps_dst = (long)g.Dy * g.Dx;
     d.clamp0 = nonneg ? 1 : 0;
+#ifndef TNMF_FFT_NO_ROWS_CHAIN
+    if (for_grad_W && f.cache_enabled && !(g.Dy == 1 && g.Ay == 1)) {
+        d.dst1 = use_mixed(g, dtype, true) ? c.RT : c.Ts;
+        CHECK(l.rowf(kFftRowsInvFwd, dtype, &d, s));
+        f.r_tag.ok = true;
+        f.r_tag.R = R;
+        f.r_tag.spec = d.dst1;
+        f.r_tag.n0 = c.sl.n0;
+        f.r_tag.dtype = dtype;
+        f.r_tag.geo = g;
+        f.r_tag.epoch = f.ws_epoch;
+        return TNMF_OK;
+    }
+#endif
     return l.rowf(kFftRowsInv, dtype, &d, s);
 }
 
@@ -618,6 +651,7 @@
 
 int fft_grad_H(tnmf_hip_ctx *ctx, const Geo &g, int dtype, const void *V, const void *R, const void *W, void *neg,
                void *pos, hipStream_t s) {
+    drop_r_tag(ctx->fft);
     if (g.Dy == 1 && g.Ay == 1) return TNMF_E_UNSUPPORTED;
     Call c;
     CHECK(prepare(ctx, g, dtype, nullptr, V, &c, true));
@@ -645,6 +679,7 @@
 
 int fft_update_H(tnmf_hip_ctx *ctx, const Geo &g, int dtype, const void *V, const void *R, const void *W, void *H,
                  double reg, hipStream_t s) {
+    drop_r_tag(ctx->fft);
     if (g.Dy == 1 && g.Ay == 1) return TNMF_E_UNSUPPORTED;
     Call c;
     CHECK(prepare(ctx, g, dtype, H, V, &c, true));
@@ -718,15 +753,19 @@
 
 int fft_grad_W(tnmf_hip_ctx *ctx, const Geo &g, int dtype, const void *V, const void *R, const void *H, void *neg,
                void *pos, bool nonneg, hipStream_t s) {
+    const FftState::RTag tag = ctx->fft.r_tag;
+    drop_r_tag(ctx->fft);
     Call c;
     CHECK(prepare(ctx, g, dtype, H, V, &c));
     const Lay &l = c.l;
     CHECK(rows_of_H(ctx, g, c, dtype, H, s));
     const bool mixed = use_mixed(g, dtype, true);
+    const bool r_hit = tag.ok && tag.R == R && tag.spec == (mixed ? c.RT : c.Ts) && tag.n0 == c.sl.n0 && tag.dtype == dtype &&
+                       tag.geo.N == g.N && same_shape(tag.geo, g) && tag.epoch == ctx->fft.ws_epoch;
     CHECK(spectra_V(ctx, g, c, dtype, V, !mixed, s));
     const int planes = 2 * g.M * g.C;
     if (mixed) {
-        CHECK(forward_rows(g, l, dtype, R, g.N * g.C, g.Dy, g.Dx, c.RT, s));
+        if (!r_hit) CHECK(forward_rows(g, l, dtype, R, g.N * g.C, g.Dy, g.Dx, c.RT, s));
         int ng_want = mix_groups(ctx, g, l);
         if (const char *e = tnmf_diag_env("TNMF_MIX_GROUPS")) ng_want = atoi(e);
         ng_want = ng_want < 1 ? 1 : (ng_want > kMixMaxGroups ? kMixMaxGroups : ng_want);
@@ -747,7 +786,10 @@
                            (cplx<float> *)(out + (size_t)count * l.csz), count, nparts, 1.0 / l.Lx);
         TNMF_LAUNCH_CHECK();
     } else {
-        CHECK(forward_planes(g, l, dtype, R, g.N * g.C, g.Dy, g.Dx, c.Ts, c.SR, s));
+        if (r_hit)
+            CHECK(columns_of(g, l, dtype, c.Ts, g.N * g.C, g.Dy, c.SR, s));
+        else
+            CHECK(forward_planes(g, l, dtype, R, g.N * g.C, g.Dy, g.Dx, c.Ts, c.SR, s));
         int ngroups = l.ngroups;
         if (use_resident(l)) {
             CHECK(spectra_of_H(ctx, g, c, dtype, H, s));
@@ -795,6 +837,19 @@
     }
     FftArgs d = base_args(g, l);
     d.src0 = at(ctx, l.TW);
+#ifndef TNMF_FFT_NO_ROWS_CHAIN
+    d.dst0 = neg;
+    d.dst1 = pos;
+    d.planes = planes;
+    d.rows = g.Ay;
+    d.cols = g.Ax;
+    d.xoff = 0;
+    d.ld_dst = g.Ax;
+    d.ps_dst = (long)g.Ay * g.Ax;
+    d.clamp0 = nonneg ? 1 : 0;
+    d.flip = 1;
+    return l.rowf(kFftRowsInv, dtype, &d, s);
+#else
     d.dst0 = at(ctx, l.Wo);
     d.planes = planes;
     d.rows = g.Ay;
@@ -818,4 +873,5 @@
     }
     TNMF_LAUNCH_CHECK();
     return TNMF_OK;
-}
+#endif
+}
diff --git a/tnmf_amd/csrc/fft_kernels.h b/tnmf_amd/csrc/fft_kernels.h
--- a/tnmf_amd/csrc/fft_kernels.h
+++ b/tnmf_amd/csrc/fft_kernels.h
@@ -89,6 +89,17 @@
             x[P::pos_of_k(L - k) * BS + pr] = zlk;
         }
     }
+}
+
+#ifdef TNMF_FFT_NO_ROWS_CHAIN
+constexpr bool kRowsChain = false;
+#else
+constexpr bool kRowsChain = true;
+#endif
+
+template <typename T>
+__device__ __forceinline__ T scaled_load(double scale, T v) {
+    return kRowsChain && scale != 0 ? (T)(scale * (double)v) : v;
 }
 
 template <typename T, int L, int NB, int NT>
@@ -109,6 +120,10 @@
         T v[R2];
 #pragma unroll
         for (int r = 0; r < R2; ++r) v[r] = src[(long)min(y0 + r, a.rows - 1) * a.ld_src + xc];
+        if (kRowsChain && a.scale != 0) {
+#pragma unroll
+            for (int r = 0; r < R2; ++r) v[r] = (T)(a.scale * (double)v[r]);
+        }
 #pragma unroll
         for (int r = 0; r < R2; ++r) xr[tid * (2 * BS) + r] = (y0 + r < a.rows && tid < a.cols) ? v[r] : (T)0;
     }
@@ -120,7 +135,7 @@
                 const int xc = min(xx, a.cols - 1);
                 T v[R2];
 #pragma unroll
-                for (int r = 0; r < R2; ++r) v[r] = src[(long)min(y0 + r, a.rows - 1) * a.ld_src + xc];
+                for (int r = 0; r < R2; ++r) v[r] = scaled_load(a.scale, src[(long)min(y0 + r, a.rows - 1) * a.ld_src + xc]);
 #pragma unroll
                 for (int r = 0; r < R2; ++r) xr[xx * (2 * BS) + r] = (y0 + r < a.rows && xx < a.cols) ? v[r] : (T)0;
             }
@@ -129,7 +144,7 @@
         const int rem = a.cols > NT ? a.cols - NT : 0, c0 = NT + rem;
         for (int idx = tid; idx < rem * R2; idx += NT) {
             const int r = idx / rem, c = idx - r * rem;
-            xr[(NT + c) * (2 * BS) + r] = y0 + r < a.rows ? src[(long)(y0 + r) * a.ld_src + NT + c] : (T)0;
+            xr[(NT + c) * (2 * BS) + r] = y0 + r < a.rows ? scaled_load(a.scale, src[(long)(y0 + r) * a.ld_src + NT + c]) : (T)0;
         }
         for (int idx = tid; idx < (L - c0) * R2; idx += NT) {
             const int c = idx / R2, r = idx - c * R2;
@@ -151,6 +166,104 @@
                 split_pair(x[pk + p], x[plk + p], A, B);
                 if (ya < a.rows) dst[(long)ya * a.KXP + k] = A;
                 if (ya + 1 < a.rows) dst[(long)(ya + 1) * a.KXP + k] = B;
+            }
+        }
+    }
+}
+
+template <typename T, typename P, int NB, int BS, int NT>
+__device__ __forceinline__ void load_rows_merge_kx(cplx<T> *x, const cplx<T> *src, int y0, int rows, int KXP, int tid) {
+    constexpr int L = P::L, KX = L / 2 + 1, KS = (KX + NT - 1) / NT;
+#pragma unroll
+    for (int ks = 0; ks < KS; ++ks) {
+        const int k = tid + ks * NT;
+        if (k < KX) {
+            const int pk = P::pos_of_k(k) * BS, plk = P::pos_of_k(k == 0 ? 0 : L - k) * BS;
+            const bool kself = (k == 0 || 2 * k == L);
+            cplx<T> A[NB], B[NB];
+#pragma unroll
+            for (int p = 0; p < NB; ++p) {
+                A[p] = src[(long)min(y0 + 2 * p, rows - 1) * KXP + k];
+                B[p] = src[(long)min(y0 + 2 * p + 1, rows - 1) * KXP + k];
+            }
+#pragma unroll
+            for (int p = 0; p < NB; ++p) {
+                const int ya = y0 + 2 * p;
+                if (ya >= rows) A[p] = {0, 0};
+                if (ya + 1 >= rows) B[p] = {0, 0};
+                cplx<T> zk, zlk;
+                merge_pair(A[p], B[p], zk, zlk);
+                if (kself) zk = {A[p].x, B[p].x};
+                x[plk + p] = zlk;
+                x[pk + p] = zk;
+            }
+        }
+    }
+}
+
+template <typename T, int L, int NB, int BS, int NT, int MODE>
+__device__ __forceinline__ void store_rows_real(const cplx<T> *x, const cplx<T> *xb, const FftArgs &a, long plane, int y0,
+                                                int tid) {
+    T *d0 = static_cast<T *>(a.dst0) + plane * a.ps_dst;
+    T *d1 = MODE == 1 ? static_cast<T *>(a.dst1) + plane * a.ps_dst : nullptr;
+    const bool clamp = MODE == 0 && a.clamp0, flip = MODE == 0 && a.flip;
+    const bool whole = y0 + 2 * NB <= a.rows;
+    const long half = (long)a.planes * a.rows / 2;
+    auto put = [&](int r, int xc, T v, T vb) {
+        const int y = y0 + r;
+        if (y >= a.rows) return;
+        if (flip) {
+            const long G = plane * a.rows + (a.flip == 1 ? a.rows - 1 - y : y);
+            T *d = G < half ? static_cast<T *>(a.dst0) + G * a.ld_dst : static_cast<T *>(a.dst1) + (G - half) * a.ld_dst;
+            d[a.cols - 1 - xc] = v;
+        } else {
+            d0[(long)y * a.ld_dst + xc] = v;
+            if (MODE == 1) d1[(long)y * a.ld_dst + xc] = vb;
+        }
+    };
+    auto column = [&](int xc) {
+        const cplx<T> *col = x + (xc + a.xoff) * BS, *colb = xb + (xc + a.xoff) * BS;
+        cplx<T> z[NB], zb[MODE == 1 ? NB : 1];
+#pragma unroll
+        for (int p = 0; p < NB; ++p) {
+            z[p] = col[p];
+            if (MODE == 1) zb[p] = colb[p];
+        }
+        if (clamp) {
+#pragma unroll
+            for (int p = 0; p < NB; ++p) z[p] = {z[p].x < (T)0 ? (T)0 : z[p].x, z[p].y < (T)0 ? (T)0 : z[p].y};
+        }
+        if (whole && !flip) {
+            T *e0 = d0 + (long)y0 * a.ld_dst + xc, *e1 = MODE == 1 ? d1 + (long)y0 * a.ld_dst + xc : nullptr;
+#pragma unroll
+            for (int p = 0; p < NB; ++p) {
+                e0[(long)(2 * p) * a.ld_dst] = z[p].x;
+                e0[(long)(2 * p + 1) * a.ld_dst] = z[p].y;
+                if (MODE == 1) {
+                    e1[(long)(2 * p) * a.ld_dst] = zb[p].x;
+                    e1[(long)(2 * p + 1) * a.ld_dst] = zb[p].y;
+                }
+            }
+        } else {
+#pragma unroll
+            for (int p = 0; p < NB; ++p) {
+                put(2 * p, xc, z[p].x, MODE == 1 ? zb[p].x : (T)0);
+                put(2 * p + 1, xc, z[p].y, MODE == 1 ? zb[p].y : (T)0);
+            }
+        }
+    };
+    if (tid < a.cols) column(tid);
+    if constexpr (L > NT) {
+        int c0 = NT;
+        for (; c0 + NT <= a.cols; c0 += NT) column(c0 + tid);
+        const int rem = a.cols - c0;
+        if (rem > 0) {
+            const T *xr = reinterpret_cast<const T *>(x), *xbr = reinterpret_cast<const T *>(xb);
+            for (int idx = tid; idx < rem * 2 * NB; idx += NT) {
+                const int r = idx / rem, xc = c0 + idx - r * rem, off = (xc + a.xoff) * (2 * BS) + r;
+                T v = xr[off];
+                if (clamp) v = v < (T)0 ? (T)0 : v;
+                put(r, xc, v, MODE == 1 ? xbr[off] : (T)0);
             }
         }
     }
@@ -167,6 +280,7 @@
     const int tid = threadIdx.x, y0 = blockIdx.x * 2 * NB;
     const long plane = blockIdx.y;
     make_twiddles<T, L>(tw, tid, NT);
+#ifdef TNMF_FFT_NO_ROWS_CHAIN
     const long tin = plane * ((long)a.rows * a.KXP);
     load_rows_merge<T, P, NB, BS, NT>(x, static_cast<const cplx<T> *>(a.src0) + tin, y0, a.rows, a.KXP, tid);
     if (MODE != 0)
@@ -186,6 +300,76 @@
         if (MODE == 0 && a.clamp0) v = v < (T)0 ? (T)0 : v;
         d0[(long)y * a.ld_dst + xc] = v;
         if (MODE == 1) d1[(long)y * a.ld_dst + xc] = xbr[off];
+    }
+#else
+    const long tin = plane * ((long)a.rows * a.KXP);
+    load_rows_merge_kx<T, P, NB, BS, NT>(x, static_cast<const cplx<T> *>(a.src0) + tin, y0, a.rows, a.KXP, tid);
+    if (MODE != 0)
+        load_rows_merge_kx<T, P, NB, BS, NT>(xb, static_cast<const cplx<T> *>(a.src1) + tin, y0, a.rows, a.KXP, tid);
+    __syncthreads();
+    tile_inv<T, P, NB, BS, NT>(x, tw, tid);
+    if (MODE != 0) tile_inv<T, P, NB, BS, NT>(xb, tw, tid);
+    store_rows_real<T, L, NB, BS, NT, MODE>(x, xb, a, plane, y0, tid);
+#endif
+}
+
+template <typename T, int L, int NB, int NT>
+__global__ __launch_bounds__(NT) void k_fft_rows_inv_fwd(FftArgs a) {
+    using P = FftPlanFor<T, L>;
+    constexpr int BS = NB + 1, KX = L / 2 + 1, XS = (L + NT - 1) / NT, KS = (KX + NT - 1) / NT;
+    extern __shared__ __align__(16) unsigned char smem[];
+    cplx<T> *x = reinterpret_cast<cplx<T> *>(smem);
+    cplx<T> *tw = x + L * BS;
+    const int tid = threadIdx.x, y0 = blockIdx.x * 2 * NB;
+    const long plane = blockIdx.y;
+    make_twiddles<T, L>(tw, tid, NT);
+    const long tin = plane * ((long)a.rows * a.KXP);
+    load_rows_merge_kx<T, P, NB, BS, NT>(x, static_cast<const cplx<T> *>(a.src0) + tin, y0, a.rows, a.KXP, tid);
+    __syncthreads();
+    tile_inv<T, P, NB, BS, NT>(x, tw, tid);
+    store_rows_real<T, L, NB, BS, NT, 0>(x, x, a, plane, y0, tid);
+    cplx<T> z[XS][NB];
+#pragma unroll
+    for (int sl = 0; sl < XS; ++sl) {
+        const int xx = tid + sl * NT;
+#pragma unroll
+        for (int p = 0; p < NB; ++p) {
+            cplx<T> v = {0, 0};
+            if (xx < a.cols) {
+                v = x[(xx + a.xoff) * BS + p];
+                if (a.clamp0) v = {v.x < (T)0 ? (T)0 : v.x, v.y < (T)0 ? (T)0 : v.y};
+                if (y0 + 2 * p >= a.rows) v.x = 0;
+                if (y0 + 2 * p + 1 >= a.rows) v.y = 0;
+            }
+            z[sl][p] = v;
+        }
+    }
+    __syncthreads();
+#pragma unroll
+    for (int sl = 0; sl < XS; ++sl) {
+        const int xx = tid + sl * NT;
+        if (xx < L) {
+#pragma unroll
+            for (int p = 0; p < NB; ++p) x[xx * BS + p] = z[sl][p];
+        }
+    }
+    __syncthreads();
+    tile_fwd<T, P, NB, BS, NT>(x, tw, tid);
+    cplx<T> *dst = static_cast<cplx<T> *>(a.dst1) + tin;
+#pragma unroll
+    for (int ks = 0; ks < KS; ++ks) {
+        const int k = tid + ks * NT;
+        if (k < KX) {
+            const int pk = P::pos_of_k(k) * BS, plk = P::pos_of_k(k == 0 ? 0 : L - k) * BS;
+#pragma unroll
+            for (int p = 0; p < NB; ++p) {
+                const int ya = y0 + 2 * p;
+                cplx<T> A, B;
+                split_pair(x[pk + p], x[plk + p], A, B);
+                if (ya < a.rows) dst[(long)ya * a.KXP + k] = A;
+                if (ya + 1 < a.rows) dst[(long)(ya + 1) * a.KXP + k] = B;
+            }
+        }
     }
 }
 
@@ -663,6 +847,7 @@
         flat = *a;
         flat.rows = a->planes;
         flat.planes = 1;
+        if (flat.flip) flat.flip = 2;
         a = &flat;
     }
     const dim3 rgrid((unsigned)cdiv(a->rows, 2 * NB), (unsigned)a->planes);
@@ -671,6 +856,9 @@
         case kFftRowsFwd: TNMF_FFT_LAUNCH((k_fft_rows_fwd<T, L, NB, NTR>), rgrid, NTR, row_tile + tw_bytes);
         case kFftRowsInv: TNMF_FFT_LAUNCH((k_fft_rows_inv<T, L, NB, NTR, 0>), rgrid, NTR, row_tile + tw_bytes);
         case kFftRowsInv2: TNMF_FFT_LAUNCH((k_fft_rows_inv<T, L, NB, NTR, 1>), rgrid, NTR, 2 * row_tile + tw_bytes);
+#ifndef TNMF_FFT_NO_ROWS_CHAIN
+        case kFftRowsInvFwd: TNMF_FFT_LAUNCH((k_fft_rows_inv_fwd<T, L, NB, NTR>), rgrid, NTR, row_tile + tw_bytes);
+#endif
         case kFftRowsMu: {
             constexpr int NBM = (sizeof(T) == 8 && L > 144) ? Cfg::mu_pairs / 2 : Cfg::mu_pairs;
             const dim3 mgrid((unsigned)cdiv(a->rows, 2 * NBM), (unsigned)a->planes);
```

Result: no change. 215.1 (median of 6 runs) (+0.8%).
